# sxyu/plenoctree

Hardware: AMD Instinct MI355X
Metric: training rays/sec (800x800, 64+128 samples) (higher is better)
Workload: dtype f32

## Files before the change

### include/plenoctree_hip.h

```cpp
#ifndef PLENOCTREE_HIP_H_
#define PLENOCTREE_HIP_H_

#include <stddef.h>
#include <stdint.h>

#ifdef __cplusplus
extern "C" {
#endif

#define PXO_OK 0
#define PXO_ERR_ARG (-1)
#define PXO_ERR_HIP (-2)
#define PXO_ERR_WORKSPACE (-3)
#define PXO_ERR_UNSUPPORTED (-4)

#define PXO_NET_DEPTH 8
#define PXO_NET_WIDTH 256
#define PXO_SKIP_LAYER 4
#define PXO_ENC_DIM 63
#define PXO_ENC_PAD 64
#define PXO_NUM_LEAVES 20
#define PXO_VD_NUM_LEAVES 24
#define PXO_VD_WIDTH_CONDITION 128
#define PXO_VD_DIR_ENC 27

typedef struct PxoCfg {
  int32_t num_coarse_samples;
  int32_t num_fine_samples;
  int32_t sh_deg;
  int32_t min_deg_point;
  int32_t max_deg_point;
  int32_t white_bkgd;
  int32_t lindisp;
  int32_t sparsity_npoints;
  float near_;
  float far_;
  float sparsity_weight;
  float sparsity_length;
  float sparsity_radius;
  float weight_decay_mult;
  int32_t mlp_precision;
  float noise_std;
  int32_t skip_zero_rows;
} PxoCfg;

#define PXO_MLP_F32 0
#define PXO_MLP_BF16X3 1
#define PXO_MLP_BF16X6 2

typedef struct PxoLeaf {
  int32_t layer;
  int32_t is_bias;
  int64_t offset;
  int32_t rows;
  int32_t cols;
} PxoLeaf;

#define PXO_ABI_VERSION 9
const char* pxo_last_error(void);
int pxo_version(void);
size_t pxo_cfg_bytes(void);
int pxo_tile_rows(void);

int pxo_param_layout(const PxoCfg* cfg, PxoLeaf* leaves, int64_t* floats_per_mlp);

int pxo_packed_sizes(const PxoCfg* cfg, int64_t* fwd_floats, int64_t* bwd_floats);
int pxo_pack_weights(const PxoCfg* cfg, const float* mlp_params, float* packed_fwd,
                     float* packed_bwd, void* stream);


int pxo_sample_along_rays(const float* origins, const float* directions, int64_t B, int S,
                          float near_, float far_, int lindisp, const float* t_rand,
                          float* z_vals, float* pts, void* stream);

int pxo_posenc(const float* x, int64_t N, float* enc, void* stream);

size_t pxo_relu_mask_bytes(int64_t M);
int pxo_mlp_fwd(const PxoCfg* cfg, const float* packed_fwd, const float* pts, int64_t M,
                float* raw_rgb, float* raw_sigma, float* acts, float* enc, void* relu_mask,
                void* stream);

size_t pxo_dbias_partial_bytes(int64_t M);
int pxo_mlp_bwd_data(const PxoCfg* cfg, const float* packed_bwd, const float* d_raw_rgb,
                     const float* d_raw_sigma, const void* relu_mask, int64_t M, float* dz,
                     float* dbias_partial, void* stream);

int pxo_wgrad_workspace_bytes(const PxoCfg* cfg, int64_t M, size_t* bytes);
int pxo_mlp_bwd_weights(const PxoCfg* cfg, const float* acts, const float* enc, const float* dz,
                        const float* d_raw_rgb, const float* d_raw_sigma,
                        const float* dbias_partial, int64_t M, float* grads, void* ws,
                        size_t ws_bytes, void* stream);

int pxo_shade_composite_fwd(const PxoCfg* cfg, const float* raw_rgb, const float* raw_sigma,
                            const float* z_vals, const float* directions, const float* viewdirs,
                            int64_t B, int S, float* comp_rgb, float* disp, float* acc,
                            float* weights, void* stream);
int pxo_shade_composite_bwd(const PxoCfg* cfg, const float* raw_rgb, const float* raw_sigma,
                            const float* z_vals, const float* directions, const float* viewdirs,
                            const float* d_comp_rgb, int64_t B, int S, float* d_raw_rgb,
                            float* d_raw_sigma, void* stream);

int pxo_shade_composite_train(const PxoCfg* cfg, const float* raw_rgb, const float* raw_sigma,
                              const float* z_vals, const float* directions, const float* viewdirs,
                              const float* pixels, int64_t B, int S, float* comp_rgb, float* weights,
                              float* ray_sse, float* d_raw_rgb, float* d_raw_sigma, int64_t n_sp,
                              float* sp_exp, void* stream);

int pxo_sample_pdf(const float* z_coarse, const float* w_coarse, const float* origins,
                   const float* directions, int64_t B, int Nc, int Nf, const float* u,
                   float* z_out, float* pts, void* stream);

int pxo_add_gaussian_noise(float* raw, int64_t n, float noise_std, const float* noise, uint64_t seed,
                           uint64_t stream_id, void* stream);

int pxo_uniform(uint64_t seed, uint64_t stream_id, int64_t n, float lo, float hi, float* out,
                void* stream);

int pxo_randint(uint64_t seed, uint64_t stream_id, int64_t count, int64_t n, int64_t* out, void* stream);

int pxo_generate_rays(const float* c2w, int W, int H, float focal, const int64_t* pixel_ids, int64_t B,
                      float* origins, float* directions, float* viewdirs, void* stream);

int pxo_sample_batch(uint64_t seed, uint64_t stream_id, const float* c2w, int W, int H, float focal,
                     const float* image_rgb, int64_t B, int64_t first, int64_t* pixel_ids, float* origins,
                     float* directions, float* viewdirs, float* pixels, void* stream);

int pxo_generate_rays_multi(const float* c2w, int n_cams, int W, int H, float focal, const int64_t* ray_ids,
                            int64_t B, float* origins, float* directions, float* viewdirs, void* stream);

int pxo_generate_rays_ndc(const float* c2w, int n_cams, int W, int H, float focal, float ndc_near, const int64_t* ray_ids,
                          int64_t B, float* origins, float* directions, float* viewdirs, void* stream);

int pxo_sample_batch_ndc(uint64_t seed, uint64_t stream_id, const float* c2w, int W, int H, float focal, float ndc_near,
                         const float* image_rgb, int64_t B, int64_t first, int64_t* pixel_ids, float* origins,
                         float* directions, float* viewdirs, float* pixels, void* stream);

int pxo_mean_over_samples(const PxoCfg* cfg, const float* raw_rgb, const float* raw_sigma, int64_t n_cells,
                          int S, float* out, void* stream);

int pxo_adam_step(float* params, float* m, float* v, const float* grads, int64_t n, float lr,
                  int64_t step, float grad_scale, void* stream);

int pxo_adam_pack_step(const PxoCfg* cfg, float* params, float* m, float* v, const float* grads, float lr,
                       int64_t step, float grad_scale, float* packed_fwd0, float* packed_bwd0,
                       float* packed_fwd1, float* packed_bwd1, void* stream);


int pxo_render_workspace_bytes(const PxoCfg* cfg, int64_t B, size_t* bytes);
int pxo_render_fwd(const PxoCfg* cfg, const float* packed_fwd0, const float* packed_fwd1,
                   const float* origins, const float* directions, const float* viewdirs,
                   int64_t B, int randomized, const float* t_rand, const float* u, uint64_t seed,
                   float* rgb_c, float* disp_c, float* acc_c, float* rgb_f, float* disp_f,
                   float* acc_f, void* ws, size_t ws_bytes, void* stream);

int pxo_sg_render_fwd(const PxoCfg* cfg, const float* lobes, const float* packed_fwd0, const float* packed_fwd1,
                      const float* origins, const float* directions, const float* viewdirs, int64_t B, int randomized,
                      const float* t_rand, const float* u, uint64_t seed, float* rgb_c, float* disp_c, float* acc_c,
                      float* rgb_f, float* disp_f, float* acc_f, void* ws, size_t ws_bytes, void* stream);

#define PXO_OCC_MAX_RESO 1024
#define PXO_OCC_MAX_CHANNELS 4096
typedef struct PxoOccGrid {
  const uint32_t* bits;
  int32_t reso;
  float offset[3];
  float scale[3];
  int32_t outside_live;
} PxoOccGrid;

int pxo_occ_pack(const float* sigma, int reso, float sigma_thresh, int dilate, uint32_t* bits, void* stream);

int pxo_occ_cull_workspace_bytes(int64_t M, size_t* bytes);
int pxo_occ_cull(const PxoOccGrid* occ, const float* pts, int64_t M, float* pts_live, int32_t* slot, int64_t* n_live_dev, void* ws,
                 size_t ws_bytes, void* stream);

int pxo_occ_expand(const float* raw_rgb_live, const float* raw_sigma_live, const int32_t* slot, int64_t M, int C, float* raw_rgb,
                   float* raw_sigma, void* stream);

int pxo_render_culled_workspace_bytes(const PxoCfg* cfg, int64_t B, size_t* bytes);
int pxo_render_fwd_culled(const PxoCfg* cfg, const PxoOccGrid* occ, const float* lobes, const float* packed_fwd0,
                          const float* packed_fwd1, const float* origins, const float* directions, const float* viewdirs, int64_t B,
                          int randomized, const float* t_rand, const float* u, uint64_t seed, float* rgb_c, float* disp_c,
                          float* acc_c, float* rgb_f, float* disp_f, float* acc_f, int64_t live_rows[2], void* ws, size_t ws_bytes,
                          void* stream);

int pxo_occ_gather(const float* d_raw_rgb, const float* d_raw_sigma, const int32_t* slot, int64_t M, int C, float* d_rgb_live,
                   float* d_sigma_live, void* stream);

int pxo_train_culled_workspace_bytes(const PxoCfg* cfg, int64_t B, size_t* bytes);
int pxo_train_fwd_bwd_culled(const PxoCfg* cfg, const PxoOccGrid* occ, const float* params, const float* packed_fwd0,
                             const float* packed_bwd0, const float* packed_fwd1, const float* packed_bwd1, const float* origins,
                             const float* directions, const float* viewdirs, const float* pixels, int64_t B, int randomized,
                             const float* t_rand, const float* u, const float* sp_points, uint64_t seed, float* grads,
                             float* stats, void* ws, size_t ws_bytes, void* grads0_ready, void* stream, int64_t live_rows[2]);

int pxo_sg_lobes(const float* sg_params, int K, float* lobes, void* stream);

#define PXO_SG_RAYS_PER_BLOCK 4
int pxo_sg_shade_composite_train(const PxoCfg* cfg, const float* lobes, const float* raw_rgb, const float* raw_sigma,
                                 const float* z_vals, const float* directions, const float* viewdirs,
                                 const float* pixels, int64_t B, int S, float* comp_rgb, float* weights,
                                 float* ray_sse, float* d_raw_rgb, float* d_raw_sigma, int64_t n_sp,
                                 float* sp_exp, float* d_lobes, float* lobe_partials, void* stream);

int pxo_sg_train_workspace_bytes(const PxoCfg* cfg, int64_t B, size_t* bytes);
int pxo_sg_train_fwd_bwd_bucketed(const PxoCfg* cfg, const float* params, const float* sg_params, const float* packed_fwd0,
                                  const float* packed_bwd0, const float* packed_fwd1, const float* packed_bwd1,
                                  const float* origins, const float* directions, const float* viewdirs,
                                  const float* pixels, int64_t B, int randomized, const float* t_rand, const float* u,
                                  const float* sp_points, uint64_t seed, float* grads, float* sg_grads, float* stats,
                                  void* ws, size_t ws_bytes, void* grads0_ready, void* stream);
int pxo_sg_train_fwd_bwd(const PxoCfg* cfg, const float* params, const float* sg_params, const float* packed_fwd0,
                         const float* packed_bwd0, const float* packed_fwd1, const float* packed_bwd1,
                         const float* origins, const float* directions, const float* viewdirs, const float* pixels,
                         int64_t B, int randomized, const float* t_rand, const float* u, const float* sp_points,
                         uint64_t seed, float* grads, float* sg_grads, float* stats, void* ws, size_t ws_bytes,
                         void* stream);

int pxo_train_workspace_bytes(const PxoCfg* cfg, int64_t B, size_t* bytes);
int pxo_train_fwd_bwd(const PxoCfg* cfg, const float* params, const float* packed_fwd0,
                      const float* packed_bwd0, const float* packed_fwd1,
                      const float* packed_bwd1, const float* origins, const float* directions,
                      const float* viewdirs, const float* pixels, int64_t B, int randomized,
                      const float* t_rand, const float* u, const float* sp_points, uint64_t seed,
                      float* grads, float* stats, void* ws, size_t ws_bytes, void* stream);

int pxo_train_fwd_bwd_bucketed(const PxoCfg* cfg, const float* params, const float* packed_fwd0,
                               const float* packed_bwd0, const float* packed_fwd1,
                               const float* packed_bwd1, const float* origins, const float* directions,
                               const float* viewdirs, const float* pixels, int64_t B, int randomized,
                               const float* t_rand, const float* u, const float* sp_points, uint64_t seed,
                               float* grads, float* stats, void* ws, size_t ws_bytes, void* grads0_ready,
                               void* stream);

int pxo_train_backward_work(const PxoCfg* cfg, int64_t B, void* ws, size_t ws_bytes, int64_t* live_chunks,
                            int64_t* total_chunks, void* stream);

int pxo_event_create(void** event);
int pxo_event_destroy(void* event);
int pxo_stream_wait_event(void* stream, void* event);

int pxo_eval_points(const PxoCfg* cfg, const float* packed_fwd, const float* points, int64_t N,
                    float* raw_rgb, float* raw_sigma, void* stream);

int pxo_grid_sigma(const PxoCfg* cfg, const float* packed_fwd, int reso, int x0, int x1,
                   const float offset[3], const float scale[3], float* sigma_out, void* stream);

int pxo_vd_param_layout(PxoLeaf* leaves, int64_t* floats_per_mlp);
int pxo_vd_packed_floats(int64_t* floats);
int pxo_vd_pack_weights(const float* mlp_params, float* packed, void* stream);

int pxo_vd_eval_workspace_bytes(int64_t N, int64_t R, int cross_broadcast, size_t* bytes);
int pxo_vd_eval_points_raw(int mlp_precision, const float* packed, const float* points, int64_t N, const float* viewdirs,
                           int64_t R, int cross_broadcast, float* raw_rgb, float* raw_sigma, void* ws, size_t ws_bytes,
                           void* stream);

int pxo_vd_project_workspace_bytes(int64_t N, int64_t R, size_t* bytes);
int pxo_vd_project_sh(int mlp_precision, const float* packed, const float* points, int64_t N, const float* dirs, int64_t R,
                      int sh_deg, float* coeffs, float* raw_sigma, void* ws, size_t ws_bytes, void* stream);

int pxo_vd_render_workspace_bytes(const PxoCfg* cfg, int64_t B, size_t* bytes);
int pxo_vd_render_fwd(const PxoCfg* cfg, const float* packed0, const float* packed1, const float* origins,
                      const float* directions, const float* viewdirs, int64_t B, int randomized, const float* t_rand,
                      const float* u, uint64_t seed, float* rgb_c, float* disp_c, float* acc_c, float* rgb_f, float* disp_f,
                      float* acc_f, void* ws, size_t ws_bytes, void* stream);
int pxo_vd_composite_fwd(const PxoCfg* cfg, const float* raw_rgb, const float* raw_sigma, const float* z_vals,
                         const float* directions, int64_t B, int S, float* comp_rgb, float* disp, float* acc,
                         float* weights, void* stream);

#define PXO_TUNE_TILE_SCHED 0
#define PXO_TUNE_WGRAD_RANGES 1
#define PXO_TUNE_WGRAD_SKINNY_RANGES 2
#define PXO_TUNE_COARSE_REVERSE_STREAM 3
#define PXO_TUNE_X6_WGRAD 4
#define PXO_TUNE_VD_RAY_BLOCK 5
#define PXO_VD_RAY_BLOCK_DEFAULT 1024
#define PXO_VD_RAY_BLOCK_MAX 4096
int pxo_set_tuning(int knob, int value);
int pxo_get_tuning(int knob, int* value);

int pxo_occupy_cus(int blocks, int threads, float micros, int lds_bytes, void* stream);

#define PXO_PROF_MLP_FWD 0
#define PXO_PROF_MLP_BWD_DATA 1
#define PXO_PROF_WGRAD_MAIN 2
#define PXO_PROF_WGRAD_OTHER 3
#define PXO_PROF_NUM_TAGS 4
#define PXO_PROF_ALL ((1 << PXO_PROF_NUM_TAGS) - 1)
int pxo_profile_enable(int tag_mask);
int pxo_profile_read(int tag, int64_t* launches, double* total_ms, int64_t* total_rows);

#ifdef __cplusplus
}
#endif
#endif
```

### plenoctree_amd/_lib.py

```python
import ctypes
import os
from ctypes import (POINTER, Structure, c_char_p, c_double, c_float, c_int, c_int32, c_int64, c_size_t,
                    c_uint64, c_void_p)

HERE = os.path.dirname(os.path.abspath(__file__))
LIB_PATH = os.path.join(HERE, "libplenoctree_hip.so")

NET_DEPTH = 8
NET_WIDTH = 256
ENC_DIM = 63
ENC_PAD = 64
NUM_LEAVES = 20
VD_NUM_LEAVES = 24
VD_WIDTH_CONDITION = 128
VD_DIR_ENC = 27
MLP_F32, MLP_BF16X3, MLP_BF16X6 = 0, 1, 2


class PxoError(RuntimeError):
    pass


class PxoCfg(Structure):
    _fields_ = [
        ("num_coarse_samples", c_int32),
        ("num_fine_samples", c_int32),
        ("sh_deg", c_int32),
        ("min_deg_point", c_int32),
        ("max_deg_point", c_int32),
        ("white_bkgd", c_int32),
        ("lindisp", c_int32),
        ("sparsity_npoints", c_int32),
        ("near_", c_float),
        ("far_", c_float),
        ("sparsity_weight", c_float),
        ("sparsity_length", c_float),
        ("sparsity_radius", c_float),
        ("weight_decay_mult", c_float),
        ("mlp_precision", c_int32),
        ("noise_std", c_float),
        ("skip_zero_rows", c_int32),
    ]


class PxoLeaf(Structure):
    _fields_ = [
        ("layer", c_int32),
        ("is_bias", c_int32),
        ("offset", c_int64),
        ("rows", c_int32),
        ("cols", c_int32),
    ]


class PxoRenderOpts(Structure):
    _fields_ = [("step_size", c_float), ("background_brightness", c_float), ("sigma_thresh", c_float),
                ("stop_thresh", c_float)]


class PxoTree(Structure):
    _fields_ = [("child", c_void_p), ("data", c_void_p), ("n_internal", c_int64), ("data_dim", c_int32),
                ("basis_dim", c_int32), ("offset", c_float * 3), ("invradius", c_float * 3)]


class PxoCamera(Structure):
    _fields_ = [("c2w", c_void_p), ("fx", c_float), ("fy", c_float), ("width", c_int32), ("height", c_int32)]


class PxoNdc(Structure):
    _fields_ = [("width", c_int32), ("height", c_int32), ("focal", c_float), ("near", c_float)]


class PxoQuantLayout(Structure):
    _fields_ = [("idx_offset", c_int64), ("palette_offset", c_int64), ("sigma_offset", c_int64),
                ("retained_offset", c_int64), ("total_bytes", c_int64), ("idx_stride", c_int32), ("ret_stride", c_int32)]


class PxoQuantTree(Structure):
    _fields_ = [("child", c_void_p), ("idx", c_void_p), ("palette", c_void_p), ("sigma", c_void_p), ("retained", c_void_p),
                ("n_internal", c_int64), ("basis_dim", c_int32), ("n_retained", c_int32), ("bits", c_int32),
                ("idx_stride", c_int32), ("ret_stride", c_int32), ("offset", c_float * 3), ("invradius", c_float * 3)]


class PxoHalfTree(Structure):
    _fields_ = [("child", c_void_p), ("data", c_void_p), ("n_internal", c_int64), ("data_dim", c_int32),
                ("basis_dim", c_int32), ("row_stride", c_int32), ("offset", c_float * 3), ("invradius", c_float * 3)]


class PxoOccGrid(Structure):
    _fields_ = [("bits", c_void_p), ("reso", c_int32), ("offset", c_float * 3), ("scale", c_float * 3), ("outside_live", c_int32)]


OCC_MAX_RESO = 1024
TREE_MAX_DEPTH = 10
ABI_VERSION = 9
SG_RAYS_PER_BLOCK = 4

P = c_void_p
CFG = POINTER(PxoCfg)
F3 = POINTER(c_float)

SIGNATURES = {
    "pxo_last_error": (c_char_p, []),
    "pxo_version": (c_int, []),
    "pxo_cfg_bytes": (c_size_t, []),
    "pxo_set_tuning": (c_int, [c_int, c_int]),
    "pxo_get_tuning": (c_int, [c_int, POINTER(c_int)]),
    "pxo_occupy_cus": (c_int, [c_int, c_int, c_float, c_int, P]),
    "pxo_tile_rows": (c_int, []),
    "pxo_param_layout": (c_int, [CFG, POINTER(PxoLeaf), POINTER(c_int64)]),
    "pxo_packed_sizes": (c_int, [CFG, POINTER(c_int64), POINTER(c_int64)]),
    "pxo_pack_weights": (c_int, [CFG, P, P, P, P]),
    "pxo_sample_along_rays": (c_int, [P, P, c_int64, c_int, c_float, c_float, c_int, P, P, P, P]),
    "pxo_posenc": (c_int, [P, c_int64, P, P]),
    "pxo_relu_mask_bytes": (c_size_t, [c_int64]),
    "pxo_mlp_fwd": (c_int, [CFG, P, P, c_int64, P, P, P, P, P, P]),
    "pxo_dbias_partial_bytes": (c_size_t, [c_int64]),
    "pxo_mlp_bwd_data": (c_int, [CFG, P, P, P, P, c_int64, P, P, P]),
    "pxo_wgrad_workspace_bytes": (c_int, [CFG, c_int64, POINTER(c_size_t)]),
    "pxo_mlp_bwd_weights": (c_int, [CFG, P, P, P, P, P, P, c_int64, P, P, c_size_t, P]),
    "pxo_shade_composite_fwd": (c_int, [CFG, P, P, P, P, P, c_int64, c_int, P, P, P, P, P]),
    "pxo_shade_composite_bwd": (c_int, [CFG, P, P, P, P, P, P, c_int64, c_int, P, P, P]),
    "pxo_shade_composite_train": (c_int, [CFG, P, P, P, P, P, P, c_int64, c_int, P, P, P, P, P, c_int64, P, P]),
    "pxo_sample_pdf": (c_int, [P, P, P, P, c_int64, c_int, c_int, P, P, P, P]),
    "pxo_add_gaussian_noise": (c_int, [P, c_int64, c_float, P, c_uint64, c_uint64, P]),
    "pxo_uniform": (c_int, [c_uint64, c_uint64, c_int64, c_float, c_float, P, P]),
    "pxo_randint": (c_int, [c_uint64, c_uint64, c_int64, c_int64, P, P]),
    "pxo_generate_rays": (c_int, [P, c_int, c_int, c_float, P, c_int64, P, P, P, P]),
    "pxo_sample_batch": (c_int, [c_uint64, c_uint64, P, c_int, c_int, c_float, P, c_int64, c_int64, P, P, P, P, P, P]),
    "pxo_generate_rays_multi": (c_int, [P, c_int, c_int, c_int, c_float, P, c_int64, P, P, P, P]),
    "pxo_generate_rays_ndc": (c_int, [P, c_int, c_int, c_int, c_float, c_float, P, c_int64, P, P, P, P]),
    "pxo_sample_batch_ndc": (c_int, [c_uint64, c_uint64, P, c_int, c_int, c_float, c_float, P, c_int64, c_int64, P, P, P, P, P,
                                     P]),
    "pxo_mean_over_samples": (c_int, [CFG, P, P, c_int64, c_int, P, P]),
    "pxo_adam_step": (c_int, [P, P, P, P, c_int64, c_float, c_int64, c_float, P]),
    "pxo_adam_pack_step": (c_int, [CFG, P, P, P, P, c_float, c_int64, c_float, P, P, P, P, P]),
    "pxo_render_workspace_bytes": (c_int, [CFG, c_int64, POINTER(c_size_t)]),
    "pxo_render_fwd": (c_int, [CFG, P, P, P, P, P, c_int64, c_int, P, P, c_uint64, P, P, P, P, P, P, P,
                               c_size_t, P]),
    "pxo_sg_render_fwd": (c_int, [CFG, P, P, P, P, P, P, c_int64, c_int, P, P, c_uint64, P, P, P, P, P, P, P,
                                  c_size_t, P]),
    "pxo_occ_pack": (c_int, [P, c_int, c_float, c_int, P, P]),
    "pxo_occ_cull_workspace_bytes": (c_int, [c_int64, POINTER(c_size_t)]),
    "pxo_occ_cull": (c_int, [POINTER(PxoOccGrid), P, c_int64, P, P, P, P, c_size_t, P]),
    "pxo_occ_expand": (c_int, [P, P, P, c_int64, c_int, P, P, P]),
    "pxo_render_culled_workspace_bytes": (c_int, [CFG, c_int64, POINTER(c_size_t)]),
    "pxo_render_fwd_culled": (c_int, [CFG, POINTER(PxoOccGrid), P, P, P, P, P, P, c_int64, c_int, P, P, c_uint64, P, P, P, P, P, P,
                                      POINTER(c_int64), P, c_size_t, P]),
    "pxo_occ_gather": (c_int, [P, P, P, c_int64, c_int, P, P, P]),
    "pxo_train_culled_workspace_bytes": (c_int, [CFG, c_int64, POINTER(c_size_t)]),
    "pxo_train_fwd_bwd_culled": (c_int, [CFG, POINTER(PxoOccGrid), P, P, P, P, P, P, P, P, P, c_int64, c_int, P, P, P, c_uint64, P,
                                         P, P, c_size_t, P, P, POINTER(c_int64)]),
    "pxo_train_workspace_bytes": (c_int, [CFG, c_int64, POINTER(c_size_t)]),
    "pxo_train_fwd_bwd": (c_int, [CFG, P, P, P, P, P, P, P, P, P, c_int64, c_int, P, P, P, c_uint64, P, P,
                                  P, c_size_t, P]),
    "pxo_train_fwd_bwd_bucketed": (c_int, [CFG, P, P, P, P, P, P, P, P, P, c_int64, c_int, P, P, P, c_uint64, P, P,
                                           P, c_size_t, P, P]),
    "pxo_sg_lobes": (c_int, [P, c_int, P, P]),
    "pxo_sg_shade_composite_train": (c_int, [CFG, P, P, P, P, P, P, P, c_int64, c_int, P, P, P, P, P, c_int64, P, P, P, P]),
    "pxo_sg_train_workspace_bytes": (c_int, [CFG, c_int64, POINTER(c_size_t)]),
    "pxo_sg_train_fwd_bwd": (c_int, [CFG, P, P, P, P, P, P, P, P, P, P, c_int64, c_int, P, P, P, c_uint64, P, P, P,
                                     P, c_size_t, P]),
    "pxo_sg_train_fwd_bwd_bucketed": (c_int, [CFG, P, P, P, P, P, P, P, P, P, P, c_int64, c_int, P, P, P, c_uint64, P, P, P,
                                              P, c_size_t, P, P]),
    "pxo_train_backward_work": (c_int, [CFG, c_int64, P, c_size_t, POINTER(c_int64), POINTER(c_int64), P]),
    "pxo_event_create": (c_int, [POINTER(c_void_p)]),
    "pxo_event_destroy": (c_int, [P]),
    "pxo_stream_wait_event": (c_int, [P, P]),
    "pxo_eval_points": (c_int, [CFG, P, P, c_int64, P, P, P]),
    "pxo_profile_enable": (c_int, [c_int]),
    "pxo_profile_read": (c_int, [c_int, POINTER(c_int64), POINTER(ctypes.c_double), POINTER(c_int64)]),
    "pxo_grid_sigma": (c_int, [CFG, P, c_int, c_int, c_int, POINTER(c_float), POINTER(c_float), P, P]),
    "pxo_vd_param_layout": (c_int, [POINTER(PxoLeaf), POINTER(c_int64)]),
    "pxo_vd_packed_floats": (c_int, [POINTER(c_int64)]),
    "pxo_vd_pack_weights": (c_int, [P, P, P]),
    "pxo_vd_eval_workspace_bytes": (c_int, [c_int64, c_int64, c_int, POINTER(c_size_t)]),
    "pxo_vd_eval_points_raw": (c_int, [c_int, P, P, c_int64, P, c_int64, c_int, P, P, P, c_size_t, P]),
    "pxo_vd_project_workspace_bytes": (c_int, [c_int64, c_int64, POINTER(c_size_t)]),
    "pxo_vd_project_sh": (c_int, [c_int, P, P, c_int64, P, c_int64, c_int, P, P, P, c_size_t, P]),
    "pxo_vd_render_workspace_bytes": (c_int, [CFG, c_int64, POINTER(c_size_t)]),
    "pxo_vd_render_fwd": (c_int, [CFG, P, P, P, P, P, c_int64, c_int, P, P, c_uint64, P, P, P, P, P, P, P, c_size_t, P]),
    "pxo_vd_composite_fwd": (c_int, [CFG, P, P, P, P, c_int64, c_int, P, P, P, P, P]),
    "pxo_threshold_mask": (c_int, [P, c_int64, c_float, P, P]),
    "pxo_tree_workspace_bytes": (c_int, [c_int, POINTER(c_size_t)]),
    "pxo_tree_count_nodes": (c_int, [P, c_int, P, c_size_t, POINTER(c_int64), P]),
    "pxo_tree_build": (c_int, [P, c_size_t, c_int, POINTER(c_int64), P, P, P]),
    "pxo_tree_sample_cells": (c_int, [P, c_int64, c_int64, c_int, P, F3, F3, P, P]),
    "pxo_tree_sample_leaves": (c_int, [P, P, c_int64, c_int, P, F3, F3, P, P]),
    "pxo_tree_query": (c_int, [P, P, c_int64, F3, F3, P, P]),
    "pxo_tree_relu_sigma": (c_int, [P, c_int64, c_int, P]),
    "pxo_grid_weight_workspace_bytes": (c_int, [c_int, POINTER(c_size_t)]),
    "pxo_grid_weight_render": (c_int, [P, c_int, P, c_int, c_float, c_float, c_int, c_int, POINTER(PxoRenderOpts),
                                       F3, F3, P, P, c_size_t, P]),
    "pxo_octree_set_lanes_per_ray": (c_int, [c_int, c_int]),
    "pxo_octree_set_tuning": (c_int, [c_int, c_int]),
    "pxo_octree_get_tuning": (c_int, [c_int, POINTER(c_int)]),
    "pxo_octree_render_fwd": (c_int, [POINTER(PxoTree), POINTER(PxoCamera), P, P, P, c_int64,
                                      POINTER(PxoRenderOpts), P, P]),
    "pxo_octree_render_aux_fwd": (c_int, [POINTER(PxoTree), POINTER(PxoCamera), P, P, P, c_int64,
                                          POINTER(PxoRenderOpts), c_float, P, P, P]),
    "pxo_octree_render_bwd": (c_int, [POINTER(PxoTree), POINTER(PxoCamera), P, P, P, c_int64,
                                      POINTER(PxoRenderOpts), P, P, P, P]),
    "pxo_octree_render_sg_fwd": (c_int, [POINTER(PxoTree), P, POINTER(PxoCamera), P, P, P, c_int64,
                                         POINTER(PxoRenderOpts), P, P]),
    "pxo_octree_render_sg_bwd": (c_int, [POINTER(PxoTree), P, POINTER(PxoCamera), P, P, P, c_int64,
                                         POINTER(PxoRenderOpts), P, P, P, P]),
    "pxo_octree_render_ndc_fwd": (c_int, [POINTER(PxoTree), POINTER(PxoCamera), P, P, P, c_int64,
                                          POINTER(PxoRenderOpts), P, P, POINTER(PxoNdc)]),
    "pxo_octree_render_ndc_bwd": (c_int, [POINTER(PxoTree), POINTER(PxoCamera), P, P, P, c_int64,
                                          POINTER(PxoRenderOpts), P, P, P, P, POINTER(PxoNdc)]),
    "pxo_grid_weight_render_ndc": (c_int, [P, c_int, P, c_int, c_float, c_float, c_int, c_int, POINTER(PxoRenderOpts),
                                           F3, F3, P, P, c_size_t, P, POINTER(PxoNdc)]),
    "pxo_octree_quant_pack_bytes": (c_int, [c_int64, c_int, c_int, c_int, POINTER(PxoQuantLayout)]),
    "pxo_octree_quant_pack": (c_int, [P, P, P, c_int, P, c_int64, c_int, c_int, c_int, P, c_size_t, P]),
    "pxo_octree_render_quant_fwd": (c_int, [POINTER(PxoQuantTree), POINTER(PxoCamera), P, P, P, c_int64,
                                            POINTER(PxoRenderOpts), P, P]),
    "pxo_octree_render_quant_aux_fwd": (c_int, [POINTER(PxoQuantTree), POINTER(PxoCamera), P, P, P, c_int64,
                                                POINTER(PxoRenderOpts), c_float, P, P, P]),
    "pxo_octree_half_pack_bytes": (c_int, [c_int64, c_int, POINTER(c_int32), POINTER(c_int64)]),
    "pxo_octree_half_pack": (c_int, [P, c_int64, c_int, P, c_size_t, P]),
    "pxo_octree_render_half_fwd": (c_int, [POINTER(PxoHalfTree), P, POINTER(PxoCamera), P, P, P, c_int64,
                                           POINTER(PxoRenderOpts), P, P, POINTER(PxoNdc)]),
    "pxo_octree_render_half_aux_fwd": (c_int, [POINTER(PxoHalfTree), POINTER(PxoCamera), P, P, P, c_int64,
                                               POINTER(PxoRenderOpts), c_float, P, P, P]),
    "pxo_octree_count_work": (c_int, [POINTER(PxoTree), POINTER(PxoCamera), POINTER(PxoRenderOpts), P, P, P]),
    "pxo_grid_weight_count_work": (c_int, [P, c_int, P, c_int, c_float, c_float, c_int, c_int, POINTER(PxoRenderOpts),
                                           F3, F3, P, P, P]),
    "pxo_octree_weight_accum_cams": (c_int, [POINTER(PxoTree), P, c_int, c_float, c_float, c_int, c_int, POINTER(PxoRenderOpts),
                                             c_int, P, P, POINTER(PxoNdc)]),
    "pxo_octree_weight_accum_rays": (c_int, [POINTER(PxoTree), P, P, c_int64, POINTER(PxoRenderOpts), c_int, P, P,
                                             POINTER(PxoNdc)]),
    "pxo_tree_collapse_mark": (c_int, [P, P, P, c_int64, c_int, P, P]),
    "pxo_tree_collapse_emit": (c_int, [P, P, P, c_int, P, P, P, c_int64, c_int64, P, P, P, P, P]),
    "pxo_tree_lod_fill": (c_int, [P, P, P, c_int64, c_int, c_int, P]),
    "pxo_octree_render_foot_fwd": (c_int, [POINTER(PxoTree), P, POINTER(PxoCamera), P, P, P, c_int64,
                                           POINTER(PxoRenderOpts), c_float, c_int, P, P]),
    "pxo_octree_render_foot_aux_fwd": (c_int, [POINTER(PxoTree), POINTER(PxoCamera), P, P, P, c_int64,
                                               POINTER(PxoRenderOpts), c_float, c_int, c_float, P, P, P]),
    "pxo_mc_workspace_bytes": (c_int, [c_int, c_int, c_int, POINTER(c_size_t)]),
    "pxo_mc_count": (c_int, [P, c_int, c_int, c_int, c_double, P, P, c_size_t, POINTER(c_int64), P]),
    "pxo_mc_emit": (c_int, [P, c_int, c_int, c_int, c_double, P, P, c_size_t, POINTER(c_int64), P, P, P, P]),
    "pxo_tree_sigma_grid": (c_int, [POINTER(PxoTree), c_int, c_int, P, P, P]),
    "pxo_mc_vertex_gradients": (c_int, [P, c_int, c_int, c_int, c_double, P, c_size_t, POINTER(c_int64), P, P, P]),
    "pxo_shade_points": (c_int, [P, c_int64, P, P, c_int64, c_int, P, P, P]),
    "pxo_image_mse": (c_int, [P, P, c_int64, P, P, P]),
    "pxo_sgd_step": (c_int, [P, P, P, c_int64, c_float, c_float, c_int, c_int, P]),
}

_lib = None


def load(path=None):
    global _lib
    if _lib is not None:
        return _lib
    if path is None and os.environ.get("PXO_LIB"):
        if os.environ.get("PXO_ALLOW_VARIANT") != "1":
            raise PxoError("PXO_LIB is set but PXO_ALLOW_VARIANT != 1: refusing to load a variant kernel library")
        path = os.environ["PXO_LIB"]
    path = path or LIB_PATH
    import torch
    if torch.cuda.is_available():
        torch.cuda.init()
    if not os.path.exists(path):
        raise PxoError(
            f"{path} not found: build it with `python -m plenoctree_amd.build` "
            "(hipcc --offload-arch=gfx950); there is no CPU fallback")
    lib = ctypes.CDLL(path)
    for name, (restype, argtypes) in SIGNATURES.items():
        try:
            fn = getattr(lib, name)
# ... 33 lines not shown
```

### plenoctree_amd/csrc/mlp_kernels.hip

```cpp
#include "pxo_mlp.h"

namespace pxo {

__global__ void pack_fwd_kernel(const float* __restrict__ p, int deg, float* __restrict__ out) {
  const int nhb = head_blocks(deg);
  const int64_t total = fwd_image_floats(deg);
  const int64_t bias_off = fwd_bias_off(deg);
  for (int64_t idx = blockIdx.x * (int64_t)blockDim.x + threadIdx.x; idx < total;
       idx += (int64_t)gridDim.x * blockDim.x) {
    float v;
    if (idx >= bias_off) {
      v = fwd_image_bias(p, deg, (int)(idx - bias_off));
    } else {
      int l = 0;
      while (l < 8 && idx >= fwd_layer_off(l + 1)) ++l;
      int64_t loc = idx - fwd_layer_off(l);
      const int ncb = l < 8 ? 8 : nhb;
      int j = (int)(loc & 3), lane = (int)((loc >> 2) & 63);
      int64_t cg = loc >> 8;
      int c = (int)(cg % ncb), g = (int)(cg / ncb);
      int k = 8 * g + 4 * (lane >> 5) + j, n = 32 * c + (lane & 31);
      v = src_weight(p, deg, l, k, n);
    }
    out[idx] = v;
// ... 7 lines not shown
  for (int64_t idx = blockIdx.x * (int64_t)blockDim.x + threadIdx.x; idx < total;
       idx += (int64_t)gridDim.x * blockDim.x) {
    int l;
    int64_t loc;
    if (idx < head_sz) { l = 8; loc = idx; }
    else { int q = (int)((idx - head_sz) / (256 * 256)); l = 7 - q; loc = idx - head_sz - (int64_t)q * 256 * 256; }
    int j = (int)(loc & 3), lane = (int)((loc >> 2) & 63);
    int64_t cg = loc >> 8;
    int c = (int)(cg % 8), g = (int)(cg / 8);
    int k = 8 * g + 4 * (lane >> 5) + j, n = 32 * c + (lane & 31);
    out[idx] = src_weight(p, deg, l, n, k);
  }
}

int launch_pack(const PxoCfg* cfg, const float* mlp_params, float* fwd, float* bwd, hipStream_t s) {
  if (cfg->mlp_precision == PXO_MLP_BF16X6) return launch_pack_x6(cfg, mlp_params, fwd, bwd, s);
  if (cfg->mlp_precision == PXO_MLP_BF16X3) {
    if (bwd) { set_error("pack_weights: mlp_precision bf16x3 is forward-only (packed_bwd must be NULL)"); return PXO_ERR_UNSUPPORTED; }
    return launch_pack_x3(cfg, mlp_params, fwd, s);
  }
  hipLaunchKernelGGL(pack_fwd_kernel, dim3(512), dim3(256), 0, s, mlp_params, cfg->sh_deg, fwd);
  if (bwd) hipLaunchKernelGGL(pack_bwd_kernel, dim3(512), dim3(256), 0, s, mlp_params, cfg->sh_deg, bwd);
  return check_launch("pack_weights");
}

__global__ void posenc_kernel(const float* __restrict__ x, int64_t N, float* __restrict__ enc) {
  int64_t idx = blockIdx.x * (int64_t)blockDim.x + threadIdx.x;
  if (idx >= N * kEnc) return;
  int64_t r = idx / kEnc;
  int col = (int)(idx - r * kEnc);
  enc[idx] = enc_value(x[r * 3], x[r * 3 + 1], x[r * 3 + 2], col);
}

int launch_posenc(const float* x, int64_t N, float* enc, hipStream_t s) {
  if (N == 0) return PXO_OK;
  int64_t total = N * kEnc;
  hipLaunchKernelGGL(posenc_kernel, dim3((unsigned)((total + 255) / 256)), dim3(256), 0, s, x, N, enc);
  return check_launch("posenc");
}

template <int RBN> struct EncGeom {
  static constexpr int kRows = 32 * RBN;
  static constexpr int kParts = kMlpThreads / kRows;
  static constexpr int kColsPer = kEncPad / kParts;
};
template <int RBN, bool GRID = true, bool KEEP = false>
__device__ __forceinline__ void posenc_tile(float* __restrict__ lds, const float* __restrict__ pts,
                                            const GridSpec& grid, int64_t row0, int64_t M, int tid,
                                            float (*keep)[EncGeom<RBN>::kColsPer] = nullptr) {
  constexpr int kRows = EncGeom<RBN>::kRows, kColsPer = EncGeom<RBN>::kColsPer;
  const int row = tid % kRows, part = tid / kRows;
  const int64_t grow = row0 + row;
  float p0 = 0.f, p1 = 0.f, p2 = 0.f;
  if (grow < M) {
    if (GRID && grid.enabled) grid_point(grid, grow, p0, p1, p2);
    else { p0 = pts[grow * 3]; p1 = pts[grow * 3 + 1]; p2 = pts[grow * 3 + 2]; }
  }
#pragma unroll 4
  for (int i = 0; i < kColsPer; ++i) {
    const int col = part * kColsPer + i;
    const float e = enc_value(p0, p1, p2, col);
    lds[row * kLDA + col] = e;
    if (KEEP) (*keep)[i] = e;
  }
}
template <int RBN>
__device__ __forceinline__ void posenc_restore(float* __restrict__ lds, int tid, const float (&keep)[EncGeom<RBN>::kColsPer]) {
  constexpr int kRows = EncGeom<RBN>::kRows, kColsPer = EncGeom<RBN>::kColsPer;
  const int row = tid % kRows, part = tid / kRows;
#pragma unroll
  for (int i = 0; i < kColsPer; ++i) lds[row * kLDA + part * kColsPer + i] = keep[i];
}

template <int RBN, int CBN>
__device__ __forceinline__ void mfma_group(const f32x4 (&a)[RBN], const f32x4 (&b)[CBN], f32x16 (&acc)[RBN][CBN]) {
#pragma unroll
  for (int j = 0; j < 4; ++j)
#pragma unroll
    for (int r = 0; r < RBN; ++r)
#pragma unroll
      for (int c = 0; c < CBN; ++c)
        acc[r][c] = __builtin_amdgcn_mfma_f32_32x32x2f32(a[r][j], b[c][j], acc[r][c], 0, 0, 0);
}

struct ARows {
  const float* base;
  uint32_t lo, hi;
};
__device__ __forceinline__ ARows make_arows(const float* lds, int lane) {
  ARows a{lds, (uint32_t)((lane & 31) * kLDA + (lane >> 5) * 4), 0u};
  a.hi = a.lo + 2 * 32 * kLDA;
  asm volatile("" : "+v"(a.hi));
  return a;
}
template <int RBN>
__device__ __forceinline__ void load_a(const ARows& ar, int g, f32x4 (&a)[RBN]) {
#pragma unroll
  for (int r = 0; r < RBN; ++r)
    a[r] = *reinterpret_cast<const f32x4*>(ar.base + (r < 2 ? ar.lo : ar.hi) + (r & 1) * 32 * kLDA + g * 8);
}
struct WImage {
  __amdgpu_buffer_rsrc_t rsrc;
  uint32_t voff;
};
__device__ __forceinline__ WImage make_wimage(const float* image, int64_t floats, int lane) {
  return WImage{__builtin_amdgcn_make_buffer_rsrc(const_cast<float*>(image), 0, (int)(floats * 4), 0x00020000),
                (uint32_t)lane * 16u};
}
typedef unsigned int u32x4 __attribute__((ext_vector_type(4)));
template <int CBN>
__device__ __forceinline__ void load_b(const WImage& w, int wu, int g, int kg_stride, f32x4 (&b)[CBN]) {
#pragma unroll
  for (int c = 0; c < CBN; ++c)
    b[c] = __builtin_bit_cast(f32x4, __builtin_amdgcn_raw_buffer_load_b128(w.rsrc, w.voff, (wu + g * kg_stride + c * 64) * 16, 0));
}

constexpr int kBDist = 3;
template <int CBN>
__device__ __forceinline__ void gemm_prefetch_b(const WImage& w, int wu, int kgroups, int kg_stride,
                                                f32x4 (&b)[4][CBN]) {
  const int last = kgroups - 1;
#pragma unroll
  for (int i = 0; i < kBDist; ++i) load_b<CBN>(w, wu, i < last ? i : last, kg_stride, b[i]);
}

struct TileCopy {
  __amdgpu_buffer_rsrc_t out;
  uint32_t voff;
  const float* src;
  uint32_t src_hi;
  bool on;
};
template <int RBN>
__device__ __forceinline__ TileCopy make_tile_copy(const float* lds, float* dst, int64_t row0, int64_t M, int wave, int lane,
                                                   bool on) {
  const int c4 = lane & 7, rsub = lane >> 3;
  const int64_t rows = M - row0 < 32 * RBN ? M - row0 : 32 * RBN;
  TileCopy t;
  t.out = __builtin_amdgcn_make_buffer_rsrc(dst + row0 * kW, 0, on ? (int)(rows * kW * 4) : 0, 0x00020000);
  t.voff = (uint32_t)(rsub * kW + wave * 32 + c4 * 4) * 4u;
  t.src = lds + rsub * kLDA + wave * 32 + c4 * 4;
  t.src_hi = 8 * 8 * kLDA;
  asm volatile("" : "+v"(t.src_hi));
  t.on = on;
  return t;
}
template <int RBN>
__device__ __forceinline__ void tile_copy_slab(const TileCopy& t, int i) {
  const f32x4 v = i < 8 ? *reinterpret_cast<const f32x4*>(t.src + i * 8 * kLDA)
                        : *reinterpret_cast<const f32x4*>(t.src + t.src_hi + (i - 8) * 8 * kLDA);
  __builtin_amdgcn_raw_buffer_store_b128(__builtin_bit_cast(u32x4, v), t.out, t.voff, i * 8 * kW * 4, 0);
}

template <int RBN, int CBN, bool COPY = false>
__device__ __forceinline__ void gemm_lds_packed(const ARows& arow, const WImage& w, int wu,
                                                int kgroups, int kg_stride, f32x16 (&acc)[RBN][CBN],
                                                f32x4 (&b)[4][CBN], const TileCopy* tc = nullptr) {
  constexpr int D = kBDist;
  static_assert(D == 2 || D == 3, "kBDist");
  f32x4 a0[RBN], a1[RBN];
  const int last = kgroups - 1;
  auto cl = [&](int g) { return g < last ? g : last; };
  load_a<RBN>(arow, 0, a0);
  for (int g = 0; g < kgroups; g += 4) {
    load_a<RBN>(arow, g + 1, a1);
    load_b<CBN>(w, wu, cl(g + D), kg_stride, b[D & 3]);
    PXO_PIN();
    mfma_group<RBN, CBN>(a0, b[0], acc);
    PXO_PIN();
    if (COPY && tc->on && g < 4 * RBN) {
      switch (g >> 2) {
        case 0: tile_copy_slab<RBN>(*tc, 0); break;
        case 1: tile_copy_slab<RBN>(*tc, 4 + 0); break;
        case 2: if (RBN > 2) tile_copy_slab<RBN>(*tc, 8 + 0); break;
        default: if (RBN > 2) tile_copy_slab<RBN>(*tc, 12 + 0); break;
      }
      PXO_PIN();
    }
    load_a<RBN>(arow, g + 2, a0);
    load_b<CBN>(w, wu, cl(g + 1 + D), kg_stride, b[(1 + D) & 3]);
    PXO_PIN();
    mfma_group<RBN, CBN>(a1, b[1], acc);
    PXO_PIN();
    if (COPY && tc->on && g < 4 * RBN) {
      switch (g >> 2) {
        case 0: tile_copy_slab<RBN>(*tc, 1); break;
        case 1: tile_copy_slab<RBN>(*tc, 4 + 1); break;
        case 2: if (RBN > 2) tile_copy_slab<RBN>(*tc, 8 + 1); break;
        default: if (RBN > 2) tile_copy_slab<RBN>(*tc, 12 + 1); break;
      }
      PXO_PIN();
    }
    load_a<RBN>(arow, g + 3, a1);
    load_b<CBN>(w, wu, cl(g + 2 + D), kg_stride, b[(2 + D) & 3]);
    PXO_PIN();
    mfma_group<RBN, CBN>(a0, b[2], acc);
    PXO_PIN();
    if (COPY && tc->on && g < 4 * RBN) {
      switch (g >> 2) {
        case 0: tile_copy_slab<RBN>(*tc, 2); break;
        case 1: tile_copy_slab<RBN>(*tc, 4 + 2); break;
        case 2: if (RBN > 2) tile_copy_slab<RBN>(*tc, 8 + 2); break;
        default: if (RBN > 2) tile_copy_slab<RBN>(*tc, 12 + 2); break;
      }
      PXO_PIN();
    }
    load_a<RBN>(arow, cl(g + 4), a0);
    load_b<CBN>(w, wu, cl(g + 3 + D), kg_stride, b[(3 + D) & 3]);
    PXO_PIN();
    mfma_group<RBN, CBN>(a1, b[3], acc);
    PXO_PIN();
    if (COPY && tc->on && g < 4 * RBN) {
      switch (g >> 2) {
        case 0: tile_copy_slab<RBN>(*tc, 3); break;
        case 1: tile_copy_slab<RBN>(*tc, 4 + 3); break;
        case 2: if (RBN > 2) tile_copy_slab<RBN>(*tc, 8 + 3); break;
        default: if (RBN > 2) tile_copy_slab<RBN>(*tc, 12 + 3); break;
      }
      PXO_PIN();
    }
  }
}

template <int CBN>
__device__ __forceinline__ void gemm_head(const float* __restrict__ arow, const f32x4* __restrict__ wp, int cb_stride,
                                          int kg_stride, f32x16 (&acc)[1][CBN]) {
  f32x4 a0[1], a1[1], b0[CBN], b1[CBN], b2[CBN], b3[CBN];
  auto lb = [&](int g, f32x4 (&b)[CBN]) {
#pragma unroll
    for (int c = 0; c < CBN; ++c) b[c] = wp[(int64_t)g * kg_stride + c * cb_stride];
  };
  auto la = [&](int g, f32x4 (&a)[1]) { a[0] = *reinterpret_cast<const f32x4*>(arow + g * 8); };
  lb(0, b0); lb(1, b1);
  la(0, a0);
  for (int g = 0; g < 32; g += 4) {
    la(g + 1, a1); lb(g + 2, b2); PXO_PIN();
    mfma_group<1, CBN>(a0, b0, acc); PXO_PIN();
    la(g + 2, a0); lb(g + 3, b3); PXO_PIN();
    mfma_group<1, CBN>(a1, b1, acc); PXO_PIN();
    la(g + 3, a1); lb(g + 4 < 31 ? g + 4 : 31, b0); PXO_PIN();
    mfma_group<1, CBN>(a0, b2, acc); PXO_PIN();
    la(g + 4 < 31 ? g + 4 : 31, a0); lb(g + 5 < 31 ? g + 5 : 31, b1); PXO_PIN();
    mfma_group<1, CBN>(a1, b3, acc); PXO_PIN();
  }
}

template <int RBN, int CBN>
__device__ __forceinline__ void zero_acc(f32x16 (&acc)[RBN][CBN]) {
#pragma unroll
  for (int r = 0; r < RBN; ++r)
#pragma unroll
    for (int c = 0; c < CBN; ++c)
#pragma unroll
      for (int i = 0; i < 16; ++i) acc[r][c][i] = 0.f;
}

__device__ __forceinline__ int frag_row(int reg, int lane) { return (reg & 3) + 8 * (reg >> 2) + 4 * (lane >> 5); }

template <int RBN>
__device__ __forceinline__ void store_wave_cols(const float* __restrict__ lds, float* __restrict__ dst, int64_t row0,
                                                int64_t M, int wave, int lane) {
  const int c4 = lane & 7, rsub = lane >> 3;
  const int64_t rows = M - row0 < 32 * RBN ? M - row0 : 32 * RBN;
  const __amdgpu_buffer_rsrc_t out = __builtin_amdgcn_make_buffer_rsrc(dst + row0 * kW, 0, (int)(rows * kW * 4), 0x00020000);
  const uint32_t voff = (uint32_t)(rsub * kW + wave * 32 + c4 * 4) * 4u;
  const float* __restrict__ src = lds + rsub * kLDA + wave * 32 + c4 * 4;
#pragma unroll
  for (int i0 = 0; i0 < 4 * RBN; i0 += 4) {
    f32x4 v[4];
#pragma unroll
    for (int i = 0; i < 4; ++i) v[i] = *reinterpret_cast<const f32x4*>(src + (i0 + i) * 8 * kLDA);
#pragma unroll
    for (int i = 0; i < 4; ++i)
      __builtin_amdgcn_raw_buffer_store_b128(__builtin_bit_cast(u32x4, v[i]), out, voff, (i0 + i) * 8 * kW * 4, 0);
  }
}

__device__ __forceinline__ float mask_pop(uint32_t& mw, float x) {
  float r;
  asm volatile("v_add_co_u32 %0, vcc, %0, %0\n\tv_cndmask_b32 %1, 0, %2, vcc" : "+v"(mw), "=v"(r) : "v"(x) : "vcc");
  return r;
}

constexpr int kRB = kTM / 32;
constexpr int kCB = 8 / kMlpWaves;

template <int NHB, bool SAVE, bool RGB, int RBN>
__device__ __forceinline__ void fwd_tile(float* __restrict__ lds, const float* __restrict__ pk,
                                         const float* __restrict__ pts, const GridSpec& grid, int64_t M, int deg,
                                         int64_t row0, int64_t slot, float* __restrict__ raw_rgb,
                                         float* __restrict__ raw_sigma, float* __restrict__ acts,
                                         float* __restrict__ enc_out, uint32_t* __restrict__ mask, int tid, int lane,
                                         int wave) {
  constexpr int kRows = 32 * RBN;
  constexpr int kWordsUsed = RBN * kCB * 16 / 32;
  asm volatile("" : "+v"(tid));
  lane = tid & 63;
  const int C = rgb_channels(deg);
  const float* __restrict__ bias = pk + fwd_bias_off(deg);
  const float* arow1 = lds + (lane & 31) * kLDA + (lane >> 5) * 4;
  const ARows arow = make_arows(lds, lane);
  const WImage wimg = make_wimage(pk, fwd_image_floats(deg), lane);
  const bool full = row0 + kRows <= M;
  lds_barrier();
  float enc_keep[EncGeom<RBN>::kColsPer];
  posenc_tile<RBN, !SAVE, !SAVE>(lds, pts, grid, row0, M, tid, &enc_keep);
  lds_barrier();
  if (SAVE) {
#pragma unroll
    for (int i = 0; i < kRows * kEncPad / 4 / kMlpThreads; ++i) {
// ... 152 lines not shown

unsigned mlp_grid(int64_t M) {
  const int64_t tiles = num_tiles(M), cap = kMlpWgPerCu * (int64_t)num_cus();
  return (unsigned)(tiles < cap ? tiles : cap);
}

static int launch_fwd_any(const PxoCfg* cfg, const float* pk, const float* pts, const GridSpec& grid,
                          int64_t M, float* raw_rgb, float* raw_sigma, float* acts, float* enc,
                          uint32_t* mask, unsigned int* tile_counter, hipStream_t s) {
  if (M == 0) return PXO_OK;
  KernelTimer timer(PXO_PROF_MLP_FWD, M, s);
  dim3 grid_dim(mlp_grid(M)), block(kMlpThreads);
  const TileSched ts = tile_sched(M, grid_dim.x);
  head_switch(cfg->sh_deg, [&](auto nhb) {
    constexpr int NHB = decltype(nhb)::value;
    const auto kernel = acts && raw_rgb && tile_counter ? mlp_fwd_kernel<NHB, true, true, true>
                        : acts && raw_rgb               ? mlp_fwd_kernel<NHB, true, true>
                        : acts                          ? mlp_fwd_kernel<NHB, true, false>
                        : raw_rgb                       ? mlp_fwd_kernel<NHB, false, true>
                                                        : mlp_fwd_kernel<NHB, false, false>;
    hipLaunchKernelGGL(kernel, grid_dim, block, 0, s, pk, pts, grid, M, cfg->sh_deg, ts, raw_rgb, raw_sigma, acts, enc, mask,
                       tile_counter);
  });
  return check_launch("mlp_fwd");
}

int launch_mlp_fwd(const PxoCfg* cfg, const float* packed_fwd, const float* pts, int64_t M,
                   float* raw_rgb, float* raw_sigma, float* acts, float* enc, uint32_t* mask,
                   hipStream_t s, unsigned int* tile_counter) {
  if (cfg->mlp_precision == PXO_MLP_BF16X6)
    return launch_mlp_fwd_x6(cfg, packed_fwd, pts, 0, 0, nullptr, nullptr, M, raw_rgb, raw_sigma, acts, enc, mask, tile_counter, s);
  if (cfg->mlp_precision == PXO_MLP_BF16X3) {
    if (acts || enc || mask) { set_error("mlp_fwd: mlp_precision bf16x3 is inference-only (no saved tensors)"); return PXO_ERR_UNSUPPORTED; }
    return launch_mlp_fwd_x3(cfg, packed_fwd, pts, 0, 0, nullptr, nullptr, M, raw_rgb, raw_sigma, s);
  }
  return launch_fwd_any(cfg, packed_fwd, pts, make_grid_spec(false, 0, 0, nullptr, nullptr), M, raw_rgb, raw_sigma, acts, enc,
                        mask, tile_counter, s);
}

int launch_mlp_fwd_grid(const PxoCfg* cfg, const float* packed_fwd, int reso, int x0, int x1,
                        const float* off, const float* scale, float* sigma_out, hipStream_t s) {
  const int64_t M = (int64_t)(x1 - x0) * reso * reso;
  if (cfg->mlp_precision == PXO_MLP_BF16X6)
    return launch_mlp_fwd_x6(cfg, packed_fwd, nullptr, reso, x0, off, scale, M, nullptr, sigma_out, nullptr, nullptr, nullptr,
                             nullptr, s);
  if (cfg->mlp_precision == PXO_MLP_BF16X3)
    return launch_mlp_fwd_x3(cfg, packed_fwd, nullptr, reso, x0, off, scale, M, nullptr, sigma_out, s);
  return launch_fwd_any(cfg, packed_fwd, nullptr, make_grid_spec(true, reso, x0, off, scale), M, nullptr, sigma_out, nullptr,
                        nullptr, nullptr, nullptr, s);
}

template <int NHB, int RBN, bool SKIP>
__device__ __forceinline__ int bwd_tile(float* __restrict__ lds, float* __restrict__ db_slot, uint8_t* __restrict__ tile_live,
                                         const float* __restrict__ pkb, const float* __restrict__ d_raw_rgb,
                                         const float* __restrict__ d_raw_sigma, const uint32_t* __restrict__ mask,
                                         int64_t M, int deg, int64_t row0, int64_t slot, float* __restrict__ dz,
                                         int* __restrict__ nz, uint8_t* __restrict__ chunk_live,
                                         int tid, int lane, int wave, int mask_word0 = 0) {
  constexpr int NH = 32 * NHB;
  constexpr int kRows = 32 * RBN;
  constexpr int kWordsUsed = RBN * kCB * 16 / 32;
  constexpr int kChunks = kRows / kLiveRows;
  const int C = rgb_channels(deg);
  const ARows arow = make_arows(lds, lane);
  const WImage wimg = make_wimage(pkb, bwd_image_floats(deg), lane);
  lds_barrier();
  if (SKIP && tid < kChunks) nz[tid] = 0;
  if (SKIP) lds_barrier();
  for (int idx = tid; idx < kRows * NH; idx += kMlpThreads) {
    const int row = idx / NH, col = idx - row * NH;
    const int64_t grow = row0 + row;
    float v = 0.f;
    if (grow < M) {
      if (col < C) { if (d_raw_rgb) v = d_raw_rgb[grow * C + col]; }
      else if (col == C) v = d_raw_sigma[grow];
    }
    lds[row * kLDA + col] = v;
    if (SKIP && v != 0.f) nz[row / kLiveRows] = 1;
  }
  lds_barrier();
  if (SKIP) {
    int any = 0;
#pragma unroll
    for (int c = 0; c < kChunks; ++c) any |= nz[c];
    if (tid < kChunks) chunk_live[row0 / kLiveRows + tid] = (uint8_t)nz[tid];
    if (tid == 0) *tile_live = (uint8_t)(any != 0);
    if (!any) return 0;
    if (RBN == kRB) {
      int lo = 0, hi = 0;
#pragma unroll
      for (int c = 0; c < kChunks / 2; ++c) { lo |= nz[c]; hi |= nz[kChunks / 2 + c]; }
      if (!hi) return 1;
      if (!lo) return 2;
    }
  } else if (tid == 0) {
    *tile_live = 1;
  }
  if (tid < NH) {
    float sum = 0.f;
#pragma unroll 8
    for (int row = 0; row < kRows; ++row) sum += lds[row * kLDA + tid];
    db_slot[8 * kW + tid] = sum;
  }
  if (NH < kW && tid >= NH && tid < kW) db_slot[8 * kW + tid] = 0.f;

  f32x16 acc[RBN][kCB];
  f32x4 bfrag[4][kCB];
  zero_acc(acc);
  uint32_t mw[kMaskWords];
  {
    const uint32_t* mp = mask + ((slot * kDepth + (kDepth - 1)) * kMlpThreads + tid) * kMaskWords + mask_word0;
#pragma unroll
    for (int w = 0; w < kWordsUsed; ++w) mw[w] = mp[w];
    const int wp = (wave * kCB) * 64;
    gemm_prefetch_b<kCB>(wimg, wp, 4 * NHB, 8 * 64, bfrag);
    gemm_lds_packed<RBN, kCB>(arow, wimg, wp, 4 * NHB, 8 * 64, acc, bfrag);
  }
  for (int l = kDepth - 1; l >= 0; --l) {
    const int wp = (int)(bwd_layer_off(l > 0 ? l : 1, deg) / 4) + (wave * kCB) * 64;
    if (l > 0) gemm_prefetch_b<kCB>(wimg, wp, 32, 8 * 64, bfrag);
    lds_barrier();
    int tid_e = tid;
    asm volatile("" : "+v"(tid_e));
    const int lane_e = tid_e & 63;
#pragma unroll
    for (int c = 0; c < kCB; ++c) {
      const int col = (wave * kCB + c) * 32 + (lane_e & 31);
      float colsum = 0.f;
#pragma unroll
      for (int r = 0; r < RBN; ++r)
#pragma unroll
        for (int reg = 0; reg < 16; ++reg) {
          const int row = r * 32 + frag_row(reg, lane_e);
          const float v = mask_pop(mw[((r * kCB + c) * 16 + reg) >> 5], acc[r][c][reg]);
          lds[row * kLDA + col] = v;
          colsum += v;
        }
      colsum += __shfl_xor(colsum, 32);
      if (lane_e < 32) db_slot[l * kW + col] = colsum;
    }
    if (l == 0) store_wave_cols<RBN>(lds, dz, row0, M, wave, lane_e);
    lds_barrier();
    if (l == 0) break;
    zero_acc(acc);
    const uint32_t* mp = mask + ((slot * kDepth + (l - 1)) * kMlpThreads + tid_e) * kMaskWords + mask_word0;
#pragma unroll
    for (int w = 0; w < kWordsUsed; ++w) mw[w] = mp[w];
    const TileCopy tc = make_tile_copy<RBN>(lds, dz + (int64_t)l * M * kW, row0, M, wave, lane, true);
    gemm_lds_packed<RBN, kCB, true>(arow, wimg, wp, 32, 8 * 64, acc, bfrag, &tc);
  }
  return 0;
}

template <int NHB, bool SKIP, bool DYN>
__global__ __launch_bounds__(kMlpThreads, kMlpWgPerCu * kMlpWaves / 4) void mlp_bwd_data_kernel(
    const float* __restrict__ pkb, const float* __restrict__ d_raw_rgb,
    const float* __restrict__ d_raw_sigma, const uint32_t* __restrict__ mask, int64_t M, int deg, TileSched ts,
    float* __restrict__ dz, float* __restrict__ dbias_partial, uint8_t* __restrict__ chunk_live,
    unsigned int* __restrict__ tile_counter) {
  __shared__ __attribute__((aligned(16))) float lds[kTM * kLDA + kTM / kLiveRows + 4];
  int* __restrict__ nz = reinterpret_cast<int*>(lds + kTM * kLDA);
  const int tid = threadIdx.x, lane = tid & 63;
  const int wave = __builtin_amdgcn_readfirstlane(tid >> 6);
  uint8_t* const tile_live = reinterpret_cast<uint8_t*>(dbias_partial + mask_slots(M) * 9 * kW);
  const int64_t n_slots = ts.n_full + ts.n_half;
  auto run = [&](int64_t slot) {
    float* db = dbias_partial + slot * 9 * kW;
    if (slot < ts.n_full) {
      const int half = bwd_tile<NHB, kRB, SKIP>(lds, db, tile_live + slot, pkb, d_raw_rgb, d_raw_sigma, mask, M, deg,
                                                slot * kTM, slot, dz, nz, chunk_live, tid, lane, wave);
      if (SKIP && half)
        bwd_tile<NHB, kRB / 2, SKIP>(lds, db, tile_live + slot, pkb, d_raw_rgb, d_raw_sigma, mask, M, deg,
                                     slot * kTM + (half - 1) * (kTM / 2), slot, dz, nz, chunk_live, tid, lane, wave, half - 1);
    } else
      bwd_tile<NHB, kRB / 2, SKIP>(lds, db, tile_live + slot, pkb, d_raw_rgb, d_raw_sigma, mask, M, deg,
                             ts.half_row0 + (slot - ts.n_full) * (kTM / 2), slot, dz, nz, chunk_live, tid, lane, wave);
  };
  if (!DYN) {
    for (int64_t slot = blockIdx.x; slot < ts.n_full; slot += gridDim.x) run(slot);
    for (int64_t h = blockIdx.x; h < ts.n_half; h += gridDim.x) run(ts.n_full + h);
  } else {
    const TileTicket tk{nz + kTM / kLiveRows, tile_counter};
    for (int64_t slot = blockIdx.x; slot < n_slots;) {
      const int ticket = tk.draw(tid);
      run(slot);
      slot = tk.take(tid, ticket);
    }
  }
}

int mlp_bwd_partials(int64_t M) {
  const TileSched ts = tile_sched(M, mlp_grid(M));
  return (int)(ts.n_full + ts.n_half);
}

int launch_mlp_bwd_data(const PxoCfg* cfg, const float* packed_bwd, const float* d_raw_rgb,
                        const float* d_raw_sigma, const uint32_t* mask, int64_t M, float* dz,
                        float* dbias_partial, uint8_t* chunk_live, unsigned int* tile_counter, hipStream_t s,
                        bool bias_from_wgrad) {
  if (M == 0) return PXO_OK;
  if (cfg->mlp_precision == PXO_MLP_BF16X6)
    return launch_mlp_bwd_data_x6(cfg, packed_bwd, d_raw_rgb, d_raw_sigma, mask, M, dz, dbias_partial, chunk_live, tile_counter, s,
                                  !bias_from_wgrad);
  if (cfg->mlp_precision != PXO_MLP_F32) { set_error("mlp_bwd_data: mlp_precision bf16x3 is inference-only"); return PXO_ERR_UNSUPPORTED; }
  KernelTimer timer(PXO_PROF_MLP_BWD_DATA, M, s);
  dim3 grid_dim(mlp_grid(M)), block(kMlpThreads);
  const TileSched ts = tile_sched(M, grid_dim.x);
  head_switch(cfg->sh_deg, [&](auto nhb) {
    constexpr int NHB = decltype(nhb)::value;
    const auto kernel = chunk_live ? (tile_counter ? mlp_bwd_data_kernel<NHB, true, true> : mlp_bwd_data_kernel<NHB, true, false>)
                                   : (tile_counter ? mlp_bwd_data_kernel<NHB, false, true> : mlp_bwd_data_kernel<NHB, false, false>);
    hipLaunchKernelGGL(kernel, grid_dim, block, 0, s, packed_bwd, d_raw_rgb, d_raw_sigma, mask, M, cfg->sh_deg, ts, dz,
                       dbias_partial, chunk_live, tile_counter);
  });
  return check_launch("mlp_bwd_data");
}

}
```

### plenoctree_amd/csrc/pxo_api.hip

```cpp
#include <atomic>
#include <cstdarg>
#include <cstdio>
#include <cstring>
#include <string>
#include <vector>

#include "pxo_common.h"

namespace pxo {

static thread_local std::string g_last_error;

void set_error(const char* fmt, ...) {
  char buf[1024];
  va_list ap;
  va_start(ap, fmt);
  vsnprintf(buf, sizeof(buf), fmt, ap);
  va_end(ap);
  g_last_error = buf;
}

int check_launch(const char* what) {
  hipError_t e = hipGetLastError();
  if (e != hipSuccess) {
    set_error("%s: %s", what, hipGetErrorString(e));
    return PXO_ERR_HIP;
  }
  return PXO_OK;
}

int num_cus() {
  static int n = 0;
  if (n == 0) {
    int dev = 0;
    hipDeviceProp_t prop;
    if (hipGetDevice(&dev) == hipSuccess && hipGetDeviceProperties(&prop, dev) == hipSuccess) n = prop.multiProcessorCount;
    if (n <= 0) n = 256;
    if (2 * n > kMaxMlpGrid) n = kMaxMlpGrid / 2;
  }
  return n;
}

static std::atomic<int> g_tune_tile_sched{1};
static std::atomic<int> g_tune_wgrad_ranges{0};
static std::atomic<int> g_tune_wgrad_skinny_ranges{0};
static std::atomic<int> g_tune_x6_wgrad{1};
static std::atomic<int> g_tune_coarse_stream{0};
static std::atomic<int> g_tune_vd_ray_block{PXO_VD_RAY_BLOCK_DEFAULT};
Tuning tuning_snapshot() {
  return Tuning{g_tune_tile_sched.load(), g_tune_wgrad_ranges.load(), g_tune_wgrad_skinny_ranges.load(),
                g_tune_coarse_stream.load(), g_tune_x6_wgrad.load(), g_tune_vd_ray_block.load()};
}

struct SideStream { hipStream_t stream = nullptr; hipEvent_t fork = nullptr, join = nullptr; };
static SideStream* side_stream() {
  static thread_local std::vector<SideStream> per_device;
  int dev = 0;
  if (hipGetDevice(&dev) != hipSuccess || dev < 0) return nullptr;
  if ((size_t)dev >= per_device.size()) per_device.resize(dev + 1);
  SideStream& x = per_device[dev];
  if (x.stream) return &x;
  int lo = 0, hi = 0;
  (void)hipDeviceGetStreamPriorityRange(&lo, &hi);
  if (hipStreamCreateWithPriority(&x.stream, hipStreamNonBlocking, lo) != hipSuccess) { x.stream = nullptr; return nullptr; }
  if (hipEventCreateWithFlags(&x.fork, hipEventDisableTiming) != hipSuccess ||
      hipEventCreateWithFlags(&x.join, hipEventDisableTiming) != hipSuccess) {
    (void)hipStreamDestroy(x.stream);
    x.stream = nullptr;
    return nullptr;
  }
  return &x;
}

struct SideFork {
  hipStream_t s, sc;
  SideStream* side = nullptr;
  SideFork(hipStream_t s_, bool fork) : s(s_), sc(s_) {
    SideStream* x = fork ? side_stream() : nullptr;
    if (x && hipEventRecord(x->fork, s) == hipSuccess && hipStreamWaitEvent(x->stream, x->fork, 0) == hipSuccess) {
      side = x;
      sc = x->stream;
    }
  }
  ~SideFork() { (void)join(); }
  bool join() {
    if (!side) return true;
    SideStream* x = side;
    side = nullptr;
    return hipEventRecord(x->join, sc) == hipSuccess && hipStreamWaitEvent(s, x->join, 0) == hipSuccess;
  }
};

int validate_cfg(const PxoCfg* cfg) {
  PXO_REQUIRE(cfg != nullptr, "cfg is NULL");
  PXO_REQUIRE(cfg->sh_deg >= 0 && cfg->sh_deg <= 4, "sh_deg %d not in [0,4] (nerf_sh/nerf/sh.py:69)", cfg->sh_deg);
  PXO_REQUIRE(cfg->min_deg_point == 0 && cfg->max_deg_point == 10,
              "only min_deg_point=0,max_deg_point=10 is built (got %d,%d)", cfg->min_deg_point, cfg->max_deg_point);
  PXO_REQUIRE(cfg->num_coarse_samples >= 3 && cfg->num_coarse_samples <= 128, "num_coarse_samples %d not in [3,128]",
              cfg->num_coarse_samples);
  PXO_REQUIRE(cfg->num_fine_samples >= 0 && cfg->num_coarse_samples + cfg->num_fine_samples <= 256,
              "num_coarse_samples+num_fine_samples must be <= 256");
  PXO_REQUIRE(cfg->mlp_precision == PXO_MLP_F32 || cfg->mlp_precision == PXO_MLP_BF16X3 || cfg->mlp_precision == PXO_MLP_BF16X6,
              "mlp_precision %d unknown", cfg->mlp_precision);
  PXO_REQUIRE(cfg->noise_std >= 0.f, "noise_std %g < 0 (0 = None)", (double)cfg->noise_std);
  PXO_REQUIRE(cfg->skip_zero_rows == 0 || cfg->skip_zero_rows == 1, "skip_zero_rows %d is not 0 / 1", cfg->skip_zero_rows);
  return PXO_OK;
}

struct ProfRecord { hipEvent_t a, b; int tag; int64_t rows; };
static unsigned g_prof_mask = 0;
static std::vector<ProfRecord> g_prof;

KernelTimer::KernelTimer(int tag, int64_t rows, hipStream_t s) : slot(-1), stream(s) {
  if (!((g_prof_mask >> tag) & 1u)) return;
  ProfRecord r;
  if (hipEventCreate(&r.a) != hipSuccess || hipEventCreate(&r.b) != hipSuccess) return;
  r.tag = tag; r.rows = rows;
  (void)hipEventRecord(r.a, s);
  g_prof.push_back(r);
  slot = (int)g_prof.size() - 1;
}
KernelTimer::~KernelTimer() {
  if (slot >= 0) (void)hipEventRecord(g_prof[slot].b, stream);
}

struct Carver {
  char* base;
  size_t off = 0;
  explicit Carver(void* b) : base(reinterpret_cast<char*>(b)) {}
  template <typename T>
  T* take(int64_t count) {
    off = (off + 255) & ~(size_t)255;
    T* p = base ? reinterpret_cast<T*>(base + off) : nullptr;
    off += (size_t)count * sizeof(T);
    return p;
  }
};

struct PassBuffers {
  int64_t M = 0;
  int S = 0;
  float *z, *pts, *raw_rgb, *raw_sigma, *acts, *enc, *comp_rgb, *disp, *acc, *weights;
  uint32_t* mask;
  float *ray_sse, *d_raw_rgb, *d_raw_sigma, *dz, *dbias;
  uint8_t* live;
};

static void carve_pass(Carver& c, PassBuffers& p, int64_t B, int S, int64_t extra_rows, int C, bool train,
                       bool own_outputs) {
  p.S = S;
  p.M = B * S + extra_rows;
  p.z = c.take<float>(B * S);
  p.pts = c.take<float>(p.M * 3);
  p.raw_rgb = c.take<float>(p.M * C);
  p.raw_sigma = c.take<float>(p.M);
  p.weights = c.take<float>(B * S);
  if (own_outputs) {
    p.comp_rgb = c.take<float>(B * 3);
    p.disp = c.take<float>(B);
    p.acc = c.take<float>(B);
  }
  if (train) {
    p.acts = c.take<float>(p.M * kW * kDepth);
    p.enc = c.take<float>(p.M * kEncPad);
    p.mask = c.take<uint32_t>(mask_words(p.M));
    p.ray_sse = c.take<float>(B);
    p.d_raw_rgb = c.take<float>(p.M * C);
    p.d_raw_sigma = c.take<float>(p.M);
    p.dz = c.take<float>(p.M * kW * kDepth);
    p.dbias = c.take<float>(dbias_floats(p.M));
    p.live = c.take<uint8_t>(live_flags(p.M));
  } else {
    p.acts = p.enc = p.ray_sse = p.d_raw_rgb = p.d_raw_sigma = p.dz = p.dbias = nullptr;
    p.mask = nullptr;
    p.live = nullptr;
  }
}

constexpr int kStepWordsAt = 98;
constexpr int kStepWords = 6;
constexpr unsigned int kStepRecord = 0x5E7D5700u;
constexpr unsigned int kStepRecordCulled = 0x5E7DC000u;

struct TrainWs {
  PassBuffers c, f;
  float *t_rand, *u, *sp, *scalars, *sp_exp;
  void* wgrad_ws;
  size_t wgrad_bytes;
  int64_t n_sp;
  size_t total;
};

static void carve_train(const PxoCfg* cfg, int64_t B, void* ws, bool train, TrainWs& t) {
  Carver c(ws);
  const int C = rgb_channels(cfg->sh_deg);
  const int Nc = cfg->num_coarse_samples, Nf = cfg->num_fine_samples;
  const bool sp = train && cfg->sparsity_weight > 0.f && cfg->sparsity_npoints > 0;
  t.n_sp = sp ? cfg->sparsity_npoints : 0;
  carve_pass(c, t.c, B, Nc, Nf > 0 ? 0 : t.n_sp, C, train, train);
  if (Nf > 0) carve_pass(c, t.f, B, Nc + Nf, t.n_sp, C, train, train);
  t.t_rand = c.take<float>(B * Nc);
  t.u = c.take<float>(B * (Nf > 0 ? Nf : 1));
  t.sp = c.take<float>(t.n_sp * 3 + 4);
  t.scalars = c.take<float>(128);
// ... 44 lines not shown
  k.total = (c.off + 255) & ~(size_t)255;
}

#define PXO_TRY(expr)            \
  do {                           \
    int _rc = (expr);            \
    if (_rc != PXO_OK) return _rc; \
  } while (0)

struct Layout { TrainWs t; SgWs g; CullWs k; size_t total; };
static int lay_out(const PxoCfg* cfg, int64_t B, void* ws, size_t ws_bytes, bool train, bool sg, bool cull, const char* who,
                   Layout& L) {
  carve_train(cfg, B, ws, train, L.t);
  L.total = L.t.total;
  L.g = SgWs{nullptr, nullptr, nullptr, 0, L.total};
  if (sg) { carve_sg(cfg, B, ws, L.total, L.g); L.total = L.g.total; }
  if (cull) {
    const int S = cfg->num_coarse_samples + cfg->num_fine_samples;
    PXO_REQUIRE(B * (int64_t)S + L.t.n_sp < ((int64_t)1 << 31), "%s: %lld rays x %d samples exceed 2^31 rows", who, (long long)B, S);
    carve_cull(cfg, B, ws, L.t, train, L.k);
    L.total = L.k.total;
  }
  if (ws && ws_bytes < L.total) {
    set_error("%s: workspace %zu < %zu", who, ws_bytes, L.total);
    return PXO_ERR_WORKSPACE;
  }
  return PXO_OK;
}
static int workspace_bytes(const PxoCfg* cfg, int64_t B, bool train, bool sg, bool cull, const char* who, size_t* bytes) {
  PXO_TRY(validate_cfg(cfg));
  PXO_REQUIRE(bytes && B >= (train ? 1 : 0), "%s: bad arguments", who);
  Layout L;
  PXO_TRY(lay_out(cfg, B, nullptr, 0, train, sg, cull, who, L));
  *bytes = L.total;
  return PXO_OK;
}

struct CullCtx { const PxoOccGrid* occ; CullWs* k; int64_t* host; int64_t* live_rows; };
static int open_cull(const PxoOccGrid* occ, CullWs& k, int64_t* live_rows, const char* who, CullCtx& cx) {
  static thread_local int64_t* pinned = nullptr;
  if (!pinned && hipHostMalloc((void**)&pinned, 2 * sizeof(int64_t), hipHostMallocDefault) != hipSuccess) pinned = nullptr;
  if (!pinned) {
    set_error("%s: hipHostMalloc of the count words failed", who);
    return PXO_ERR_HIP;
  }
  cx = CullCtx{occ, &k, pinned, live_rows};
  return PXO_OK;
}
static int refuse_noise(const PxoCfg* cfg, int randomized, const char* who) {
  if (randomized && cfg->noise_std > 0.f) {
    set_error("%s: noise_std > 0 with randomized sampling (noise on a culled sample's zero sigma would resurrect it)", who);
    return PXO_ERR_UNSUPPORTED;
  }
  return PXO_OK;
}
static int require_train_precision(const PxoCfg* cfg, const char* who) {
  if (cfg->mlp_precision != PXO_MLP_F32 && cfg->mlp_precision != PXO_MLP_BF16X6) {
    set_error("%s: training runs in float32 or its float32-accurate bf16x6 emulation only (mlp_precision bf16x3 is an inference option)", who);
    return PXO_ERR_UNSUPPORTED;
  }
  return PXO_OK;
}

struct Draws { const float* t_rand; const float* u; bool noisy; uint64_t seed; };

static int prepare_draws(const PxoCfg* cfg, TrainWs& t, int64_t B, int randomized, const float* t_rand, const float* u,
                         const float* sp_points, uint64_t seed, hipStream_t s, Draws& out, const float* params = nullptr,
                         int64_t n_params = 0, float* sumsq_partial = nullptr, unsigned int* step_words = nullptr,
                         int n_words = 0, unsigned int first_word = 0) {
  const int Nc = cfg->num_coarse_samples, Nf = cfg->num_fine_samples;
  PassBuffers& last = Nf > 0 ? t.f : t.c;
  UniformJob jobs[3];
  int nj = 0;
  if (randomized && !t_rand) { jobs[nj++] = UniformJob{0, B * Nc, 0.f, 1.f, t.t_rand}; t_rand = t.t_rand; }
  if (randomized && Nf > 0 && !u) { jobs[nj++] = UniformJob{1, B * Nf, 0.f, 1.f, t.u}; u = t.u; }
  if (!randomized) { t_rand = nullptr; u = nullptr; }
  if (t.n_sp > 0) {
    float* dst = last.pts + B * last.S * 3;
    if (sp_points) {
      if (hipMemcpyAsync(dst, sp_points, (size_t)t.n_sp * 3 * sizeof(float), hipMemcpyDeviceToDevice, s) != hipSuccess) {
        set_error("hipMemcpyAsync(sp_points) failed");
        return PXO_ERR_HIP;
      }
    } else {
      jobs[nj++] = UniformJob{2, t.n_sp * 3, -cfg->sparsity_radius, cfg->sparsity_radius, dst};
    }
  }
  out.t_rand = t_rand; out.u = u;
  out.noisy = randomized != 0 && cfg->noise_std > 0.f;
  out.seed = seed;
  return launch_uniform_jobs(seed, jobs, nj, s, params, n_params, sumsq_partial, step_words, n_words, first_word);
}

static int level_forward(const PxoCfg* cfg, TrainWs& t, int level, const float* packed_fwd, const float* o, const float* d,
                         const float* v, int64_t B, const Draws& dr, const float* pixels, float* rgb, float* disp, float* acc,
                         hipStream_t s, unsigned int* tile_counter, const float* lobes, float* lobe_partials, const CullCtx* cx,
                         const char* who, int64_t* M_run = nullptr) {
  const int Nc = cfg->num_coarse_samples, Nf = cfg->num_fine_samples;
  const bool last = level == 1 || Nf == 0;
  PassBuffers& p = level == 0 ? t.c : t.f;
  if (level == 0)
    PXO_TRY(launch_sample_along_rays(o, d, B, Nc, cfg->near_, cfg->far_, cfg->lindisp, dr.t_rand, p.z, p.pts, s));
  else
    PXO_TRY(launch_sample_pdf(t.c.z, t.c.weights, o, d, B, Nc, Nf, dr.u, p.z, p.pts, s));
  int64_t M = p.M;
  if (!cx) {
    PXO_TRY(launch_mlp_fwd(cfg, packed_fwd, p.pts, M, p.raw_rgb, p.raw_sigma, p.acts, p.enc, p.mask, s, tile_counter));
  } else {
    CullWs& k = *cx->k;
    const int64_t rows = B * p.S, extra = p.M - rows;
    PXO_TRY(launch_occ_cull(*cx->occ, p.pts, rows, k.pts_live, k.slot, k.n_live + level, k.cull, s));
    if (hipMemcpyAsync(cx->host + level, k.n_live + level, sizeof(int64_t), hipMemcpyDeviceToHost, s) != hipSuccess ||
        hipStreamSynchronize(s) != hipSuccess) {
      set_error("%s: reading the live-row count: %s", who, hipGetErrorString(hipGetLastError()));
      return PXO_ERR_HIP;
    }
    const int64_t n_live = cx->host[level];
    if (n_live < 0 || n_live > rows) {
      set_error("%s: live-row count %lld outside [0, %lld]", who, (long long)n_live, (long long)rows);
      return PXO_ERR_HIP;
    }
    if (extra > 0) {
      if (hipMemcpyAsync(k.pts_live + 3 * n_live, p.pts + 3 * rows, (size_t)extra * 3 * sizeof(float), hipMemcpyDeviceToDevice, s) !=
          hipSuccess) {
        set_error("%s: hipMemcpyAsync(sparsity points) failed", who);
        return PXO_ERR_HIP;
      }
      PXO_TRY(launch_occ_tail_slots(k.slot + rows, extra, n_live, s));
    }
    M = n_live + extra;
    if (M > 0) PXO_TRY(launch_mlp_fwd(cfg, packed_fwd, k.pts_live, M, k.rgb_live, k.sigma_live, p.acts, p.enc, p.mask, s, tile_counter));
    PXO_TRY(launch_occ_expand(k.rgb_live, k.sigma_live, k.slot, p.M, rgb_channels(cfg->sh_deg), p.raw_rgb, p.raw_sigma, s));
    if (cx->live_rows) cx->live_rows[level] = n_live;
  }
  if (M_run) *M_run = M;
  if (dr.noisy) PXO_TRY(launch_add_noise(p.raw_sigma, B * p.S, cfg->noise_std, nullptr, dr.seed, 3 + level, s));
  if (pixels)
    return launch_shade_composite_train(cfg, p.raw_rgb, p.raw_sigma, p.z, d, v, pixels, B, p.S, nullptr, last ? nullptr : p.weights,
                                        p.ray_sse, p.d_raw_rgb, p.d_raw_sigma, last ? t.n_sp : 0, t.sp_exp, lobes, lobe_partials, s);
  return launch_shade_composite_fwd(cfg, p.raw_rgb, p.raw_sigma, p.z, d, v, B, p.S, rgb, disp, acc, p.weights, s, lobes);
}

static int level_reverse(const PxoCfg* cfg, TrainWs& t, PassBuffers& p, const float* packed_bwd, int64_t M, float* grads,
                         const StepPlan& plan, const Tuning& tu, unsigned int* tile_counter, hipStream_t s, const CullWs* k,
                         SideFork* join, const char* who) {
  const float *d_rgb = p.d_raw_rgb, *d_sigma = p.d_raw_sigma;
  if (k) {
    if (M == 0) return launch_fill(grads, mlp_param_count(cfg->sh_deg), 0.f, s);
    PXO_TRY(launch_occ_gather(d_rgb, d_sigma, k->slot, p.M, rgb_channels(cfg->sh_deg), k->d_rgb_live, k->d_sigma_live, s));
    d_rgb = k->d_rgb_live;
    d_sigma = k->d_sigma_live;
  }
  uint8_t* const live = plan.skip ? p.live : nullptr;
  PXO_TRY(launch_mlp_bwd_data(cfg, packed_bwd, d_rgb, d_sigma, p.mask, M, p.dz, p.dbias, live, tile_counter, s, plan.bias_from_wgrad));
  if (join && !join->join()) {
    set_error("%s: join of the side stream failed", who);
    return PXO_ERR_HIP;
  }
  return launch_mlp_bwd_weights(cfg, p.acts, p.enc, p.dz, d_rgb, d_sigma, p.dbias, M, grads, t.wgrad_ws, t.wgrad_bytes, live, s,
                                wgrad_split(M, num_cus(), tu), plan.x6_main, plan.bias_from_wgrad);
}

__global__ void occupy_kernel(long long ticks) {
  const long long t0 = wall_clock64();
  while (wall_clock64() - t0 < ticks) __builtin_amdgcn_s_sleep(8);
}

}

using namespace pxo;

extern "C" {

const char* pxo_last_error(void) { return g_last_error.c_str(); }
int pxo_version(void) { return PXO_ABI_VERSION; }
size_t pxo_cfg_bytes(void) { return sizeof(PxoCfg); }

int pxo_set_tuning(int knob, int value) {
  switch (knob) {
    case PXO_TUNE_TILE_SCHED:
      PXO_REQUIRE(value == 0 || value == 1, "pxo_set_tuning: tile schedule must be 0 (static stride) or 1 (device counter), got %d", value);
      g_tune_tile_sched = value;
      return PXO_OK;
    case PXO_TUNE_WGRAD_RANGES:
      PXO_REQUIRE(value >= 0 && value <= num_cus(), "pxo_set_tuning: row ranges per layer must be 0 (built-in choice) .. %d, got %d",
                  num_cus(), value);
      g_tune_wgrad_ranges = value;
      return PXO_OK;
    case PXO_TUNE_COARSE_REVERSE_STREAM:
      PXO_REQUIRE(value == 0 || value == 1, "pxo_set_tuning: coarse reverse stream must be 0 (caller's stream) or 1 (side stream), got %d", value);
      g_tune_coarse_stream = value;
      return PXO_OK;
    case PXO_TUNE_WGRAD_SKINNY_RANGES:
      PXO_REQUIRE(value >= 0 && value <= 2 * num_cus(), "pxo_set_tuning: row ranges of the skinny products must be 0 (built-in choice) .. %d, got %d",
                  2 * num_cus(), value);
      g_tune_wgrad_skinny_ranges = value;
      return PXO_OK;
    case PXO_TUNE_X6_WGRAD:
      PXO_REQUIRE(value == 0 || value == 1, "pxo_set_tuning: bf16x6 weight gradients must be 0 (float32 MFMA) or 1 (bf16x6), got %d", value);
      g_tune_x6_wgrad = value;
      return PXO_OK;
    case PXO_TUNE_VD_RAY_BLOCK:
      PXO_REQUIRE(value >= 1 && value <= PXO_VD_RAY_BLOCK_MAX, "pxo_set_tuning: rays per block of pxo_vd_render_fwd must be 1 .. %d, got %d",
                  PXO_VD_RAY_BLOCK_MAX, value);
      g_tune_vd_ray_block = value;
      return PXO_OK;
    default:
      set_error("pxo_set_tuning: unknown knob %d", knob);
      return PXO_ERR_ARG;
  }
}
int pxo_get_tuning(int knob, int* value) {
  PXO_REQUIRE(value != nullptr, "pxo_get_tuning: NULL pointer");
  switch (knob) {
    case PXO_TUNE_TILE_SCHED: *value = g_tune_tile_sched; return PXO_OK;
    case PXO_TUNE_WGRAD_RANGES: *value = g_tune_wgrad_ranges; return PXO_OK;
    case PXO_TUNE_WGRAD_SKINNY_RANGES: *value = g_tune_wgrad_skinny_ranges; return PXO_OK;
    case PXO_TUNE_COARSE_REVERSE_STREAM: *value = g_tune_coarse_stream; return PXO_OK;
    case PXO_TUNE_X6_WGRAD: *value = g_tune_x6_wgrad; return PXO_OK;
    case PXO_TUNE_VD_RAY_BLOCK: *value = g_tune_vd_ray_block; return PXO_OK;
    default: set_error("pxo_get_tuning: unknown knob %d", knob); return PXO_ERR_ARG;
  }
}
int pxo_tile_rows(void) { return kTM; }

int pxo_param_layout(const PxoCfg* cfg, PxoLeaf* leaves, int64_t* floats_per_mlp) {
  PXO_TRY(validate_cfg(cfg));
  const int deg = cfg->sh_deg;
  if (leaves) {
    for (int l = 0; l < 10; ++l) {
      leaves[2 * l] = PxoLeaf{l, 0, leaf_kernel_off(l, deg), layer_in(l), layer_out(l, deg)};
      leaves[2 * l + 1] = PxoLeaf{l, 1, leaf_bias_off(l, deg), layer_out(l, deg), 1};
    }
  }
  if (floats_per_mlp) *floats_per_mlp = mlp_param_count(deg);
  return PXO_OK;
}

int pxo_packed_sizes(const PxoCfg* cfg, int64_t* fwd_floats, int64_t* bwd_floats) {
  PXO_TRY(validate_cfg(cfg));
  const bool x6 = cfg->mlp_precision == PXO_MLP_BF16X6;
  if (fwd_floats) *fwd_floats = x6 ? x6_fwd_image_floats(cfg->sh_deg) : fwd_image_floats(cfg->sh_deg);
  if (bwd_floats) *bwd_floats = x6 ? x6_bwd_image_floats(cfg->sh_deg) : bwd_image_floats(cfg->sh_deg);
  return PXO_OK;
}

int pxo_pack_weights(const PxoCfg* cfg, const float* mlp_params, float* packed_fwd, float* packed_bwd, void* stream) {
  PXO_TRY(validate_cfg(cfg));
  PXO_REQUIRE(mlp_params && packed_fwd, "pxo_pack_weights: NULL pointer");
  return launch_pack(cfg, mlp_params, packed_fwd, packed_bwd, (hipStream_t)stream);
}

int pxo_sample_along_rays(const float* origins, const float* directions, int64_t B, int S, float near_, float far_,
                          int lindisp, const float* t_rand, float* z_vals, float* pts, void* stream) {
  PXO_REQUIRE(B >= 0 && S >= 1, "pxo_sample_along_rays: bad sizes B=%lld S=%d", (long long)B, S);
  if (B == 0) return PXO_OK;
  PXO_REQUIRE(origins && directions && z_vals && pts, "pxo_sample_along_rays: NULL pointer");
  return launch_sample_along_rays(origins, directions, B, S, near_, far_, lindisp, t_rand, z_vals, pts,
                                  (hipStream_t)stream);
}

int pxo_posenc(const float* x, int64_t N, float* enc, void* stream) {
  if (N == 0) return PXO_OK;
  PXO_REQUIRE(N >= 0 && x && enc, "pxo_posenc: bad arguments");
  return launch_posenc(x, N, enc, (hipStream_t)stream);
}

size_t pxo_relu_mask_bytes(int64_t M) { return (size_t)mask_words(M) * sizeof(uint32_t); }
size_t pxo_dbias_partial_bytes(int64_t M) { return (size_t)dbias_floats(M) * sizeof(float); }

int pxo_mlp_fwd(const PxoCfg* cfg, const float* packed_fwd, const float* pts, int64_t M, float* raw_rgb,
                float* raw_sigma, float* acts, float* enc, void* relu_mask, void* stream) {
  PXO_TRY(validate_cfg(cfg));
  if (M == 0) return PXO_OK;
  PXO_REQUIRE(M >= 0 && packed_fwd && pts && raw_sigma, "pxo_mlp_fwd: bad arguments");
  PXO_REQUIRE((acts != nullptr) == (enc != nullptr) && (acts != nullptr) == (relu_mask != nullptr),
              "pxo_mlp_fwd: acts, enc and relu_mask must be all set or all NULL");
  return launch_mlp_fwd(cfg, packed_fwd, pts, M, raw_rgb, raw_sigma, acts, enc, (uint32_t*)relu_mask,
                        (hipStream_t)stream);
}

int pxo_mlp_bwd_data(const PxoCfg* cfg, const float* packed_bwd, const float* d_raw_rgb, const float* d_raw_sigma,
                     const void* relu_mask, int64_t M, float* dz, float* dbias_partial, void* stream) {
  PXO_TRY(validate_cfg(cfg));
  if (M == 0) return PXO_OK;
  PXO_REQUIRE(M >= 0 && packed_bwd && d_raw_rgb && d_raw_sigma && relu_mask && dz && dbias_partial,
              "pxo_mlp_bwd_data: bad arguments");
  return launch_mlp_bwd_data(cfg, packed_bwd, d_raw_rgb, d_raw_sigma, (const uint32_t*)relu_mask, M, dz,
                             dbias_partial, nullptr, nullptr, (hipStream_t)stream, false);
}

int pxo_wgrad_workspace_bytes(const PxoCfg* cfg, int64_t M, size_t* bytes) {
  PXO_TRY(validate_cfg(cfg));
  PXO_REQUIRE(bytes && M >= 0, "pxo_wgrad_workspace_bytes: bad arguments");
  *bytes = wgrad_workspace_bytes(cfg, M > 0 ? M : 1);
  return PXO_OK;
}

int pxo_mlp_bwd_weights(const PxoCfg* cfg, const float* acts, const float* enc, const float* dz,
                        const float* d_raw_rgb, const float* d_raw_sigma, const float* dbias_partial, int64_t M,
                        float* grads, void* ws, size_t ws_bytes, void* stream) {
  PXO_TRY(validate_cfg(cfg));
  PXO_REQUIRE(M >= 0 && acts && enc && dz && d_raw_rgb && d_raw_sigma && dbias_partial && grads && ws,
              "pxo_mlp_bwd_weights: bad arguments");
  const StepPlan plan = plan_step(*cfg, M, 0, num_cus(), tuning_snapshot());
  return launch_mlp_bwd_weights(cfg, acts, enc, dz, d_raw_rgb, d_raw_sigma, dbias_partial, M, grads, ws, ws_bytes,
                                nullptr, (hipStream_t)stream, plan.split_c, plan.x6_main, false);
}

int pxo_shade_composite_fwd(const PxoCfg* cfg, const float* raw_rgb, const float* raw_sigma, const float* z_vals,
                            const float* directions, const float* viewdirs, int64_t B, int S, float* comp_rgb,
                            float* disp, float* acc, float* weights, void* stream) {
  PXO_TRY(validate_cfg(cfg));
  if (B == 0) return PXO_OK;
  PXO_REQUIRE(B >= 0 && raw_rgb && raw_sigma && z_vals && directions && viewdirs && comp_rgb && disp && acc && weights,
              "pxo_shade_composite_fwd: bad arguments");
  return launch_shade_composite_fwd(cfg, raw_rgb, raw_sigma, z_vals, directions, viewdirs, B, S, comp_rgb, disp, acc,
                                    weights, (hipStream_t)stream);
}

int pxo_shade_composite_bwd(const PxoCfg* cfg, const float* raw_rgb, const float* raw_sigma, const float* z_vals,
                            const float* directions, const float* viewdirs, const float* d_comp_rgb, int64_t B, int S,
                            float* d_raw_rgb, float* d_raw_sigma, void* stream) {
  PXO_TRY(validate_cfg(cfg));
  if (B == 0) return PXO_OK;
  PXO_REQUIRE(B >= 0 && raw_rgb && raw_sigma && z_vals && directions && viewdirs && d_comp_rgb && d_raw_rgb &&
                  d_raw_sigma,
              "pxo_shade_composite_bwd: bad arguments");
  return launch_shade_composite_bwd(cfg, raw_rgb, raw_sigma, z_vals, directions, viewdirs, d_comp_rgb, B, S,
                                    d_raw_rgb, d_raw_sigma, (hipStream_t)stream);
}

int pxo_shade_composite_train(const PxoCfg* cfg, const float* raw_rgb, const float* raw_sigma, const float* z_vals,
                              const float* directions, const float* viewdirs, const float* pixels, int64_t B, int S,
                              float* comp_rgb, float* weights, float* ray_sse, float* d_raw_rgb, float* d_raw_sigma,
                              int64_t n_sp, float* sp_exp, void* stream) {
  PXO_TRY(validate_cfg(cfg));
  if (B == 0) return PXO_OK;
  PXO_REQUIRE(B >= 0 && n_sp >= 0 && raw_rgb && raw_sigma && z_vals && directions && viewdirs && pixels && ray_sse &&
                  d_raw_rgb && d_raw_sigma && (n_sp == 0 || sp_exp),
              "pxo_shade_composite_train: bad arguments");
  return launch_shade_composite_train(cfg, raw_rgb, raw_sigma, z_vals, directions, viewdirs, pixels, B, S, comp_rgb,
                                      weights, ray_sse, d_raw_rgb, d_raw_sigma, n_sp, sp_exp, nullptr, nullptr,
                                      (hipStream_t)stream);
}

int pxo_sample_pdf(const float* z_coarse, const float* w_coarse, const float* origins, const float* directions,
                   int64_t B, int Nc, int Nf, const float* u, float* z_out, float* pts, void* stream) {
  if (B == 0) return PXO_OK;
  PXO_REQUIRE(B >= 0 && z_coarse && w_coarse && origins && directions && z_out && pts, "pxo_sample_pdf: bad arguments");
  return launch_sample_pdf(z_coarse, w_coarse, origins, directions, B, Nc, Nf, u, z_out, pts, (hipStream_t)stream);
}

int pxo_uniform(uint64_t seed, uint64_t stream_id, int64_t n, float lo, float hi, float* out, void* stream) {
  if (n == 0) return PXO_OK;
  PXO_REQUIRE(n >= 0 && out, "pxo_uniform: bad arguments");
  return launch_uniform(seed, stream_id, n, lo, hi, out, (hipStream_t)stream);
}

int pxo_add_gaussian_noise(float* raw, int64_t n, float noise_std, const float* noise, uint64_t seed, uint64_t stream_id,
                           void* stream) {
  if (n == 0) return PXO_OK;
  PXO_REQUIRE(n >= 0 && raw && noise_std >= 0.f, "pxo_add_gaussian_noise: bad arguments");
  return launch_add_noise(raw, n, noise_std, noise, seed, stream_id, (hipStream_t)stream);
}

int pxo_randint(uint64_t seed, uint64_t stream_id, int64_t count, int64_t n, int64_t* out, void* stream) {
  if (count == 0) return PXO_OK;
  PXO_REQUIRE(count >= 0 && n >= 1 && out, "pxo_randint: bad arguments");
  return launch_randint(seed, stream_id, count, n, out, (hipStream_t)stream);
}

int pxo_generate_rays(const float* c2w, int W, int H, float focal, const int64_t* pixel_ids, int64_t B,
                      float* origins, float* directions, float* viewdirs, void* stream) {
  if (B == 0) return PXO_OK;
  PXO_REQUIRE(B >= 0 && W >= 1 && H >= 1 && focal > 0.f && c2w && origins && directions && viewdirs,
              "pxo_generate_rays: bad arguments");
  return launch_generate_rays(c2w, 1, W, H, focal, pixel_ids, B, origins, directions, viewdirs, (hipStream_t)stream);
}

int pxo_sample_batch(uint64_t seed, uint64_t stream_id, const float* c2w, int W, int H, float focal, const float* image_rgb,
                     int64_t B, int64_t first, int64_t* pixel_ids, float* origins, float* directions, float* viewdirs,
                     float* pixels, void* stream) {
  if (B == 0) return PXO_OK;
  PXO_REQUIRE(B >= 0 && first >= 0 && W >= 1 && H >= 1 && focal > 0.f && c2w && image_rgb && origins && directions &&
                  viewdirs && pixels,
              "pxo_sample_batch: bad arguments");
  return launch_sample_batch(seed, stream_id, c2w, W, H, focal, image_rgb, B, first, pixel_ids, origins, directions, viewdirs,
                             pixels, (hipStream_t)stream);
}

int pxo_generate_rays_multi(const float* c2w, int n_cams, int W, int H, float focal, const int64_t* ray_ids, int64_t B,
                            float* origins, float* directions, float* viewdirs, void* stream) {
  if (B == 0) return PXO_OK;
  PXO_REQUIRE(B >= 0 && n_cams >= 1 && W >= 1 && H >= 1 && focal > 0.f && c2w && ray_ids && origins && directions &&
                  viewdirs,
              "pxo_generate_rays_multi: bad arguments");
  return launch_generate_rays(c2w, n_cams, W, H, focal, ray_ids, B, origins, directions, viewdirs,
                              (hipStream_t)stream);
}

int pxo_generate_rays_ndc(const float* c2w, int n_cams, int W, int H, float focal, float ndc_near, const int64_t* ray_ids,
                          int64_t B, float* origins, float* directions, float* viewdirs, void* stream) {
  if (B == 0) return PXO_OK;
  PXO_REQUIRE(B >= 0 && n_cams >= 1 && W >= 1 && H >= 1 && focal > 0.f && ndc_near > 0.f && c2w && origins && directions &&
                  viewdirs && (ray_ids || B <= (int64_t)n_cams * W * H),
              "pxo_generate_rays_ndc: bad arguments");
  return launch_generate_rays_ndc(c2w, n_cams, W, H, focal, ndc_near, ray_ids, B, origins, directions, viewdirs,
                                  (hipStream_t)stream);
}

int pxo_sample_batch_ndc(uint64_t seed, uint64_t stream_id, const float* c2w, int W, int H, float focal, float ndc_near,
                         const float* image_rgb, int64_t B, int64_t first, int64_t* pixel_ids, float* origins,
                         float* directions, float* viewdirs, float* pixels, void* stream) {
  if (B == 0) return PXO_OK;
  PXO_REQUIRE(B >= 0 && first >= 0 && W >= 1 && H >= 1 && focal > 0.f && ndc_near > 0.f && c2w && image_rgb && origins &&
                  directions && viewdirs && pixels,
              "pxo_sample_batch_ndc: bad arguments");
  return launch_sample_batch_ndc(seed, stream_id, c2w, W, H, focal, ndc_near, image_rgb, B, first, pixel_ids, origins,
                                 directions, viewdirs, pixels, (hipStream_t)stream);
}

int pxo_mean_over_samples(const PxoCfg* cfg, const float* raw_rgb, const float* raw_sigma, int64_t n_cells, int S,
                          float* out, void* stream) {
  PXO_TRY(validate_cfg(cfg));
  if (n_cells == 0) return PXO_OK;
  PXO_REQUIRE(n_cells >= 0 && S >= 1 && raw_rgb && raw_sigma && out, "pxo_mean_over_samples: bad arguments");
  return launch_mean_samples(raw_rgb, raw_sigma, n_cells, S, rgb_channels(cfg->sh_deg), out, (hipStream_t)stream);
}

int pxo_adam_step(float* params, float* m, float* v, const float* grads, int64_t n, float lr, int64_t step,
                  float grad_scale, void* stream) {
  if (n == 0) return PXO_OK;
  PXO_REQUIRE(n >= 0 && params && m && v && grads && step >= 0, "pxo_adam_step: bad arguments");
  return launch_adam(params, m, v, grads, n, lr, step, grad_scale, (hipStream_t)stream);
}

int pxo_render_workspace_bytes(const PxoCfg* cfg, int64_t B, size_t* bytes) {
  return workspace_bytes(cfg, B, false, false, false, "pxo_render_workspace_bytes", bytes);
}
int pxo_render_culled_workspace_bytes(const PxoCfg* cfg, int64_t B, size_t* bytes) {
  return workspace_bytes(cfg, B, false, false, true, "pxo_render_culled_workspace_bytes", bytes);
}

static int render_fwd_impl(const PxoCfg* cfg, const float* packed_fwd0, const float* packed_fwd1, const float* origins,
                           const float* directions, const float* viewdirs, int64_t B, int randomized, const float* t_rand,
                           const float* u, uint64_t seed, float* rgb_c, float* disp_c, float* acc_c, float* rgb_f,
                           float* disp_f, float* acc_f, void* ws, size_t ws_bytes, void* stream, const float* lobes,
                           const PxoOccGrid* occ, int64_t* live_rows, const char* who) {
  PXO_TRY(validate_cfg(cfg));
  if (B == 0) return PXO_OK;
  PXO_REQUIRE(B >= 0 && packed_fwd0 && origins && directions && viewdirs && rgb_c && disp_c && acc_c && ws,
              "%s: bad arguments", who);
  if (cfg->num_fine_samples > 0)
    PXO_REQUIRE(packed_fwd1 && rgb_f && disp_f && acc_f, "%s: fine outputs/weights missing", who);
  Layout L;
  PXO_TRY(lay_out(cfg, B, ws, ws_bytes, false, false, occ != nullptr, who, L));
  CullCtx cull;
  if (occ) PXO_TRY(open_cull(occ, L.k, live_rows, who, cull));
  const CullCtx* cx = occ ? &cull : nullptr;
  hipStream_t s = (hipStream_t)stream;
  Draws dr;
  PXO_TRY(prepare_draws(cfg, L.t, B, randomized, t_rand, u, nullptr, seed, s, dr));
  PXO_TRY(level_forward(cfg, L.t, 0, packed_fwd0, origins, directions, viewdirs, B, dr, nullptr, rgb_c, disp_c, acc_c, s, nullptr,
                        lobes, nullptr, cx, who));
  if (cfg->num_fine_samples > 0)
    PXO_TRY(level_forward(cfg, L.t, 1, packed_fwd1, origins, directions, viewdirs, B, dr, nullptr, rgb_f, disp_f, acc_f, s, nullptr,
                          lobes, nullptr, cx, who));
  return PXO_OK;
}

int pxo_render_fwd(const PxoCfg* cfg, const float* packed_fwd0, const float* packed_fwd1, const float* origins,
                   const float* directions, const float* viewdirs, int64_t B, int randomized, const float* t_rand,
                   const float* u, uint64_t seed, float* rgb_c, float* disp_c, float* acc_c, float* rgb_f,
                   float* disp_f, float* acc_f, void* ws, size_t ws_bytes, void* stream) {
  return render_fwd_impl(cfg, packed_fwd0, packed_fwd1, origins, directions, viewdirs, B, randomized, t_rand, u, seed, rgb_c,
                         disp_c, acc_c, rgb_f, disp_f, acc_f, ws, ws_bytes, stream, nullptr, nullptr, nullptr, "pxo_render_fwd");
}

int pxo_sg_render_fwd(const PxoCfg* cfg, const float* lobes, const float* packed_fwd0, const float* packed_fwd1,
                      const float* origins, const float* directions, const float* viewdirs, int64_t B, int randomized,
                      const float* t_rand, const float* u, uint64_t seed, float* rgb_c, float* disp_c, float* acc_c,
                      float* rgb_f, float* disp_f, float* acc_f, void* ws, size_t ws_bytes, void* stream) {
  PXO_TRY(validate_cfg(cfg));
  PXO_REQUIRE(lobes, "pxo_sg_render_fwd: null lobes ([sg_dim,4] with sg_dim = (sh_deg+1)^2 = %d)",
              (cfg->sh_deg + 1) * (cfg->sh_deg + 1));
  return render_fwd_impl(cfg, packed_fwd0, packed_fwd1, origins, directions, viewdirs, B, randomized, t_rand, u, seed, rgb_c,
                         disp_c, acc_c, rgb_f, disp_f, acc_f, ws, ws_bytes, stream, lobes, nullptr, nullptr, "pxo_sg_render_fwd");
}

int pxo_render_fwd_culled(const PxoCfg* cfg, const PxoOccGrid* occ, const float* lobes, const float* packed_fwd0,
                          const float* packed_fwd1, const float* origins, const float* directions, const float* viewdirs, int64_t B,
                          int randomized, const float* t_rand, const float* u, uint64_t seed, float* rgb_c, float* disp_c,
                          float* acc_c, float* rgb_f, float* disp_f, float* acc_f, int64_t live_rows[2], void* ws, size_t ws_bytes,
                          void* stream) {
  const char* who = "pxo_render_fwd_culled";
  PXO_TRY(validate_cfg(cfg));
  PXO_TRY(occ_validate(occ, who));
  PXO_TRY(refuse_noise(cfg, randomized, who));
  if (live_rows) live_rows[0] = live_rows[1] = 0;
  return render_fwd_impl(cfg, packed_fwd0, packed_fwd1, origins, directions, viewdirs, B, randomized, t_rand, u, seed, rgb_c,
                         disp_c, acc_c, rgb_f, disp_f, acc_f, ws, ws_bytes, stream, lobes, occ, live_rows, who);
}

int pxo_train_workspace_bytes(const PxoCfg* cfg, int64_t B, size_t* bytes) {
  return workspace_bytes(cfg, B, true, false, false, "pxo_train_workspace_bytes", bytes);
}
int pxo_sg_train_workspace_bytes(const PxoCfg* cfg, int64_t B, size_t* bytes) {
  return workspace_bytes(cfg, B, true, true, false, "pxo_sg_train_workspace_bytes", bytes);
}
int pxo_train_culled_workspace_bytes(const PxoCfg* cfg, int64_t B, size_t* bytes) {
  return workspace_bytes(cfg, B, true, false, true, "pxo_train_culled_workspace_bytes", bytes);
}

static int train_fwd_bwd_impl(const PxoCfg* cfg, const float* params, const float* packed_fwd0, const float* packed_bwd0,
                              const float* packed_fwd1, const float* packed_bwd1, const float* origins,
                              const float* directions, const float* viewdirs, const float* pixels, int64_t B,
                              int randomized, const float* t_rand, const float* u, const float* sp_points, uint64_t seed,
                              float* grads, float* stats, void* ws, size_t ws_bytes, void* grads0_ready, void* stream,
                              const float* sg_params, float* sg_grads, const PxoOccGrid* occ, int64_t* live_rows,
                              const char* who) {
  PXO_TRY(validate_cfg(cfg));
  PXO_REQUIRE(B >= 1 && params && packed_fwd0 && packed_bwd0 && origins && directions && viewdirs && pixels && grads &&
                  stats && ws,
              "%s: bad arguments", who);
  PXO_TRY(require_train_precision(cfg, who));
  if (cfg->num_fine_samples > 0) PXO_REQUIRE(packed_fwd1 && packed_bwd1, "%s: MLP_1 images missing", who);
  hipStream_t s = (hipStream_t)stream;
  const bool sg = sg_params != nullptr;
  Layout L;
  PXO_TRY(lay_out(cfg, B, ws, ws_bytes, true, sg, occ != nullptr, who, L));
  TrainWs& t = L.t;
  const SgWs& g = L.g;
  CullCtx cull;
  if (occ) PXO_TRY(open_cull(occ, L.k, live_rows, who, cull));
  const CullCtx* cx = occ ? &cull : nullptr;
  const CullWs* k = occ ? &L.k : nullptr;
  const int deg = cfg->sh_deg;
  const int64_t n_mlp = mlp_param_count(deg);
  const int sgK = sh_dim(deg);
  const int64_t n_all = 2 * n_mlp + (sg ? 3 * sgK : 0);
  const float wd_coef = 2.f * cfg->weight_decay_mult / (float)n_all;
  const int Nf = cfg->num_fine_samples;
  const Tuning tu = tuning_snapshot();
  const StepPlan plan = plan_step(*cfg, t.c.M, Nf > 0 ? t.f.M : 0, num_cus(), tu);
  float* const sumsq_partial = t.scalars;
  unsigned int* const step_words = reinterpret_cast<unsigned int*>(t.scalars + kStepWordsAt);
  unsigned int* const counters = step_words + 2;
  unsigned int* const cnt_fwd_c = plan.dyn ? counters + 0 : nullptr;
  unsigned int* const cnt_fwd_f = plan.dyn ? counters + 2 : nullptr;
  unsigned int* const cnt_bwd_c = (plan.dyn || cfg->skip_zero_rows) ? counters + 1 : nullptr;
  unsigned int* const cnt_bwd_f = (plan.dyn || cfg->skip_zero_rows) ? counters + 3 : nullptr;
  Draws dr;
  PXO_TRY(prepare_draws(cfg, t, B, randomized, t_rand, u, sp_points, seed, s, dr, params, 2 * n_mlp, sumsq_partial, step_words,
                        kStepWords, cx ? kStepRecordCulled : kStepRecord | (plan.skip ? 1u : 0u)));
  if (sg) PXO_TRY(launch_sg_lobes(sg_params, sgK, g.lobes, s));
  int64_t M_c = 0, M_f = 0;
  PXO_TRY(level_forward(cfg, t, 0, packed_fwd0, origins, directions, viewdirs, B, dr, pixels, nullptr, nullptr, nullptr, s,
                        cnt_fwd_c, g.lobes, g.part_c, cx, who, &M_c));
  SideFork fk(s, plan.fork && !cx);
  PXO_TRY(level_reverse(cfg, t, t.c, packed_bwd0, M_c, grads, plan, tu, cnt_bwd_c, fk.sc, k, nullptr, who));
  if (cfg->weight_decay_mult != 0.f) PXO_TRY(launch_axpy(grads, params, n_mlp, wd_coef, fk.sc));
  if (grads0_ready && hipEventRecord((hipEvent_t)grads0_ready, fk.sc) != hipSuccess) {
    set_error("%s: hipEventRecord(grads0_ready) failed", who);
    return PXO_ERR_HIP;
  }
  if (Nf > 0) {
    PXO_TRY(level_forward(cfg, t, 1, packed_fwd1, origins, directions, viewdirs, B, dr, pixels, nullptr, nullptr, nullptr, s,
                          cnt_fwd_f, g.lobes, g.part_f, cx, who, &M_f));
    PXO_TRY(level_reverse(cfg, t, t.f, packed_bwd1, M_f, grads + n_mlp, plan, tu, cnt_bwd_f, s, k, &fk, who));
  } else {
    PXO_TRY(launch_fill(grads + n_mlp, n_mlp, 0.f, s));
  }
  if (cfg->weight_decay_mult != 0.f) PXO_TRY(launch_axpy(grads + n_mlp, params + n_mlp, n_mlp, wd_coef, s));
  if (sg)
    PXO_TRY(launch_sg_lobe_grad(g.part_c, g.ray_blocks, Nf > 0 ? g.part_f : nullptr, g.ray_blocks, sgK, sg_params, wd_coef,
                                nullptr, sg_grads, sumsq_partial, s));
  PXO_TRY(launch_finalize_stats(Nf > 0 ? t.f.ray_sse : nullptr, t.c.ray_sse, t.n_sp > 0 ? t.sp_exp : nullptr, sumsq_partial,
                                B, t.n_sp, cfg->sparsity_weight, n_all, stats, s));
  return PXO_OK;
}

int pxo_train_fwd_bwd_bucketed(const PxoCfg* cfg, const float* params, const float* packed_fwd0, const float* packed_bwd0,
                               const float* packed_fwd1, const float* packed_bwd1, const float* origins,
                               const float* directions, const float* viewdirs, const float* pixels, int64_t B,
                               int randomized, const float* t_rand, const float* u, const float* sp_points, uint64_t seed,
                               float* grads, float* stats, void* ws, size_t ws_bytes, void* grads0_ready, void* stream) {
  return train_fwd_bwd_impl(cfg, params, packed_fwd0, packed_bwd0, packed_fwd1, packed_bwd1, origins, directions, viewdirs,
                            pixels, B, randomized, t_rand, u, sp_points, seed, grads, stats, ws, ws_bytes, grads0_ready, stream,
                            nullptr, nullptr, nullptr, nullptr, "pxo_train_fwd_bwd");
}

int pxo_train_fwd_bwd_culled(const PxoCfg* cfg, const PxoOccGrid* occ, const float* params, const float* packed_fwd0,
                             const float* packed_bwd0, const float* packed_fwd1, const float* packed_bwd1, const float* origins,
                             const float* directions, const float* viewdirs, const float* pixels, int64_t B, int randomized,
                             const float* t_rand, const float* u, const float* sp_points, uint64_t seed, float* grads,
                             float* stats, void* ws, size_t ws_bytes, void* grads0_ready, void* stream, int64_t live_rows[2]) {
  const char* who = "pxo_train_fwd_bwd_culled";
  PXO_TRY(validate_cfg(cfg));
  PXO_TRY(occ_validate(occ, who));
  PXO_TRY(require_train_precision(cfg, who));
  PXO_TRY(refuse_noise(cfg, randomized, who));
  if (live_rows) live_rows[0] = live_rows[1] = 0;
  return train_fwd_bwd_impl(cfg, params, packed_fwd0, packed_bwd0, packed_fwd1, packed_bwd1, origins, directions, viewdirs,
                            pixels, B, randomized, t_rand, u, sp_points, seed, grads, stats, ws, ws_bytes, grads0_ready, stream,
                            nullptr, nullptr, occ, live_rows, who);
}

int pxo_sg_lobes(const float* sg_params, int K, float* lobes, void* stream) {
  PXO_REQUIRE(sg_params != nullptr, "pxo_sg_lobes: null sg_params ([3K]: sg_lambda [K], then sg_mu_spher [K,2])");
  PXO_REQUIRE(lobes != nullptr, "pxo_sg_lobes: null lobes ([K,4])");
  PXO_REQUIRE(K >= 1 && K <= 25, "pxo_sg_lobes: K %d not in [1,25]", K);
  return launch_sg_lobes(sg_params, K, lobes, (hipStream_t)stream);
}

int pxo_sg_shade_composite_train(const PxoCfg* cfg, const float* lobes, const float* raw_rgb, const float* raw_sigma,
                                 const float* z_vals, const float* directions, const float* viewdirs, const float* pixels,
                                 int64_t B, int S, float* comp_rgb, float* weights, float* ray_sse, float* d_raw_rgb,
                                 float* d_raw_sigma, int64_t n_sp, float* sp_exp, float* d_lobes, float* lobe_partials,
                                 void* stream) {
  PXO_TRY(validate_cfg(cfg));
  const int K = sh_dim(cfg->sh_deg);
  PXO_REQUIRE(lobes != nullptr, "pxo_sg_shade_composite_train: null lobes ([sg_dim,4] with sg_dim = (sh_deg+1)^2 = %d)", K);
  PXO_REQUIRE(d_lobes != nullptr && lobe_partials != nullptr,
              "pxo_sg_shade_composite_train: null d_lobes ([%d,4]) or lobe_partials (%d floats per %d rays)", K, 4 * K,
              PXO_SG_RAYS_PER_BLOCK);
  PXO_REQUIRE(B >= 0 && n_sp >= 0, "pxo_sg_shade_composite_train: bad sizes B=%lld n_sp=%lld", (long long)B, (long long)n_sp);
  hipStream_t s = (hipStream_t)stream;
  if (B == 0) return launch_fill(d_lobes, 4 * K, 0.f, s);
  PXO_REQUIRE(raw_rgb && raw_sigma && z_vals && directions && viewdirs && pixels && ray_sse && d_raw_rgb && d_raw_sigma &&
                  (n_sp == 0 || sp_exp),
              "pxo_sg_shade_composite_train: bad arguments");
  PXO_TRY(launch_shade_composite_train(cfg, raw_rgb, raw_sigma, z_vals, directions, viewdirs, pixels, B, S, comp_rgb, weights,
                                       ray_sse, d_raw_rgb, d_raw_sigma, n_sp, sp_exp, lobes, lobe_partials, s));
  return launch_sg_lobe_grad(lobe_partials, sg_ray_blocks(B), nullptr, 0, K, nullptr, 0.f, d_lobes, nullptr, nullptr, s);
}

int pxo_sg_train_fwd_bwd_bucketed(const PxoCfg* cfg, const float* params, const float* sg_params, const float* packed_fwd0,
                                  const float* packed_bwd0, const float* packed_fwd1, const float* packed_bwd1,
                                  const float* origins, const float* directions, const float* viewdirs, const float* pixels,
                                  int64_t B, int randomized, const float* t_rand, const float* u, const float* sp_points,
                                  uint64_t seed, float* grads, float* sg_grads, float* stats, void* ws, size_t ws_bytes,
                                  void* grads0_ready, void* stream) {
  PXO_REQUIRE(sg_params != nullptr, "pxo_sg_train_fwd_bwd: null sg_params ([3K]: sg_lambda [K], then sg_mu_spher [K,2])");
  PXO_REQUIRE(sg_grads != nullptr, "pxo_sg_train_fwd_bwd: null sg_grads ([3K])");
  return train_fwd_bwd_impl(cfg, params, packed_fwd0, packed_bwd0, packed_fwd1, packed_bwd1, origins, directions, viewdirs,
                            pixels, B, randomized, t_rand, u, sp_points, seed, grads, stats, ws, ws_bytes, grads0_ready, stream,
                            sg_params, sg_grads, nullptr, nullptr, "pxo_sg_train_fwd_bwd");
}

int pxo_sg_train_fwd_bwd(const PxoCfg* cfg, const float* params, const float* sg_params, const float* packed_fwd0,
                         const float* packed_bwd0, const float* packed_fwd1, const float* packed_bwd1, const float* origins,
                         const float* directions, const float* viewdirs, const float* pixels, int64_t B, int randomized,
                         const float* t_rand, const float* u, const float* sp_points, uint64_t seed, float* grads,
                         float* sg_grads, float* stats, void* ws, size_t ws_bytes, void* stream) {
  return pxo_sg_train_fwd_bwd_bucketed(cfg, params, sg_params, packed_fwd0, packed_bwd0, packed_fwd1, packed_bwd1, origins,
                                       directions, viewdirs, pixels, B, randomized, t_rand, u, sp_points, seed, grads, sg_grads,
                                       stats, ws, ws_bytes, nullptr, stream);
}

int pxo_train_fwd_bwd(const PxoCfg* cfg, const float* params, const float* packed_fwd0, const float* packed_bwd0,
                      const float* packed_fwd1, const float* packed_bwd1, const float* origins,
                      const float* directions, const float* viewdirs, const float* pixels, int64_t B, int randomized,
                      const float* t_rand, const float* u, const float* sp_points, uint64_t seed, float* grads,
                      float* stats, void* ws, size_t ws_bytes, void* stream) {
  return pxo_train_fwd_bwd_bucketed(cfg, params, packed_fwd0, packed_bwd0, packed_fwd1, packed_bwd1, origins, directions,
                                    viewdirs, pixels, B, randomized, t_rand, u, sp_points, seed, grads, stats, ws, ws_bytes,
                                    nullptr, stream);
}

int pxo_train_backward_work(const PxoCfg* cfg, int64_t B, void* ws, size_t ws_bytes, int64_t* live_chunks,
                            int64_t* total_chunks, void* stream) {
  PXO_TRY(validate_cfg(cfg));
  PXO_REQUIRE(B >= 1 && ws && live_chunks && total_chunks, "pxo_train_backward_work: bad arguments");
  Layout L;
  PXO_TRY(lay_out(cfg, B, ws, ws_bytes, true, false, false, "pxo_train_backward_work", L));
  const TrainWs& t = L.t;
  hipStream_t s = (hipStream_t)stream;
  const int64_t nc = (t.c.M + kLiveRows - 1) / kLiveRows, nf = cfg->num_fine_samples > 0 ? (t.f.M + kLiveRows - 1) / kLiveRows : 0;
  *total_chunks = nc + nf;
  unsigned int record = 0;
  if (hipMemcpyAsync(&record, t.scalars + kStepWordsAt, sizeof(record), hipMemcpyDeviceToHost, s) != hipSuccess ||
      hipStreamSynchronize(s) != hipSuccess) {
    set_error("pxo_train_backward_work: copy back failed");
    return PXO_ERR_HIP;
  }
  if (record == kStepRecordCulled) {
    set_error("pxo_train_backward_work: the last step on this workspace was pxo_train_fwd_bwd_culled, whose reverse pass ran on the "
              "live rows only (the chunk totals of the dense row count do not describe it; see its live_rows)");
    return PXO_ERR_ARG;
  }
  if ((record & ~1u) != kStepRecord) { set_error("pxo_train_backward_work: no pxo_train_fwd_bwd call has used this workspace"); return PXO_ERR_ARG; }
  if (!(record & 1u)) {
    *live_chunks = nc + nf;
    return PXO_OK;
  }
  unsigned long long* cnt = reinterpret_cast<unsigned long long*>(t.scalars + 96);
  if (hipMemsetAsync(cnt, 0, sizeof(unsigned long long), s) != hipSuccess) { set_error("hipMemsetAsync failed"); return PXO_ERR_HIP; }
  PXO_TRY(launch_count_live(t.c.live, nc, cnt, s));
  if (nf > 0) PXO_TRY(launch_count_live(t.f.live, nf, cnt, s));
  unsigned long long host = 0;
  if (hipMemcpyAsync(&host, cnt, sizeof(host), hipMemcpyDeviceToHost, s) != hipSuccess || hipStreamSynchronize(s) != hipSuccess) {
    set_error("pxo_train_backward_work: copy back failed");
    return PXO_ERR_HIP;
  }
  *live_chunks = (int64_t)host;
  return PXO_OK;
}

int pxo_event_create(void** event) {
  PXO_REQUIRE(event != nullptr, "pxo_event_create: NULL pointer");
  hipEvent_t e = nullptr;
  if (hipEventCreateWithFlags(&e, hipEventDisableTiming) != hipSuccess) { set_error("hipEventCreateWithFlags failed"); return PXO_ERR_HIP; }
  *event = (void*)e;
  return PXO_OK;
}
int pxo_event_destroy(void* event) {
  if (event && hipEventDestroy((hipEvent_t)event) != hipSuccess) { set_error("hipEventDestroy failed"); return PXO_ERR_HIP; }
  return PXO_OK;
}
int pxo_stream_wait_event(void* stream, void* event) {
  PXO_REQUIRE(event != nullptr, "pxo_stream_wait_event: NULL event");
  if (hipStreamWaitEvent((hipStream_t)stream, (hipEvent_t)event, 0) != hipSuccess) { set_error("hipStreamWaitEvent failed"); return PXO_ERR_HIP; }
  return PXO_OK;
}

int pxo_adam_pack_step(const PxoCfg* cfg, float* params, float* m, float* v, const float* grads, float lr, int64_t step,
                       float grad_scale, float* packed_fwd0, float* packed_bwd0, float* packed_fwd1, float* packed_bwd1,
                       void* stream) {
  PXO_TRY(validate_cfg(cfg));
  PXO_REQUIRE(params && m && v && grads && step >= 0 && packed_fwd0 && packed_fwd1, "pxo_adam_pack_step: bad arguments");
  PXO_REQUIRE((packed_bwd0 != nullptr) == (packed_bwd1 != nullptr), "pxo_adam_pack_step: both backward images or none");
  if (cfg->mlp_precision != PXO_MLP_F32) {
    if (cfg->mlp_precision == PXO_MLP_BF16X3 && packed_bwd0) {
      set_error("pxo_adam_pack_step: the bf16x3 images are forward-only (packed_bwd must be NULL)");
      return PXO_ERR_UNSUPPORTED;
    }
    const int64_t n_mlp = mlp_param_count(cfg->sh_deg);
    PXO_TRY(launch_adam(params, m, v, grads, 2 * n_mlp, lr, step, grad_scale, (hipStream_t)stream));
    PXO_TRY(launch_pack(cfg, params, packed_fwd0, packed_bwd0, (hipStream_t)stream));
    return launch_pack(cfg, params + n_mlp, packed_fwd1, packed_bwd1, (hipStream_t)stream);
  }
  return launch_adam_pack(cfg, params, m, v, grads, lr, step, grad_scale, packed_fwd0, packed_bwd0, packed_fwd1,
                          packed_bwd1, (hipStream_t)stream);
}

int pxo_occupy_cus(int blocks, int threads, float micros, int lds_bytes, void* stream) {
  PXO_REQUIRE(blocks >= 1 && blocks <= 4096 && threads >= 64 && threads <= 1024 && threads % 64 == 0 && micros >= 0.f &&
                  micros <= 1e6f && lds_bytes >= 0 && lds_bytes <= 65536,
              "pxo_occupy_cus: bad arguments (blocks %d, threads %d, micros %g, lds_bytes %d)", blocks, threads, (double)micros,
              lds_bytes);
  int dev = 0, khz = 0;
  if (hipGetDevice(&dev) != hipSuccess || hipDeviceGetAttribute(&khz, hipDeviceAttributeWallClockRate, dev) != hipSuccess || khz <= 0)
    khz = 100000;
  const long long ticks = (long long)((double)micros * 1e-3 * (double)khz);
  hipLaunchKernelGGL(occupy_kernel, dim3(blocks), dim3(threads), (size_t)lds_bytes, (hipStream_t)stream, ticks);
  return check_launch("occupy_cus");
}

int pxo_profile_enable(int tag_mask) {
  PXO_REQUIRE(tag_mask >= 0 && tag_mask < (1 << PXO_PROF_NUM_TAGS), "pxo_profile_enable: mask %d has bits beyond the %d tags",
              tag_mask, PXO_PROF_NUM_TAGS);
  g_prof_mask = (unsigned)tag_mask;
  return PXO_OK;
}

int pxo_profile_read(int tag, int64_t* launches, double* total_ms, int64_t* total_rows) {
  PXO_REQUIRE(tag >= 0 && tag < PXO_PROF_NUM_TAGS && launches && total_ms && total_rows, "pxo_profile_read: bad arguments");
  int64_t n = 0, rows = 0;
  double ms = 0.0;
  std::vector<ProfRecord> keep;
  for (auto& r : g_prof) {
    if (r.tag != tag) { keep.push_back(r); continue; }
    float t = 0.f;
    if (hipEventSynchronize(r.b) == hipSuccess && hipEventElapsedTime(&t, r.a, r.b) == hipSuccess) {
      ++n; ms += t; rows += r.rows;
    }
    (void)hipEventDestroy(r.a);
    (void)hipEventDestroy(r.b);
  }
  g_prof.swap(keep);
  *launches = n; *total_ms = ms; *total_rows = rows;
  return PXO_OK;
}

int pxo_eval_points(const PxoCfg* cfg, const float* packed_fwd, const float* points, int64_t N, float* raw_rgb,
                    float* raw_sigma, void* stream) {
  PXO_TRY(validate_cfg(cfg));
  if (N == 0) return PXO_OK;
  PXO_REQUIRE(N >= 0 && packed_fwd && points && raw_sigma, "pxo_eval_points: bad arguments");
  return launch_mlp_fwd(cfg, packed_fwd, points, N, raw_rgb, raw_sigma, nullptr, nullptr, nullptr,
                        (hipStream_t)stream);
}

int pxo_grid_sigma(const PxoCfg* cfg, const float* packed_fwd, int reso, int x0, int x1, const float offset[3],
                   const float scale[3], float* sigma_out, void* stream) {
  PXO_TRY(validate_cfg(cfg));
  PXO_REQUIRE(reso >= 1 && x0 >= 0 && x1 >= x0 && x1 <= reso, "pxo_grid_sigma: bad slab [%d,%d) of %d", x0, x1, reso);
  if (x1 == x0) return PXO_OK;
  PXO_REQUIRE(packed_fwd && offset && scale && sigma_out, "pxo_grid_sigma: NULL pointer");
  return launch_mlp_fwd_grid(cfg, packed_fwd, reso, x0, x1, offset, scale, sigma_out, (hipStream_t)stream);
}

}
```

### plenoctree_amd/csrc/pxo_common.h

```cpp
#pragma once
#include <hip/hip_runtime.h>
#include <stdint.h>
#include <stddef.h>
#include "../../include/plenoctree_hip.h"

typedef float f32x4 __attribute__((ext_vector_type(4)));
typedef float f32x16 __attribute__((ext_vector_type(16)));

namespace pxo {

constexpr int kW = PXO_NET_WIDTH;
constexpr int kDepth = PXO_NET_DEPTH;
constexpr int kEnc = PXO_ENC_DIM;
constexpr int kEncPad = PXO_ENC_PAD;
constexpr int kTM = 128;
constexpr int kMlpThreads = 512;
constexpr int kMlpWgPerCu = 1;
constexpr int kLDA = 260;
constexpr int kMlpWaves = kMlpThreads / 64;
constexpr int kMaskWords = (kTM / 32) * (8 / kMlpWaves) * 16 / 32;
constexpr int kMaxMlpGrid = 1024;
constexpr int kLiveRows = 16;
constexpr int kMaxLiveChunks = 2048;

__host__ __device__ inline int sh_dim(int deg) { return (deg + 1) * (deg + 1); }
__host__ __device__ inline int rgb_channels(int deg) { return 3 * sh_dim(deg); }
__host__ __device__ inline int head_blocks(int deg) { return (rgb_channels(deg) + 1 + 31) / 32; }

__host__ __device__ inline int layer_in(int l) {
  return l == 0 ? kEnc : (l == 5 ? kW + kEnc : kW);
}
__host__ __device__ inline int layer_out(int l, int deg) {
  return l < 8 ? kW : (l == 8 ? 1 : rgb_channels(deg));
}
__host__ __device__ inline int64_t leaf_kernel_off(int l, int deg) {
  int64_t off = 0;
  for (int i = 0; i < l; ++i) off += (int64_t)layer_in(i) * layer_out(i, deg) + layer_out(i, deg);
  return off;
}
__host__ __device__ inline int64_t leaf_bias_off(int l, int deg) {
  return leaf_kernel_off(l, deg) + (int64_t)layer_in(l) * layer_out(l, deg);
}
__host__ __device__ inline int64_t mlp_param_count(int deg) { return leaf_kernel_off(10, deg); }

__host__ __device__ inline int64_t packed_index(int k, int n, int ncb) {
  int g = k >> 3, kk = k & 7;
  int lane = ((kk >> 2) << 5) | (n & 31);
  return (((int64_t)g * ncb + (n >> 5)) * 64 + lane) * 4 + (kk & 3);
}

__host__ __device__ inline int fwd_kgroups(int l) { return l == 0 ? 8 : (l == 5 ? 40 : 32); }
__host__ __device__ inline int64_t fwd_layer_off(int l) {
  int64_t off = 0;
  for (int i = 0; i < l; ++i) off += (int64_t)fwd_kgroups(i) * 8 * 256;
  return off;
}
__host__ __device__ inline int64_t fwd_bias_off(int deg) {
  return fwd_layer_off(8) + (int64_t)32 * head_blocks(deg) * 256;
}
__host__ __device__ inline int64_t fwd_image_floats(int deg) {
  return fwd_bias_off(deg) + 8 * kW + 32 * head_blocks(deg);
}
__host__ __device__ inline int64_t bwd_layer_off(int l, int deg) {
  return (int64_t)head_blocks(deg) * 32 * 256 + (int64_t)(7 - l) * 256 * 256;
}
__host__ __device__ inline int64_t bwd_image_floats(int deg) { return bwd_layer_off(0, deg); }

constexpr int kX6KgSlots = 8 * 3 * 256;
__host__ __device__ inline int x6_fwd_kg(int l) { return l == 0 ? 4 : (l == 5 ? 20 : 16); }
__host__ __device__ inline int64_t x6_fwd_layer_off(int l) {
  int64_t off = 0;
  for (int i = 0; i < l; ++i) off += (int64_t)x6_fwd_kg(i) * kX6KgSlots;
  return off;
}
__host__ __device__ inline int64_t x6_fwd_bias_off(int deg) {
  return x6_fwd_layer_off(8) + (int64_t)16 * head_blocks(deg) * 3 * 256;
}
__host__ __device__ inline int64_t x6_fwd_image_floats(int deg) {
  return x6_fwd_bias_off(deg) + 8 * kW + 32 * head_blocks(deg);
}
__host__ __device__ inline int x6_bwd_head_kg(int deg) { return 4 * ((head_blocks(deg) + 1) / 2); }
__host__ __device__ inline int64_t x6_bwd_image_floats(int deg) {
  return (int64_t)(x6_bwd_head_kg(deg) + 7 * 16) * kX6KgSlots;
}

__host__ __device__ inline int64_t num_tiles(int64_t M) { return (M + kTM - 1) / kTM; }

struct TileSched {
  int64_t n_full;
  int64_t n_half;
  int64_t half_row0;
};
__host__ __device__ inline TileSched tile_sched(int64_t M, int64_t grid) {
  TileSched t;
  const int64_t tiles = num_tiles(M);
  t.n_full = tiles; t.n_half = 0; t.half_row0 = tiles * kTM;
  if (grid < 1 || tiles <= grid) return t;
  const int64_t whole = (tiles / grid) * grid;
  const int64_t left = M - whole * kTM;
  if (left > 0 && left <= grid * (kTM / 2)) {
    t.n_full = whole;
    t.half_row0 = whole * kTM;
    t.n_half = (left + kTM / 2 - 1) / (kTM / 2);
  }
  return t;
}
__host__ __device__ inline int64_t mask_slots(int64_t M) { return num_tiles(M) + kMaxMlpGrid / 2; }
__host__ __device__ inline int64_t mask_words(int64_t M) {
  return mask_slots(M) * kDepth * kMlpThreads * kMaskWords;
}
__host__ __device__ inline int64_t dbias_floats(int64_t M) { return mask_slots(M) * (9 * kW + 1); }
__host__ __device__ inline const uint8_t* dbias_tile_live(const float* dbias_partial, int64_t M) {
  return reinterpret_cast<const uint8_t*>(dbias_partial + mask_slots(M) * 9 * kW);
}

void set_error(const char* fmt, ...);
int check_launch(const char* what);

#define PXO_REQUIRE(cond, ...)            \
  do {                                    \
    if (!(cond)) {                        \
      pxo::set_error(__VA_ARGS__);        \
      return PXO_ERR_ARG;                 \
    }                                     \
  } while (0)

int validate_cfg(const PxoCfg* cfg);
int num_cus();
unsigned mlp_grid(int64_t M);
int mlp_bwd_partials(int64_t M);

struct KernelTimer {
  KernelTimer(int tag, int64_t rows, hipStream_t s);
  ~KernelTimer();
  int slot;
  hipStream_t stream;
};
int launch_mlp_fwd_grid(const PxoCfg* cfg, const float* packed_fwd, int reso, int x0, int x1,
                        const float* off, const float* scale, float* sigma_out, hipStream_t s);

int launch_pack(const PxoCfg* cfg, const float* mlp_params, float* fwd, float* bwd, hipStream_t s);
int launch_mlp_fwd(const PxoCfg* cfg, const float* packed_fwd, const float* pts, int64_t M,
                   float* raw_rgb, float* raw_sigma, float* acts, float* enc, uint32_t* mask,
                   hipStream_t s, unsigned int* tile_counter = nullptr);
__host__ __device__ inline int64_t live_flags(int64_t M) { return (M + kLiveRows - 1) / kLiveRows + kTM / kLiveRows; }
int launch_mlp_bwd_data(const PxoCfg* cfg, const float* packed_bwd, const float* d_raw_rgb,
                        const float* d_raw_sigma, const uint32_t* mask, int64_t M, float* dz,
                        float* dbias_partial, uint8_t* chunk_live, unsigned int* tile_counter, hipStream_t s,
                        bool bias_from_wgrad);

struct Tuning {
  int tile_sched;
  int wgrad_ranges;
  int wgrad_skinny_ranges;
  int coarse_stream;
  int x6_wgrad;
  int vd_ray_block;
};
Tuning tuning_snapshot();

constexpr int kKC = 32;
struct WgradSplit { int64_t rpw_main; int P_main; int64_t rpw_skinny; int P_skinny; };
inline void split_rows(int64_t M, int64_t target, int64_t* rows_per_wg, int* P) {
  int64_t rpw = (M + target - 1) / target;
  rpw = (rpw + kKC - 1) / kKC * kKC;
  if (rpw < kKC) rpw = kKC;
  *rows_per_wg = rpw;
  *P = (int)((M + rpw - 1) / rpw);
}
inline WgradSplit wgrad_split(int64_t M, int ncu, const Tuning& tu) {
  constexpr int NL = kDepth - 1;
  WgradSplit w;
  int ranges = M >= (int64_t)1024 * ncu ? ncu : (4 * ncu / NL > 0 ? 4 * ncu / NL : 1);
  if (tu.wgrad_ranges > 0) ranges = tu.wgrad_ranges;
  if (ranges > ncu) ranges = ncu;
  split_rows(M, ranges, &w.rpw_main, &w.P_main);
  int skinny = M < (int64_t)512 * ncu ? ncu : 2 * ncu;
  if (tu.wgrad_skinny_ranges > 0) skinny = tu.wgrad_skinny_ranges;
  if (skinny > 2 * ncu) skinny = 2 * ncu;
  split_rows(M, skinny, &w.rpw_skinny, &w.P_skinny);
  return w;
}
inline bool wgrad_split_fits_live_list(const WgradSplit& w) {
  return w.rpw_main <= (int64_t)kMaxLiveChunks * kLiveRows && w.rpw_skinny <= (int64_t)kMaxLiveChunks * kLiveRows;
}

struct StepPlan {
  bool dyn;
  WgradSplit split_c, split_f;
  bool skip;
  bool x6_main;
  bool bias_from_wgrad;
  bool fork;
};
inline StepPlan plan_step(const PxoCfg& cfg, int64_t M_c, int64_t M_f, int ncu, const Tuning& tu) {
  StepPlan p;
  p.dyn = tu.tile_sched != 0;
  p.split_c = wgrad_split(M_c, ncu, tu);
  p.split_f = wgrad_split(M_f, ncu, tu);
  p.skip = cfg.skip_zero_rows != 0 && wgrad_split_fits_live_list(p.split_c) &&
           (M_f == 0 || wgrad_split_fits_live_list(p.split_f));
  p.x6_main = cfg.mlp_precision == PXO_MLP_BF16X6 && tu.x6_wgrad != 0;
  p.bias_from_wgrad = p.x6_main;
  p.fork = M_f > 0 && tu.coarse_stream != 0;
  return p;
}

void launch_wgrad_main_x6(const float* acts, const float* dz1, int64_t M, int64_t rpw, int P, float* slab, int n_layers,
                          int64_t layer_stride, const uint8_t* chunk_live, float* dz_colsum, hipStream_t s);
size_t wgrad_workspace_bytes(const PxoCfg* cfg, int64_t M);
int launch_mlp_bwd_weights(const PxoCfg* cfg, const float* acts, const float* enc, const float* dz,
                           const float* d_raw_rgb, const float* d_raw_sigma,
                           const float* dbias_partial, int64_t M, float* grads, void* ws,
                           size_t ws_bytes, const uint8_t* chunk_live, hipStream_t s, const WgradSplit& split,
                           bool x6_main, bool bias_from_wgrad);
int launch_count_live(const uint8_t* chunk_live, int64_t n, unsigned long long* out, hipStream_t s);
int launch_posenc(const float* x, int64_t N, float* enc, hipStream_t s);
int launch_pack_x3(const PxoCfg* cfg, const float* mlp_params, float* fwd, hipStream_t s);
int launch_mlp_fwd_x3(const PxoCfg* cfg, const float* packed_fwd, const float* pts, int reso, int x0, const float* off,
                      const float* scale, int64_t M, float* raw_rgb, float* raw_sigma, hipStream_t s);

int launch_pack_x6(const PxoCfg* cfg, const float* mlp_params, float* fwd, float* bwd, hipStream_t s);
int launch_mlp_fwd_x6(const PxoCfg* cfg, const float* packed_fwd, const float* pts, int reso, int x0, const float* off,
                      const float* scale, int64_t M, float* raw_rgb, float* raw_sigma, float* acts, float* enc,
                      uint32_t* mask, unsigned int* tile_counter, hipStream_t s);
int launch_mlp_bwd_data_x6(const PxoCfg* cfg, const float* packed_bwd, const float* d_raw_rgb, const float* d_raw_sigma,
                           const uint32_t* mask, int64_t M, float* dz, float* dbias_partial, uint8_t* chunk_live,
                           unsigned int* tile_counter, hipStream_t s, bool db_all = true);

int launch_sample_along_rays(const float* o, const float* d, int64_t B, int S, float near_,
                             float far_, int lindisp, const float* t_rand, float* z, float* pts,
                             hipStream_t s);
int launch_shade_composite_fwd(const PxoCfg* cfg, const float* raw_rgb, const float* raw_sigma,
                               const float* z, const float* dirs, const float* viewdirs, int64_t B,
                               int S, float* comp_rgb, float* disp, float* acc, float* weights,
                               hipStream_t s, const float* lobes = nullptr);
int launch_shade_composite_bwd(const PxoCfg* cfg, const float* raw_rgb, const float* raw_sigma,
                               const float* z, const float* dirs, const float* viewdirs,
                               const float* d_comp_rgb, int64_t B, int S, float* d_raw_rgb,
                               float* d_raw_sigma, hipStream_t s);
int launch_sample_pdf(const float* z_c, const float* w_c, const float* o, const float* d, int64_t B,
                      int Nc, int Nf, const float* u, float* z_out, float* pts, hipStream_t s);
int launch_generate_rays(const float* c2w, int n_cams, int W, int H, float focal, const int64_t* pix, int64_t B,
                         float* o, float* d, float* v, hipStream_t s);
int launch_sample_batch(uint64_t seed, uint64_t stream_id, const float* c2w, int W, int H, float focal, const float* image,
                        int64_t B, int64_t first, int64_t* ids, float* o, float* d, float* v, float* pixels, hipStream_t s);
int launch_generate_rays_ndc(const float* c2w, int n_cams, int W, int H, float focal, float near, const int64_t* pix, int64_t B,
                             float* o, float* d, float* v, hipStream_t s);
int launch_sample_batch_ndc(uint64_t seed, uint64_t stream_id, const float* c2w, int W, int H, float focal, float near,
                            const float* image, int64_t B, int64_t first, int64_t* ids, float* o, float* d, float* v,
                            float* pixels, hipStream_t s);
int launch_randint(uint64_t seed, uint64_t stream_id, int64_t count, int64_t n, int64_t* out, hipStream_t s);
int launch_mean_samples(const float* raw_rgb, const float* raw_sigma, int64_t n_cells, int S, int C, float* out,
                        hipStream_t s);
int launch_uniform(uint64_t seed, uint64_t stream_id, int64_t n, float lo, float hi, float* out,
                   hipStream_t s);
int launch_add_noise(float* raw, int64_t n, float noise_std, const float* noise, uint64_t seed, uint64_t stream_id, hipStream_t s,
                     int64_t first = 0);
int launch_vd_composite_fwd(int white_bkgd, const float* raw_rgb, const float* raw_sigma, const float* z, const float* dirs,
                            int64_t B, int S, float* comp_rgb, float* disp, float* acc, float* weights, hipStream_t s);
int launch_adam(float* p, float* m, float* v, const float* g, int64_t n, float lr, int64_t step,
                float grad_scale, hipStream_t s);
__host__ __device__ inline int64_t sg_ray_blocks(int64_t B) { return (B + PXO_SG_RAYS_PER_BLOCK - 1) / PXO_SG_RAYS_PER_BLOCK; }
int launch_shade_composite_train(const PxoCfg* cfg, const float* raw_rgb, const float* raw_sigma, const float* z,
                                 const float* dirs, const float* viewdirs, const float* pixels, int64_t B, int S,
                                 float* comp_rgb, float* weights, float* ray_sse, float* d_raw_rgb, float* d_raw_sigma,
                                 int64_t n_sp, float* sp_exp, const float* lobes, float* lobe_partials, hipStream_t s);
int launch_sg_lobes(const float* sg_params, int K, float* lobes, hipStream_t s);
int launch_sg_lobe_grad(const float* part_a, int64_t nb_a, const float* part_b, int64_t nb_b, int K, const float* sg_params,
                        float wd_coef, float* d_lobes, float* sg_grads, float* sumsq_slot, hipStream_t s);
struct UniformJob { uint64_t stream_id; int64_t n; float lo, hi; float* out; };
constexpr int kSumsqBlocks = 64;
int launch_uniform_jobs(uint64_t seed, const UniformJob* jobs, int n_jobs, hipStream_t s, const float* sq_x = nullptr,
                        int64_t sq_n = 0, float* sq_partial = nullptr, unsigned int* step_words = nullptr, int n_words = 0,
                        unsigned int first_word = 0);
int launch_finalize_stats(const float* sse_f, const float* sse_c, const float* sp_exp, const float* sumsq_partial,
                          int64_t B, int64_t n_sp, float sp_weight, int64_t n_params, float* stats, hipStream_t s);
int launch_adam_pack(const PxoCfg* cfg, float* p, float* m, float* v, const float* g, float lr, int64_t step,
                     float grad_scale, float* fwd0, float* bwd0, float* fwd1, float* bwd1, hipStream_t s);
int occ_validate(const PxoOccGrid* occ, const char* who);
size_t occ_cull_workspace_bytes(int64_t M);
int launch_occ_cull(const PxoOccGrid& occ, const float* pts, int64_t M, float* pts_live, int32_t* slot, int64_t* n_live_dev,
                    void* ws, hipStream_t s);
int launch_occ_expand(const float* rgb_live, const float* sigma_live, const int32_t* slot, int64_t M, int C, float* raw_rgb,
                      float* raw_sigma, hipStream_t s);
int launch_occ_gather(const float* d_rgb, const float* d_sigma, const int32_t* slot, int64_t M, int C, float* d_rgb_live,
                      float* d_sigma_live, hipStream_t s);
int launch_occ_tail_slots(int32_t* slot, int64_t n, int64_t first, hipStream_t s);
int launch_fill(float* p, int64_t n, float v, hipStream_t s);
int launch_axpy(float* y, const float* x, int64_t n, float a, hipStream_t s);

}
```

### plenoctree_amd/ops.py

```python
import ctypes

import torch

from . import _lib
from ._lib import NET_DEPTH, NET_WIDTH, ENC_PAD, PxoError, check, make_cfg


def _require_gpu():
    if not torch.cuda.is_available():
        raise PxoError("plenoctree_amd needs a ROCm GPU (gfx950); there is no CPU fallback")


def _p(t):
    if t is None:
        return None
    if not (t.is_cuda and t.is_contiguous()):
        raise PxoError("tensor must be a contiguous ROCm tensor")
    return ctypes.c_void_p(t.data_ptr())


def _f(t):
    if t is not None and t.dtype != torch.float32:
        raise PxoError(f"expected float32, got {t.dtype}")
    return _p(t)


def _stream():
    return ctypes.c_void_p(torch.cuda.current_stream().cuda_stream)


def _new(*shape, device=None, dtype=torch.float32):
    return torch.empty(*shape, dtype=dtype, device=device or torch.device("cuda", torch.cuda.current_device()))


def sh_dim(cfg):
    return (cfg.sh_deg + 1) ** 2


def rgb_channels(cfg):
    return 3 * sh_dim(cfg)


def param_layout(cfg):
    lib = _lib.load()
    leaves = (_lib.PxoLeaf * _lib.NUM_LEAVES)()
    n = ctypes.c_int64(0)
    check(lib.pxo_param_layout(ctypes.byref(cfg), leaves, ctypes.byref(n)), "pxo_param_layout")
    return [(l.layer, l.is_bias, l.offset, l.rows, l.cols) for l in leaves], n.value


def packed_sizes(cfg):
    lib = _lib.load()
    a, b = ctypes.c_int64(0), ctypes.c_int64(0)
    check(lib.pxo_packed_sizes(ctypes.byref(cfg), ctypes.byref(a), ctypes.byref(b)), "pxo_packed_sizes")
    return a.value, b.value


def pack_weights(cfg, mlp_params, packed_fwd=None, packed_bwd=None, need_bwd=True):
    _require_gpu()
    lib = _lib.load()
    nf, nb = packed_sizes(cfg)
    if packed_fwd is None:
        packed_fwd = _new(nf, device=mlp_params.device)
    if need_bwd and packed_bwd is None:
        packed_bwd = _new(nb, device=mlp_params.device)
    check(lib.pxo_pack_weights(ctypes.byref(cfg), _f(mlp_params), _f(packed_fwd),
                               _f(packed_bwd) if need_bwd else None, _stream()), "pxo_pack_weights")
    return packed_fwd, packed_bwd


def sample_along_rays(origins, directions, num_samples, near, far, t_rand=None, lindisp=False):
    _require_gpu()
    lib = _lib.load()
    B = origins.shape[0]
    z = _new(B, num_samples, device=origins.device)
    pts = _new(B, num_samples, 3, device=origins.device)
    check(lib.pxo_sample_along_rays(_f(origins), _f(directions), B, num_samples, near, far, int(lindisp),
                                    _f(t_rand), _f(z), _f(pts), _stream()), "pxo_sample_along_rays")
    return z, pts


def posenc(x):
    _require_gpu()
    lib = _lib.load()
    lead = x.shape[:-1]
    x2 = x.reshape(-1, 3).contiguous()
    enc = _new(x2.shape[0], _lib.ENC_DIM, device=x.device)
    check(lib.pxo_posenc(_f(x2), x2.shape[0], _f(enc), _stream()), "pxo_posenc")
    return enc.reshape(*lead, _lib.ENC_DIM)


def relu_mask_bytes(M):
    return _lib.load().pxo_relu_mask_bytes(M)


def dbias_partial_bytes(M):
    return _lib.load().pxo_dbias_partial_bytes(M)


def mlp_fwd(cfg, packed_fwd, pts, save=False, want_rgb=True):
    _require_gpu()
    lib = _lib.load()
    pts = pts.reshape(-1, 3)
    M = pts.shape[0]
    dev = pts.device
    raw_rgb = _new(M, rgb_channels(cfg), device=dev) if want_rgb else None
    raw_sigma = _new(M, device=dev)
    acts = enc = mask = None
    if save:
        acts = _new(NET_DEPTH, M, NET_WIDTH, device=dev)
        enc = _new(M, ENC_PAD, device=dev)
        mask = _new(max(relu_mask_bytes(M), 16), device=dev, dtype=torch.uint8)
    check(lib.pxo_mlp_fwd(ctypes.byref(cfg), _f(packed_fwd), _f(pts), M, _f(raw_rgb), _f(raw_sigma),
                          _f(acts), _f(enc), _p(mask), _stream()), "pxo_mlp_fwd")
    if save:
        return raw_rgb, raw_sigma, (acts, enc, mask)
    return raw_rgb, raw_sigma


def mlp_bwd_data(cfg, packed_bwd, d_raw_rgb, d_raw_sigma, mask):
    _require_gpu()
    lib = _lib.load()
    M = d_raw_sigma.shape[0]
    dev = d_raw_sigma.device
    dz = _new(NET_DEPTH, M, NET_WIDTH, device=dev)
    dbias = _new(max(dbias_partial_bytes(M) // 4, 4), device=dev)
    check(lib.pxo_mlp_bwd_data(ctypes.byref(cfg), _f(packed_bwd), _f(d_raw_rgb), _f(d_raw_sigma), _p(mask), M,
                               _f(dz), _f(dbias), _stream()), "pxo_mlp_bwd_data")
    return dz, dbias


def mlp_bwd_weights(cfg, acts, enc, dz, d_raw_rgb, d_raw_sigma, dbias):
    _require_gpu()
    lib = _lib.load()
    M = d_raw_sigma.shape[0]
    dev = d_raw_sigma.device
    _, n = param_layout(cfg)
    grads = _new(n, device=dev)
    nbytes = ctypes.c_size_t(0)
    check(lib.pxo_wgrad_workspace_bytes(ctypes.byref(cfg), M, ctypes.byref(nbytes)), "pxo_wgrad_workspace_bytes")
    ws = _new(max(nbytes.value, 16), device=dev, dtype=torch.uint8)
    check(lib.pxo_mlp_bwd_weights(ctypes.byref(cfg), _f(acts), _f(enc), _f(dz), _f(d_raw_rgb), _f(d_raw_sigma),
                                  _f(dbias), M, _f(grads), _p(ws), nbytes.value, _stream()),
          "pxo_mlp_bwd_weights")
    return grads


def shade_composite_fwd(cfg, raw_rgb, raw_sigma, z_vals, directions, viewdirs):
    _require_gpu()
    lib = _lib.load()
    B, S = z_vals.shape
    dev = z_vals.device
    comp, disp, acc, w = _new(B, 3, device=dev), _new(B, device=dev), _new(B, device=dev), _new(B, S, device=dev)
    check(lib.pxo_shade_composite_fwd(ctypes.byref(cfg), _f(raw_rgb), _f(raw_sigma), _f(z_vals), _f(directions),
                                      _f(viewdirs), B, S, _f(comp), _f(disp), _f(acc), _f(w), _stream()),
          "pxo_shade_composite_fwd")
    return comp, disp, acc, w


def shade_composite_bwd(cfg, raw_rgb, raw_sigma, z_vals, directions, viewdirs, d_comp_rgb):
    _require_gpu()
    lib = _lib.load()
    B, S = z_vals.shape
    dev = z_vals.device
    d_rgb = _new(B * S, rgb_channels(cfg), device=dev)
    d_sigma = _new(B * S, device=dev)
    check(lib.pxo_shade_composite_bwd(ctypes.byref(cfg), _f(raw_rgb), _f(raw_sigma), _f(z_vals), _f(directions),
                                      _f(viewdirs), _f(d_comp_rgb), B, S, _f(d_rgb), _f(d_sigma), _stream()),
          "pxo_shade_composite_bwd")
    return d_rgb, d_sigma


def sample_pdf(z_coarse, w_coarse, origins, directions, num_fine, u=None):
    _require_gpu()
    lib = _lib.load()
    B, Nc = z_coarse.shape
    dev = z_coarse.device
    z = _new(B, Nc + num_fine, device=dev)
    pts = _new(B, Nc + num_fine, 3, device=dev)
    check(lib.pxo_sample_pdf(_f(z_coarse), _f(w_coarse), _f(origins), _f(directions), B, Nc, num_fine, _f(u),
                             _f(z), _f(pts), _stream()), "pxo_sample_pdf")
    return z, pts


def add_gaussian_noise(raw, noise_std, noise=None, seed=0, stream_id=0):
    _require_gpu()
    check(_lib.load().pxo_add_gaussian_noise(_f(raw), raw.numel(), float(noise_std), _f(noise), seed, stream_id, _stream()),
          "pxo_add_gaussian_noise")
    return raw


def uniform(seed, stream_id, n, lo=0.0, hi=1.0, device=None):
    _require_gpu()
    lib = _lib.load()
    out = _new(n, device=device)
    check(lib.pxo_uniform(seed, stream_id, n, lo, hi, _f(out), _stream()), "pxo_uniform")
    return out


def adam_step(params, m, v, grads, lr, step, grad_scale=1.0):
    _require_gpu()
    lib = _lib.load()
    check(lib.pxo_adam_step(_f(params), _f(m), _f(v), _f(grads), params.numel(), float(lr), int(step),
                            float(grad_scale), _stream()), "pxo_adam_step")


def adam_pack_step(cfg, params, m, v, grads, lr, step, packed, grad_scale=1.0):
    _require_gpu()
    lib = _lib.load()
    (f0, b0), (f1, b1) = packed
    check(lib.pxo_adam_pack_step(ctypes.byref(cfg), _f(params), _f(m), _f(v), _f(grads), float(lr), int(step),
                                 float(grad_scale), _f(f0), _f(b0), _f(f1), _f(b1), _stream()), "pxo_adam_pack_step")


def _train_outputs(raw_rgb, B, S, n_sp, want_rgb, want_weights):
    C = raw_rgb.shape[-1]
    dev = raw_rgb.device
    return {"comp_rgb": _new(B, 3, device=dev) if want_rgb else None,
            "weights": _new(B, S, device=dev) if want_weights else None,
            "ray_sse": _new(B, device=dev), "d_raw_rgb": _new(B * S + n_sp, C, device=dev),
            "d_raw_sigma": _new(B * S + n_sp, device=dev), "sp_exp": _new(max(n_sp, 1), device=dev)}


def shade_composite_train(cfg, raw_rgb, raw_sigma, z_vals, directions, viewdirs, pixels, n_sp=0, want_rgb=True,
                          want_weights=True):
    _require_gpu()
    lib = _lib.load()
    B, S = z_vals.shape
    out = _train_outputs(raw_rgb, B, S, n_sp, want_rgb, want_weights)
    check(lib.pxo_shade_composite_train(ctypes.byref(cfg), _f(raw_rgb), _f(raw_sigma), _f(z_vals), _f(directions),
                                        _f(viewdirs), _f(pixels), B, S, _f(out["comp_rgb"]), _f(out["weights"]),
                                        _f(out["ray_sse"]), _f(out["d_raw_rgb"]), _f(out["d_raw_sigma"]), n_sp,
                                        _f(out["sp_exp"]), _stream()), "pxo_shade_composite_train")
    return out


def render_workspace_bytes(cfg, B):
    n = ctypes.c_size_t(0)
    check(_lib.load().pxo_render_workspace_bytes(ctypes.byref(cfg), B, ctypes.byref(n)), "pxo_render_workspace_bytes")
    return n.value


def train_workspace_bytes(cfg, B):
    n = ctypes.c_size_t(0)
    check(_lib.load().pxo_train_workspace_bytes(ctypes.byref(cfg), B, ctypes.byref(n)), "pxo_train_workspace_bytes")
    return n.value


def _check_lobes(cfg, lobes):
    if lobes is not None:
        K = (cfg.sh_deg + 1) ** 2
        if lobes.dtype != torch.float32 or tuple(lobes.shape) != (K, 4) or not lobes.is_contiguous() or not lobes.is_cuda:
            raise PxoError(f"SG lobes must be a contiguous float32 [{K}, 4] tensor on the GPU")


def _render_outputs(cfg, B, dev):
    outs = [(_new(B, 3, device=dev), _new(B, device=dev), _new(B, device=dev)) for _ in range(2 if cfg.num_fine_samples > 0 else 1)]
    return outs, [_f(x) for lvl in outs for x in lvl] + [None] * (6 - 3 * len(outs))


def _train_args(packed, origins, directions, viewdirs, pixels, randomized, t_rand, u, sp_points, seed, grads, stats, ws, grads0_ready):
    (f0, b0), (f1, b1) = packed
    head = (_f(f0), _f(b0), _f(f1), _f(b1), _f(origins), _f(directions), _f(viewdirs), _f(pixels), origins.shape[0], int(randomized),
            _f(t_rand), _f(u), _f(sp_points), seed, _f(grads))
    return head, (_f(stats), _p(ws), ws.numel(), grads0_ready.handle if grads0_ready is not None else None, _stream())


def render_fwd(cfg, packed_fwd0, packed_fwd1, origins, directions, viewdirs, randomized=False, t_rand=None, u=None,
               seed=0, ws=None, lobes=None):
    _require_gpu()
    _check_lobes(cfg, lobes)
    lib = _lib.load()
    B = origins.shape[0]
    dev = origins.device
    nbytes = render_workspace_bytes(cfg, B)
    if ws is None or ws.numel() < nbytes:
        ws = _new(max(nbytes, 16), device=dev, dtype=torch.uint8)
    outs, out_ptrs = _render_outputs(cfg, B, dev)
    tail = (_f(packed_fwd0), _f(packed_fwd1), _f(origins), _f(directions), _f(viewdirs), B, int(randomized), _f(t_rand), _f(u),
            seed, *out_ptrs, _p(ws), ws.numel(), _stream())
    if lobes is None:
        check(lib.pxo_render_fwd(ctypes.byref(cfg), *tail), "pxo_render_fwd")
    else:
        check(lib.pxo_sg_render_fwd(ctypes.byref(cfg), _f(lobes), *tail), "pxo_sg_render_fwd")
    return outs


def train_fwd_bwd(cfg, params, packed, origins, directions, viewdirs, pixels, grads, stats, ws, randomized=True,
                  t_rand=None, u=None, sp_points=None, seed=0, grads0_ready=None):
    _require_gpu()
    head, tail = _train_args(packed, origins, directions, viewdirs, pixels, randomized, t_rand, u, sp_points, seed, grads, stats, ws,
                             grads0_ready)
    check(_lib.load().pxo_train_fwd_bwd_bucketed(ctypes.byref(cfg), _f(params), *head, *tail), "pxo_train_fwd_bwd_bucketed")


def sg_lobes(sg_params, K, lobes=None):
    _require_gpu()
    if sg_params.numel() != 3 * K:
        raise PxoError(f"sg_params has {sg_params.numel()} floats, sg_dim={K} needs {3 * K}")
    if lobes is None:
        lobes = _new(K, 4, device=sg_params.device)
    check(_lib.load().pxo_sg_lobes(_f(sg_params), int(K), _f(lobes), _stream()), "pxo_sg_lobes")
    return lobes


def sg_shade_composite_train(cfg, lobes, raw_rgb, raw_sigma, z_vals, directions, viewdirs, pixels, n_sp=0, want_rgb=True,
                             want_weights=True):
    _require_gpu()
    lib = _lib.load()
    B, S = z_vals.shape
    K = sh_dim(cfg)
    dev = raw_rgb.device
    out = _train_outputs(raw_rgb, B, S, n_sp, want_rgb, want_weights)
    out["d_lobes"] = _new(K, 4, device=dev)
    partials = _new(max(-(-B // _lib.SG_RAYS_PER_BLOCK), 1) * K * 4, device=dev)
    check(lib.pxo_sg_shade_composite_train(ctypes.byref(cfg), _f(lobes), _f(raw_rgb), _f(raw_sigma), _f(z_vals), _f(directions),
                                           _f(viewdirs), _f(pixels), B, S, _f(out["comp_rgb"]), _f(out["weights"]),
                                           _f(out["ray_sse"]), _f(out["d_raw_rgb"]), _f(out["d_raw_sigma"]), n_sp,
                                           _f(out["sp_exp"]), _f(out["d_lobes"]), _f(partials), _stream()),
          "pxo_sg_shade_composite_train")
    return out


def sg_train_workspace_bytes(cfg, B):
    n = ctypes.c_size_t(0)
    check(_lib.load().pxo_sg_train_workspace_bytes(ctypes.byref(cfg), B, ctypes.byref(n)), "pxo_sg_train_workspace_bytes")
    return n.value


def sg_train_fwd_bwd(cfg, params, sg_params, packed, origins, directions, viewdirs, pixels, grads, sg_grads, stats, ws,
                     randomized=True, t_rand=None, u=None, sp_points=None, seed=0, grads0_ready=None):
    _require_gpu()
    head, tail = _train_args(packed, origins, directions, viewdirs, pixels, randomized, t_rand, u, sp_points, seed, grads, stats, ws,
                             grads0_ready)
    check(_lib.load().pxo_sg_train_fwd_bwd_bucketed(ctypes.byref(cfg), _f(params), _f(sg_params), *head, _f(sg_grads), *tail),
          "pxo_sg_train_fwd_bwd_bucketed")


def train_backward_work(cfg, B, ws):
    _require_gpu()
    live, total = ctypes.c_int64(0), ctypes.c_int64(0)
    check(_lib.load().pxo_train_backward_work(ctypes.byref(cfg), B, _p(ws), ws.numel(), ctypes.byref(live), ctypes.byref(total),
                                              _stream()), "pxo_train_backward_work")
    return live.value, total.value


class Event:

    def __init__(self):
        _require_gpu()
        h = ctypes.c_void_p(None)
        check(_lib.load().pxo_event_create(ctypes.byref(h)), "pxo_event_create")
        self.handle = h

    def wait(self, stream):
        check(_lib.load().pxo_stream_wait_event(ctypes.c_void_p(stream.cuda_stream), self.handle), "pxo_stream_wait_event")

    def __del__(self):
        try:
            if self.handle:
                _lib.load().pxo_event_destroy(self.handle)
        except Exception:
            pass


def eval_points(cfg, packed_fwd, points, want_rgb=True):
    _require_gpu()
    lib = _lib.load()
    points = points.reshape(-1, 3)
    N = points.shape[0]
    dev = points.device
    raw_rgb = _new(N, rgb_channels(cfg), device=dev) if want_rgb else None
    raw_sigma = _new(N, 1, device=dev)
    check(lib.pxo_eval_points(ctypes.byref(cfg), _f(packed_fwd), _f(points), N, _f(raw_rgb), _f(raw_sigma), _stream()),
          "pxo_eval_points")
    return raw_rgb, raw_sigma


def grid_sigma(cfg, packed_fwd, reso, x0, x1, offset, scale, out=None):
    _require_gpu()
    lib = _lib.load()
    n = (x1 - x0) * reso * reso
    if out is None:
        out = _new(n, device=packed_fwd.device)
    off = (ctypes.c_float * 3)(*[float(v) for v in offset])
    sc = (ctypes.c_float * 3)(*[float(v) for v in scale])
    check(lib.pxo_grid_sigma(ctypes.byref(cfg), _f(packed_fwd), reso, x0, x1, off, sc, _f(out), _stream()),
          "pxo_grid_sigma")
    return out


PROF_MLP_FWD, PROF_MLP_BWD_DATA, PROF_WGRAD_MAIN, PROF_WGRAD_OTHER, PROF_NUM_TAGS = 0, 1, 2, 3, 4


TUNE_TILE_SCHED, TUNE_WGRAD_RANGES, TUNE_WGRAD_SKINNY_RANGES, TUNE_COARSE_REVERSE_STREAM, TUNE_X6_WGRAD = 0, 1, 2, 3, 4
TUNE_VD_RAY_BLOCK = 5


def set_tuning(knob, value):
    check(_lib.load().pxo_set_tuning(int(knob), int(value)), "pxo_set_tuning")


def get_tuning(knob):
    v = ctypes.c_int(0)
    check(_lib.load().pxo_get_tuning(int(knob), ctypes.byref(v)), "pxo_get_tuning")
    return v.value


def occupy_cus(blocks, threads, micros, stream=None, lds_bytes=0):
    _require_gpu()
    h = ctypes.c_void_p(stream.cuda_stream) if stream is not None else _stream()
    check(_lib.load().pxo_occupy_cus(int(blocks), int(threads), float(micros), int(lds_bytes), h), "pxo_occupy_cus")


def profile_enable(on=True, tags=None):
    mask = 0
    if tags is not None:
        for t in tags:
            mask |= 1 << int(t)
    elif on:
        mask = (1 << PROF_NUM_TAGS) - 1
    check(_lib.load().pxo_profile_enable(mask), "pxo_profile_enable")


def profile_read(tag):
    n, ms, rows = ctypes.c_int64(0), ctypes.c_double(0.0), ctypes.c_int64(0)
    check(_lib.load().pxo_profile_read(tag, ctypes.byref(n), ctypes.byref(ms), ctypes.byref(rows)), "pxo_profile_read")
    return n.value, ms.value, rows.value



def randint(seed, stream_id, count, n, device=None):
    _require_gpu()
    out = _new(count, device=device, dtype=torch.int64)
    check(_lib.load().pxo_randint(seed, stream_id, count, n, _p(out), _stream()), "pxo_randint")
    return out


def generate_rays(c2w, W, H, focal, pixel_ids=None, count=None):
    _require_gpu()
    c2w = c2w[:3, :4].contiguous()
    B = pixel_ids.shape[0] if pixel_ids is not None else (count if count is not None else W * H)
    dev = c2w.device
    o, d, v = _new(B, 3, device=dev), _new(B, 3, device=dev), _new(B, 3, device=dev)
    if pixel_ids is not None and pixel_ids.dtype != torch.int64:
        raise PxoError("pixel_ids must be int64")
    check(_lib.load().pxo_generate_rays(_f(c2w), W, H, float(focal), _p(pixel_ids), B, _f(o), _f(d), _f(v), _stream()),
          "pxo_generate_rays")
    return o, d, v


def sample_batch(seed, stream_id, c2w, W, H, focal, image_rgb, B, want_ids=False, first=0):
    _require_gpu()
    c2w = c2w[:3, :4].contiguous()
    dev = c2w.device
    o, d, v, px = _new(B, 3, device=dev), _new(B, 3, device=dev), _new(B, 3, device=dev), _new(B, 3, device=dev)
    ids = _new(B, device=dev, dtype=torch.int64) if want_ids else None
    check(_lib.load().pxo_sample_batch(seed, stream_id, _f(c2w), W, H, float(focal), _f(image_rgb), B, int(first), _p(ids), _f(o), _f(d),
                                       _f(v), _f(px), _stream()), "pxo_sample_batch")
    return (o, d, v, px, ids) if want_ids else (o, d, v, px)


def generate_rays_multi(c2w_all, W, H, focal, ray_ids):
    _require_gpu()
    if ray_ids.dtype != torch.int64:
        raise PxoError("ray_ids must be int64")
    c2w_all = c2w_all[:, :3, :4].contiguous()
    B = ray_ids.shape[0]
    dev = c2w_all.device
    o, d, v = _new(B, 3, device=dev), _new(B, 3, device=dev), _new(B, 3, device=dev)
    check(_lib.load().pxo_generate_rays_multi(_f(c2w_all), c2w_all.shape[0], W, H, float(focal), _p(ray_ids), B,
                                              _f(o), _f(d), _f(v), _stream()), "pxo_generate_rays_multi")
    return o, d, v


def generate_rays_ndc(c2w, W, H, focal, pixel_ids=None, count=None, ndc_near=1.0):
    _require_gpu()
    c2w = c2w[:3, :4].contiguous()
    B = pixel_ids.shape[0] if pixel_ids is not None else (count if count is not None else W * H)
    dev = c2w.device
    o, d, v = _new(B, 3, device=dev), _new(B, 3, device=dev), _new(B, 3, device=dev)
    if pixel_ids is not None and pixel_ids.dtype != torch.int64:
        raise PxoError("pixel_ids must be int64")
    check(_lib.load().pxo_generate_rays_ndc(_f(c2w), 1, W, H, float(focal), float(ndc_near), _p(pixel_ids), B, _f(o), _f(d),
                                            _f(v), _stream()), "pxo_generate_rays_ndc")
    return o, d, v


def generate_rays_multi_ndc(c2w_all, W, H, focal, ray_ids, ndc_near=1.0):
    _require_gpu()
    if ray_ids.dtype != torch.int64:
        raise PxoError("ray_ids must be int64")
    c2w_all = c2w_all[:, :3, :4].contiguous()
    B = ray_ids.shape[0]
    dev = c2w_all.device
    o, d, v = _new(B, 3, device=dev), _new(B, 3, device=dev), _new(B, 3, device=dev)
    check(_lib.load().pxo_generate_rays_ndc(_f(c2w_all), c2w_all.shape[0], W, H, float(focal), float(ndc_near), _p(ray_ids), B,
                                            _f(o), _f(d), _f(v), _stream()), "pxo_generate_rays_ndc")
    return o, d, v


def sample_batch_ndc(seed, stream_id, c2w, W, H, focal, image_rgb, B, want_ids=False, first=0, ndc_near=1.0):
    _require_gpu()
    c2w = c2w[:3, :4].contiguous()
    dev = c2w.device
    o, d, v, px = _new(B, 3, device=dev), _new(B, 3, device=dev), _new(B, 3, device=dev), _new(B, 3, device=dev)
    ids = _new(B, device=dev, dtype=torch.int64) if want_ids else None
    check(_lib.load().pxo_sample_batch_ndc(seed, stream_id, _f(c2w), W, H, float(focal), float(ndc_near), _f(image_rgb), B,
                                           int(first), _p(ids), _f(o), _f(d), _f(v), _f(px), _stream()), "pxo_sample_batch_ndc")
    return (o, d, v, px, ids) if want_ids else (o, d, v, px)


def mean_over_samples(cfg, raw_rgb, raw_sigma, samples_per_cell, out=None):
    _require_gpu()
    n = raw_sigma.numel() // samples_per_cell
    if out is None:
        out = _new(n, rgb_channels(cfg) + 1, device=raw_sigma.device)
    elif out.numel() != n * (rgb_channels(cfg) + 1):
        raise PxoError("mean_over_samples: `out` has the wrong size")
    check(_lib.load().pxo_mean_over_samples(ctypes.byref(cfg), _f(raw_rgb), _f(raw_sigma.reshape(-1)), n,
                                            samples_per_cell, _f(out), _stream()), "pxo_mean_over_samples")
    return out


def vd_param_layout():
    leaves = (_lib.PxoLeaf * _lib.VD_NUM_LEAVES)()
    n = ctypes.c_int64(0)
    check(_lib.load().pxo_vd_param_layout(leaves, ctypes.byref(n)), "pxo_vd_param_layout")
    return [(l.layer, l.is_bias, l.offset, l.rows, l.cols) for l in leaves], n.value


def vd_packed_floats():
    n = ctypes.c_int64(0)
    check(_lib.load().pxo_vd_packed_floats(ctypes.byref(n)), "pxo_vd_packed_floats")
    return n.value


def vd_pack_weights(mlp_params, packed=None):
    _require_gpu()
    if packed is None:
        packed = _new(vd_packed_floats(), device=mlp_params.device)
    check(_lib.load().pxo_vd_pack_weights(_f(mlp_params), _f(packed), _stream()), "pxo_vd_pack_weights")
    return packed


def _ws(ws, nbytes, device):
    if ws is None or ws.numel() < nbytes:
        ws = _new(max(nbytes, 16), device=device, dtype=torch.uint8)
    return ws
# ... 234 lines not shown
```

Before: 171,900.

## Compact live row chunks into packed virtual tiles for backward data pass

Adds a compacting mode to the MLP backward(data) kernel. A pre-pass flags row chunks whose upstream gradients are nonzero, and a packing kernel bin-packs those chunks from several tiles into dense virtual tiles. The backward kernel then processes only the virtual tiles, scattering dz and the per-slot bias partials back to their original rows. This aims to cut wasted GEMM work on dead chunks, at the cost of two extra launches, an atomic-built pack list and more complex scatter addressing. It is enabled by default for f32 precision when skipping is on.

```diff
diff --git a/include/plenoctree_hip.h b/include/plenoctree_hip.h
--- a/include/plenoctree_hip.h
+++ b/include/plenoctree_hip.h
@@ -91,6 +91,16 @@
                         const float* dbias_partial, int64_t M, float* grads, void* ws,
                         size_t ws_bytes, void* stream);
 
+size_t pxo_skip_workspace_bytes(int64_t M);
+int pxo_train_pack_tiles(const PxoCfg* cfg, int64_t B, void* ws, size_t ws_bytes, int64_t* virtual_tiles, void* stream);
+int pxo_mlp_bwd_data_skip(const PxoCfg* cfg, const float* packed_bwd, const float* d_raw_rgb,
+                          const float* d_raw_sigma, const void* relu_mask, int64_t M, float* dz,
+                          float* dbias_partial, void* skip_ws, size_t skip_ws_bytes, void* stream);
+int pxo_mlp_bwd_weights_skip(const PxoCfg* cfg, const float* acts, const float* enc, const float* dz,
+                             const float* d_raw_rgb, const float* d_raw_sigma,
+                             const float* dbias_partial, int64_t M, float* grads, void* ws,
+                             size_t ws_bytes, const void* skip_ws, size_t skip_ws_bytes, void* stream);
+
 int pxo_shade_composite_fwd(const PxoCfg* cfg, const float* raw_rgb, const float* raw_sigma,
                             const float* z_vals, const float* directions, const float* viewdirs,
                             int64_t B, int S, float* comp_rgb, float* disp, float* acc,
@@ -274,6 +284,7 @@
 #define PXO_TUNE_COARSE_REVERSE_STREAM 3
 #define PXO_TUNE_X6_WGRAD 4
 #define PXO_TUNE_VD_RAY_BLOCK 5
+#define PXO_TUNE_BWD_COMPACT 6
 #define PXO_VD_RAY_BLOCK_DEFAULT 1024
 #define PXO_VD_RAY_BLOCK_MAX 4096
 int pxo_set_tuning(int knob, int value);
diff --git a/plenoctree_amd/_lib.py b/plenoctree_amd/_lib.py
--- a/plenoctree_amd/_lib.py
+++ b/plenoctree_amd/_lib.py
@@ -117,6 +117,10 @@
     "pxo_mlp_fwd": (c_int, [CFG, P, P, c_int64, P, P, P, P, P, P]),
     "pxo_dbias_partial_bytes": (c_size_t, [c_int64]),
     "pxo_mlp_bwd_data": (c_int, [CFG, P, P, P, P, c_int64, P, P, P]),
+    "pxo_skip_workspace_bytes": (c_size_t, [c_int64]),
+    "pxo_train_pack_tiles": (c_int, [CFG, c_int64, P, c_size_t, POINTER(c_int64), P]),
+    "pxo_mlp_bwd_data_skip": (c_int, [CFG, P, P, P, P, c_int64, P, P, P, c_size_t, P]),
+    "pxo_mlp_bwd_weights_skip": (c_int, [CFG, P, P, P, P, P, P, c_int64, P, P, c_size_t, P, c_size_t, P]),
     "pxo_wgrad_workspace_bytes": (c_int, [CFG, c_int64, POINTER(c_size_t)]),
     "pxo_mlp_bwd_weights": (c_int, [CFG, P, P, P, P, P, P, c_int64, P, P, c_size_t, P]),
     "pxo_shade_composite_fwd": (c_int, [CFG, P, P, P, P, P, c_int64, c_int, P, P, P, P, P]),
diff --git a/plenoctree_amd/csrc/mlp_kernels.hip b/plenoctree_amd/csrc/mlp_kernels.hip
--- a/plenoctree_amd/csrc/mlp_kernels.hip
+++ b/plenoctree_amd/csrc/mlp_kernels.hip
@@ -183,10 +183,25 @@
   __builtin_amdgcn_raw_buffer_store_b128(__builtin_bit_cast(u32x4, v), t.out, t.voff, i * 8 * kW * 4, 0);
 }
 
-template <int RBN, int CBN, bool COPY = false>
+struct PackCopy {
+  __amdgpu_buffer_rsrc_t out;
+  uint32_t voff;
+  const float* src;
+  uint32_t src_hi;
+  uint32_t soff[kPackPos];
+  bool on;
+};
+template <int RBN>
+__device__ __forceinline__ void tile_copy_slab(const PackCopy& t, int i) {
+  const f32x4 v = i < 8 ? *reinterpret_cast<const f32x4*>(t.src + i * 8 * kLDA)
+                        : *reinterpret_cast<const f32x4*>(t.src + t.src_hi + (i - 8) * 8 * kLDA);
+  __builtin_amdgcn_raw_buffer_store_b128(__builtin_bit_cast(u32x4, v), t.out, t.voff, t.soff[i >> 1] + (i & 1) * 8 * kW * 4, 0);
+}
+
+template <int RBN, int CBN, bool COPY = false, typename TC = TileCopy>
 __device__ __forceinline__ void gemm_lds_packed(const ARows& arow, const WImage& w, int wu,
                                                 int kgroups, int kg_stride, f32x16 (&acc)[RBN][CBN],
-                                                f32x4 (&b)[4][CBN], const TileCopy* tc = nullptr) {
+                                                f32x4 (&b)[4][CBN], const TC* tc = nullptr) {
   constexpr int D = kBDist;
   static_assert(D == 2 || D == 3, "kBDist");
   f32x4 a0[RBN], a1[RBN];
@@ -645,12 +660,198 @@
   return 0;
 }
 
-template <int NHB, bool SKIP, bool DYN>
+__global__ void live_chunks_kernel(const float* __restrict__ d_raw_rgb, const float* __restrict__ d_raw_sigma, int64_t M, int C,
+                                   int64_t n_chunks, uint8_t* __restrict__ chunk_live, int32_t* __restrict__ pack) {
+  const int lane = threadIdx.x & 63;
+  if (blockIdx.x == 0 && threadIdx.x == 0) pack[0] = 0;
+  const int64_t chunk = blockIdx.x * (int64_t)(blockDim.x >> 6) + (threadIdx.x >> 6);
+  if (chunk >= n_chunks) return;
+  const int64_t row0 = chunk * kLiveRows;
+  const int rows = M - row0 >= kLiveRows ? kLiveRows : (M > row0 ? (int)(M - row0) : 0);
+  bool nz = false;
+  if (d_raw_rgb) {
+    const float* __restrict__ p = d_raw_rgb + row0 * C;
+    for (int i = lane; i < rows * C; i += 64) nz |= p[i] != 0.f;
+  }
+  if (lane < rows) nz |= d_raw_sigma[row0 + lane] != 0.f;
+  const bool live = __ballot(nz) != 0ull;
+  if (lane == 0) chunk_live[chunk] = (uint8_t)live;
+}
+constexpr int kPackLanes = 4;
+constexpr int kPackThreads = 64;
+__global__ __launch_bounds__(kPackThreads) void pack_live_kernel(const uint8_t* __restrict__ chunk_live, TileSched ts,
+                                                                 uint8_t* __restrict__ tile_live, int32_t* __restrict__ pack) {
+  __shared__ __attribute__((aligned(4))) uint8_t flags[kPackLanes * kPackWindow * kPackPos];
+  const int t = threadIdx.x;
+  const int64_t n_slots = ts.n_full + ts.n_half, n_win = pack_windows(ts);
+  const int64_t w0 = blockIdx.x * (int64_t)kPackLanes;
+  const int64_t s0 = w0 * kPackWindow, s1 = s0 + kPackLanes * kPackWindow < n_slots ? s0 + kPackLanes * kPackWindow : n_slots;
+  const int64_t c0 = slot_row0(ts, s0) / kLiveRows, c1 = slot_row0(ts, s1) / kLiveRows;
+  const uint32_t* __restrict__ src = reinterpret_cast<const uint32_t*>(chunk_live + c0);
+  for (int i = t; i < (int)(c1 - c0) / 4; i += kPackThreads) reinterpret_cast<uint32_t*>(flags)[i] = src[i];
+  __syncthreads();
+  const int64_t w = w0 + t;
+  if (t >= kPackLanes || w >= n_win) return;
+  const int n = pack_window(flags, ts, w, nullptr, tile_live, c0);
+  if (n == 0) return;
+  const int64_t base = atomicAdd(reinterpret_cast<unsigned int*>(pack), (unsigned int)n);
+  pack_window(flags, ts, w, pack + kPackHead + base * kPackPos, nullptr, c0);
+}
+
+template <int NHB>
+__device__ __forceinline__ void bwd_tile_packed(float* __restrict__ lds, float* __restrict__ dbias_partial,
+                                                const float* __restrict__ pkb, const float* __restrict__ d_raw_rgb,
+                                                const float* __restrict__ d_raw_sigma, const uint32_t* __restrict__ mask,
+                                                int64_t M, int deg, const TileSched& ts, const int32_t* __restrict__ vt,
+                                                float* __restrict__ dz, int* __restrict__ lsrc, int tid, int lane, int wave) {
+  constexpr int NH = 32 * NHB;
+  constexpr int RBN = kRB;
+  constexpr int kRows = 32 * RBN;
+  static_assert(kPackPos == 2 * RBN && kMaskWords == 2 && kCB == 1, "chunk position = (row block, register half)");
+  const int C = rgb_channels(deg);
+  const ARows arow = make_arows(lds, lane);
+  const WImage wimg = make_wimage(pkb, bwd_image_floats(deg), lane);
+  lds_barrier();
+  if (tid < kPackPos) lsrc[tid] = vt[tid];
+  lds_barrier();
+  int slot[kPackPos];
+  uint32_t soff[kPackPos];
+  unsigned used = 0;
+  unsigned ends = 0;
+  unsigned mbytes = 0;
+  const int half_row0 = (int)ts.half_row0, n_full = (int)ts.n_full;
+  const int base_row = __builtin_amdgcn_readfirstlane(lsrc[0]);
+  int end_row = base_row;
+#pragma unroll
+  for (int p = 0; p < kPackPos; ++p) {
+    const int r = __builtin_amdgcn_readfirstlane(lsrc[p]);
+    const bool on = r >= 0, full = r < half_row0;
+    slot[p] = !on ? -1 : full ? r / kTM : n_full + (r - half_row0) / (kTM / 2);
+    const int j = full ? (r % kTM) / kLiveRows : ((r - half_row0) % (kTM / 2)) / kLiveRows;
+    if (on) {
+      used |= 1u << p;
+      mbytes |= (unsigned)((j >> 2) * 4 + 3 - (j & 3)) << (4 * p);
+      end_row = r + kLiveRows;
+    }
+    soff[p] = (uint32_t)(r - base_row) * (kW * 4);
+  }
+#pragma unroll
+  for (int p = 0; p < kPackPos; ++p)
+    if (((used >> p) & 1u) && (p == kPackPos - 1 || slot[p + 1] != slot[p])) ends |= 1u << p;
+  if (end_row > M) end_row = (int)M;
+  const uint32_t span_bytes = (uint32_t)(end_row - base_row) * (kW * 4);
+#pragma unroll
+  for (int p = 0; p < kPackPos; ++p)
+    if (!((used >> p) & 1u)) soff[p] = span_bytes;
+
+  for (int idx = tid; idx < kRows * NH; idx += kMlpThreads) {
+    const int row = idx / NH, col = idx - row * NH;
+    const int s = lsrc[row / kLiveRows];
+    const int64_t grow = (int64_t)s + (row % kLiveRows);
+    float v = 0.f;
+    if (s >= 0 && grow < M) {
+      if (col < C) { if (d_raw_rgb) v = d_raw_rgb[grow * C + col]; }
+      else if (col == C) v = d_raw_sigma[grow];
+    }
+    lds[row * kLDA + col] = v;
+  }
+  lds_barrier();
+  if (tid < kW) {
+    float sum = 0.f;
+#pragma unroll
+    for (int p = 0; p < kPackPos; ++p) {
+      if (!((used >> p) & 1u)) continue;
+      if (tid < NH) {
+#pragma unroll 8
+        for (int row = p * kLiveRows; row < (p + 1) * kLiveRows; ++row) sum += lds[row * kLDA + tid];
+      }
+      if ((ends >> p) & 1u) {
+        dbias_partial[(int64_t)slot[p] * 9 * kW + 8 * kW + tid] = sum;
+        sum = 0.f;
+      }
+    }
+  }
+
+  const uint8_t* __restrict__ mask_bytes = reinterpret_cast<const uint8_t*>(mask);
+  auto load_mask = [&](int l, int t, uint32_t (&mb)[kPackPos]) {
+#pragma unroll
+    for (int p = 0; p < kPackPos; ++p) {
+      mb[p] = 0u;
+      if ((used >> p) & 1u)
+        mb[p] = mask_bytes[((((int64_t)slot[p] * kDepth + l) * kMlpThreads + t) * kMaskWords) * 4 + ((mbytes >> (4 * p)) & 7u)];
+    }
+  };
+  auto join_mask = [&](const uint32_t (&mb)[kPackPos], uint32_t (&mw)[kMaskWords]) {
+#pragma unroll
+    for (int w = 0; w < kMaskWords; ++w)
+      mw[w] = (mb[4 * w] << 24) | (mb[4 * w + 1] << 16) | (mb[4 * w + 2] << 8) | mb[4 * w + 3];
+  };
+
+  f32x16 acc[RBN][kCB];
+  f32x4 bfrag[4][kCB];
+  zero_acc(acc);
+  uint32_t mb[kPackPos];
+  {
+    load_mask(kDepth - 1, tid, mb);
+    const int wp = (wave * kCB) * 64;
+    gemm_prefetch_b<kCB>(wimg, wp, 4 * NHB, 8 * 64, bfrag);
+    gemm_lds_packed<RBN, kCB>(arow, wimg, wp, 4 * NHB, 8 * 64, acc, bfrag);
+  }
+  for (int l = kDepth - 1; l >= 0; --l) {
+    const int wp = (int)(bwd_layer_off(l > 0 ? l : 1, deg) / 4) + (wave * kCB) * 64;
+    if (l > 0) gemm_prefetch_b<kCB>(wimg, wp, 32, 8 * 64, bfrag);
+    uint32_t mw[kMaskWords];
+    join_mask(mb, mw);
+    lds_barrier();
+    int tid_e = tid;
+    asm volatile("" : "+v"(tid_e));
+    const int lane_e = tid_e & 63;
+    {
+      const int col = wave * 32 + (lane_e & 31);
+      float colsum = 0.f;
+#pragma unroll
+      for (int r = 0; r < RBN; ++r)
+#pragma unroll
+        for (int reg = 0; reg < 16; ++reg) {
+          const int row = r * 32 + frag_row(reg, lane_e);
+          const float v = mask_pop(mw[(r * 16 + reg) >> 5], acc[r][0][reg]);
+          lds[row * kLDA + col] = v;
+          colsum += v;
+          if ((reg & 7) == 7 && ((ends >> (2 * r + (reg >> 3))) & 1u)) {
+            const float both = colsum + __shfl_xor(colsum, 32);
+            if (lane_e < 32) dbias_partial[(int64_t)slot[2 * r + (reg >> 3)] * 9 * kW + l * kW + col] = both;
+            colsum = 0.f;
+          }
+        }
+    }
+    const int c4 = lane_e & 7, rsub = lane_e >> 3;
+    PackCopy tc;
+    tc.voff = (uint32_t)(rsub * kW + wave * 32 + c4 * 4) * 4u;
+    tc.src = lds + rsub * kLDA + wave * 32 + c4 * 4;
+    tc.src_hi = 8 * 8 * kLDA;
+    asm volatile("" : "+v"(tc.src_hi));
+#pragma unroll
+    for (int p = 0; p < kPackPos; ++p) tc.soff[p] = soff[p];
+    tc.on = true;
+    tc.out = __builtin_amdgcn_make_buffer_rsrc(dz + ((int64_t)l * M + base_row) * kW, 0, (int)span_bytes, 0x00020000);
+    if (l == 0) {
+#pragma unroll
+      for (int i = 0; i < 4 * RBN; ++i) tile_copy_slab<RBN>(tc, i);
+    }
+    lds_barrier();
+    if (l == 0) break;
+    zero_acc(acc);
+    load_mask(l - 1, tid_e, mb);
+    gemm_lds_packed<RBN, kCB, true, PackCopy>(arow, wimg, wp, 32, 8 * 64, acc, bfrag, &tc);
+  }
+}
+
+template <int NHB, bool SKIP, bool DYN, bool PACK = false>
 __global__ __launch_bounds__(kMlpThreads, kMlpWgPerCu * kMlpWaves / 4) void mlp_bwd_data_kernel(
     const float* __restrict__ pkb, const float* __restrict__ d_raw_rgb,
     const float* __restrict__ d_raw_sigma, const uint32_t* __restrict__ mask, int64_t M, int deg, TileSched ts,
     float* __restrict__ dz, float* __restrict__ dbias_partial, uint8_t* __restrict__ chunk_live,
-    unsigned int* __restrict__ tile_counter) {
+    unsigned int* __restrict__ tile_counter, const int32_t* __restrict__ pack) {
   __shared__ __attribute__((aligned(16))) float lds[kTM * kLDA + kTM / kLiveRows + 4];
   int* __restrict__ nz = reinterpret_cast<int*>(lds + kTM * kLDA);
   const int tid = threadIdx.x, lane = tid & 63;
@@ -669,7 +870,16 @@
       bwd_tile<NHB, kRB / 2, SKIP>(lds, db, tile_live + slot, pkb, d_raw_rgb, d_raw_sigma, mask, M, deg,
                              ts.half_row0 + (slot - ts.n_full) * (kTM / 2), slot, dz, nz, chunk_live, tid, lane, wave);
   };
-  if (!DYN) {
+  if (PACK) {
+    const TileTicket tk{nz + kTM / kLiveRows, tile_counter};
+    const int n_vt = __builtin_amdgcn_readfirstlane(pack[0]);
+    for (int v = blockIdx.x; v < n_vt;) {
+      const int ticket = tk.draw(tid);
+      bwd_tile_packed<NHB>(lds, dbias_partial, pkb, d_raw_rgb, d_raw_sigma, mask, M, deg, ts,
+                           pack + kPackHead + (int64_t)v * kPackPos, dz, nz, tid, lane, wave);
+      v = (int)tk.take(tid, ticket);
+    }
+  } else if (!DYN) {
     for (int64_t slot = blockIdx.x; slot < ts.n_full; slot += gridDim.x) run(slot);
     for (int64_t h = blockIdx.x; h < ts.n_half; h += gridDim.x) run(ts.n_full + h);
   } else {
@@ -690,7 +900,7 @@
 int launch_mlp_bwd_data(const PxoCfg* cfg, const float* packed_bwd, const float* d_raw_rgb,
                         const float* d_raw_sigma, const uint32_t* mask, int64_t M, float* dz,
                         float* dbias_partial, uint8_t* chunk_live, unsigned int* tile_counter, hipStream_t s,
-                        bool bias_from_wgrad) {
+                        bool bias_from_wgrad, bool compact) {
   if (M == 0) return PXO_OK;
   if (cfg->mlp_precision == PXO_MLP_BF16X6)
     return launch_mlp_bwd_data_x6(cfg, packed_bwd, d_raw_rgb, d_raw_sigma, mask, M, dz, dbias_partial, chunk_live, tile_counter, s,
@@ -699,12 +909,25 @@
   KernelTimer timer(PXO_PROF_MLP_BWD_DATA, M, s);
   dim3 grid_dim(mlp_grid(M)), block(kMlpThreads);
   const TileSched ts = tile_sched(M, grid_dim.x);
+  int32_t* const pack = compact ? dbias_pack_list(dbias_partial, M, ts.n_full + ts.n_half) : nullptr;
+  if (compact) {
+    if (!chunk_live || !tile_counter || !pack || M >= ((int64_t)1 << 31)) {
+      set_error("mlp_bwd_data: the compacting mode needs chunk_live, a tile counter, fewer than 2^31 rows and room for the pack list");
+      return PXO_ERR_ARG;
+    }
+    const int64_t n_chunks = num_tiles(M) * (kTM / kLiveRows);
+    hipLaunchKernelGGL(live_chunks_kernel, dim3((unsigned)((n_chunks + 3) / 4)), dim3(256), 0, s, d_raw_rgb, d_raw_sigma, M,
+                       rgb_channels(cfg->sh_deg), n_chunks, chunk_live, pack);
+    hipLaunchKernelGGL(pack_live_kernel, dim3((unsigned)((pack_windows(ts) + kPackLanes - 1) / kPackLanes)), dim3(kPackThreads), 0, s,
+                       chunk_live, ts,
+                       const_cast<uint8_t*>(dbias_tile_live(dbias_partial, M)), pack);
+  }
   head_switch(cfg->sh_deg, [&](auto nhb) {
     constexpr int NHB = decltype(nhb)::value;
-    const auto kernel = chunk_live ? (tile_counter ? mlp_bwd_data_kernel<NHB, true, true> : mlp_bwd_data_kernel<NHB, true, false>)
+    const auto kernel = pack ? mlp_bwd_data_kernel<NHB, true, true, true> : chunk_live ? (tile_counter ? mlp_bwd_data_kernel<NHB, true, true> : mlp_bwd_data_kernel<NHB, true, false>)
                                    : (tile_counter ? mlp_bwd_data_kernel<NHB, false, true> : mlp_bwd_data_kernel<NHB, false, false>);
     hipLaunchKernelGGL(kernel, grid_dim, block, 0, s, packed_bwd, d_raw_rgb, d_raw_sigma, mask, M, cfg->sh_deg, ts, dz,
-                       dbias_partial, chunk_live, tile_counter);
+                       dbias_partial, chunk_live, tile_counter, pack);
   });
   return check_launch("mlp_bwd_data");
 }
diff --git a/plenoctree_amd/csrc/pxo_api.hip b/plenoctree_amd/csrc/pxo_api.hip
--- a/plenoctree_amd/csrc/pxo_api.hip
+++ b/plenoctree_amd/csrc/pxo_api.hip
@@ -47,9 +47,10 @@
 static std::atomic<int> g_tune_x6_wgrad{1};
 static std::atomic<int> g_tune_coarse_stream{0};
 static std::atomic<int> g_tune_vd_ray_block{PXO_VD_RAY_BLOCK_DEFAULT};
+static std::atomic<int> g_tune_bwd_compact{1};
 Tuning tuning_snapshot() {
   return Tuning{g_tune_tile_sched.load(), g_tune_wgrad_ranges.load(), g_tune_wgrad_skinny_ranges.load(),
-                g_tune_coarse_stream.load(), g_tune_x6_wgrad.load(), g_tune_vd_ray_block.load()};
+                g_tune_coarse_stream.load(), g_tune_x6_wgrad.load(), g_tune_vd_ray_block.load(), g_tune_bwd_compact.load()};
 }
 
 struct SideStream { hipStream_t stream = nullptr; hipEvent_t fork = nullptr, join = nullptr; };
@@ -400,7 +401,8 @@
     d_sigma = k->d_sigma_live;
   }
   uint8_t* const live = plan.skip ? p.live : nullptr;
-  PXO_TRY(launch_mlp_bwd_data(cfg, packed_bwd, d_rgb, d_sigma, p.mask, M, p.dz, p.dbias, live, tile_counter, s, plan.bias_from_wgrad));
+  PXO_TRY(launch_mlp_bwd_data(cfg, packed_bwd, d_rgb, d_sigma, p.mask, M, p.dz, p.dbias, live, tile_counter, s, plan.bias_from_wgrad,
+                              plan.compact));
   if (join && !join->join()) {
     set_error("%s: join of the side stream failed", who);
     return PXO_ERR_HIP;
@@ -453,6 +455,10 @@
                   PXO_VD_RAY_BLOCK_MAX, value);
       g_tune_vd_ray_block = value;
       return PXO_OK;
+    case PXO_TUNE_BWD_COMPACT:
+      PXO_REQUIRE(value == 0 || value == 1, "pxo_set_tuning: compacting backward(data) must be 0 (tile / half-tile skipping) or 1, got %d", value);
+      g_tune_bwd_compact = value;
+      return PXO_OK;
     default:
       set_error("pxo_set_tuning: unknown knob %d", knob);
       return PXO_ERR_ARG;
@@ -467,6 +473,7 @@
     case PXO_TUNE_COARSE_REVERSE_STREAM: *value = g_tune_coarse_stream; return PXO_OK;
     case PXO_TUNE_X6_WGRAD: *value = g_tune_x6_wgrad; return PXO_OK;
     case PXO_TUNE_VD_RAY_BLOCK: *value = g_tune_vd_ray_block; return PXO_OK;
+    case PXO_TUNE_BWD_COMPACT: *value = g_tune_bwd_compact; return PXO_OK;
     default: set_error("pxo_get_tuning: unknown knob %d", knob); return PXO_ERR_ARG;
   }
 }
@@ -536,6 +543,53 @@
               "pxo_mlp_bwd_data: bad arguments");
   return launch_mlp_bwd_data(cfg, packed_bwd, d_raw_rgb, d_raw_sigma, (const uint32_t*)relu_mask, M, dz,
                              dbias_partial, nullptr, nullptr, (hipStream_t)stream, false);
+}
+
+struct SkipWs { uint8_t* live; unsigned int* counter; size_t total; };
+static SkipWs carve_skip(void* ws, int64_t M) {
+  Carver c(ws);
+  SkipWs k;
+  k.live = c.take<uint8_t>(live_flags(M));
+  k.counter = c.take<unsigned int>(4);
+  k.total = (c.off + 255) & ~(size_t)255;
+  return k;
+}
+size_t pxo_skip_workspace_bytes(int64_t M) { return carve_skip(nullptr, M > 0 ? M : 1).total; }
+
+int pxo_mlp_bwd_data_skip(const PxoCfg* cfg, const float* packed_bwd, const float* d_raw_rgb, const float* d_raw_sigma,
+                          const void* relu_mask, int64_t M, float* dz, float* dbias_partial, void* skip_ws, size_t skip_ws_bytes,
+                          void* stream) {
+  PXO_TRY(validate_cfg(cfg));
+  if (M == 0) return PXO_OK;
+  PXO_REQUIRE(M >= 0 && packed_bwd && d_raw_rgb && d_raw_sigma && relu_mask && dz && dbias_partial && skip_ws,
+              "pxo_mlp_bwd_data_skip: bad arguments");
+  PXO_TRY(require_train_precision(cfg, "pxo_mlp_bwd_data_skip"));
+  PxoCfg c = *cfg;
+  c.skip_zero_rows = 1;
+  const StepPlan plan = plan_step(c, M, 0, num_cus(), tuning_snapshot());
+  PXO_REQUIRE(plan.skip, "pxo_mlp_bwd_data_skip: %lld rows do not fit the live-chunk lists of the weight gradients", (long long)M);
+  const SkipWs k = carve_skip(skip_ws, M);
+  if (skip_ws_bytes < k.total) { set_error("pxo_mlp_bwd_data_skip: workspace %zu < %zu", skip_ws_bytes, k.total); return PXO_ERR_WORKSPACE; }
+  hipStream_t s = (hipStream_t)stream;
+  if (hipMemsetAsync(k.counter, 0, sizeof(unsigned int), s) != hipSuccess) { set_error("hipMemsetAsync failed"); return PXO_ERR_HIP; }
+  return launch_mlp_bwd_data(cfg, packed_bwd, d_raw_rgb, d_raw_sigma, (const uint32_t*)relu_mask, M, dz, dbias_partial, k.live,
+                             k.counter, s, plan.bias_from_wgrad, plan.compact);
+}
+
+int pxo_mlp_bwd_weights_skip(const PxoCfg* cfg, const float* acts, const float* enc, const float* dz, const float* d_raw_rgb,
+                             const float* d_raw_sigma, const float* dbias_partial, int64_t M, float* grads, void* ws,
+                             size_t ws_bytes, const void* skip_ws, size_t skip_ws_bytes, void* stream) {
+  PXO_TRY(validate_cfg(cfg));
+  PXO_REQUIRE(M >= 0 && acts && enc && dz && d_raw_rgb && d_raw_sigma && dbias_partial && grads && ws && skip_ws,
+              "pxo_mlp_bwd_weights_skip: bad arguments");
+  PxoCfg c = *cfg;
+  c.skip_zero_rows = 1;
+  const StepPlan plan = plan_step(c, M, 0, num_cus(), tuning_snapshot());
+  PXO_REQUIRE(plan.skip, "pxo_mlp_bwd_weights_skip: %lld rows do not fit the live-chunk lists of the weight gradients", (long long)M);
+  const SkipWs k = carve_skip(const_cast<void*>(skip_ws), M > 0 ? M : 1);
+  if (skip_ws_bytes < k.total) { set_error("pxo_mlp_bwd_weights_skip: workspace %zu < %zu", skip_ws_bytes, k.total); return PXO_ERR_WORKSPACE; }
+  return launch_mlp_bwd_weights(cfg, acts, enc, dz, d_raw_rgb, d_raw_sigma, dbias_partial, M, grads, ws, ws_bytes, k.live,
+                                (hipStream_t)stream, plan.split_c, plan.x6_main, plan.bias_from_wgrad);
 }
 
 int pxo_wgrad_workspace_bytes(const PxoCfg* cfg, int64_t M, size_t* bytes) {
@@ -801,7 +855,7 @@
   unsigned int* const cnt_bwd_f = (plan.dyn || cfg->skip_zero_rows) ? counters + 3 : nullptr;
   Draws dr;
   PXO_TRY(prepare_draws(cfg, t, B, randomized, t_rand, u, sp_points, seed, s, dr, params, 2 * n_mlp, sumsq_partial, step_words,
-                        kStepWords, cx ? kStepRecordCulled : kStepRecord | (plan.skip ? 1u : 0u)));
+                        kStepWords, cx ? kStepRecordCulled : kStepRecord | (plan.skip ? 1u : 0u) | (plan.compact ? 2u : 0u)));
   if (sg) PXO_TRY(launch_sg_lobes(sg_params, sgK, g.lobes, s));
   int64_t M_c = 0, M_f = 0;
   PXO_TRY(level_forward(cfg, t, 0, packed_fwd0, origins, directions, viewdirs, B, dr, pixels, nullptr, nullptr, nullptr, s,
@@ -938,7 +992,7 @@
               "live rows only (the chunk totals of the dense row count do not describe it; see its live_rows)");
     return PXO_ERR_ARG;
   }
-  if ((record & ~1u) != kStepRecord) { set_error("pxo_train_backward_work: no pxo_train_fwd_bwd call has used this workspace"); return PXO_ERR_ARG; }
+  if ((record & ~3u) != kStepRecord) { set_error("pxo_train_backward_work: no pxo_train_fwd_bwd call has used this workspace"); return PXO_ERR_ARG; }
   if (!(record & 1u)) {
     *live_chunks = nc + nf;
     return PXO_OK;
@@ -953,6 +1007,32 @@
     return PXO_ERR_HIP;
   }
   *live_chunks = (int64_t)host;
+  return PXO_OK;
+}
+
+int pxo_train_pack_tiles(const PxoCfg* cfg, int64_t B, void* ws, size_t ws_bytes, int64_t* virtual_tiles, void* stream) {
+  PXO_TRY(validate_cfg(cfg));
+  PXO_REQUIRE(B >= 1 && ws && virtual_tiles, "pxo_train_pack_tiles: bad arguments");
+  Layout L;
+  PXO_TRY(lay_out(cfg, B, ws, ws_bytes, true, false, false, "pxo_train_pack_tiles", L));
+  const TrainWs& t = L.t;
+  hipStream_t s = (hipStream_t)stream;
+  unsigned int record = 0;
+  int32_t n[2] = {0, 0};
+  bool ok = hipMemcpyAsync(&record, t.scalars + kStepWordsAt, sizeof(record), hipMemcpyDeviceToHost, s) == hipSuccess &&
+            hipStreamSynchronize(s) == hipSuccess;
+  if (ok && (record & ~3u) == kStepRecord && (record & 2u)) {
+    const int32_t* pack_c = dbias_pack_list(t.c.dbias, t.c.M, mlp_bwd_partials(t.c.M));
+    const int32_t* pack_f = cfg->num_fine_samples > 0 ? dbias_pack_list(t.f.dbias, t.f.M, mlp_bwd_partials(t.f.M)) : nullptr;
+    ok = pack_c && hipMemcpyAsync(&n[0], pack_c, sizeof(int32_t), hipMemcpyDeviceToHost, s) == hipSuccess &&
+         (!pack_f || hipMemcpyAsync(&n[1], pack_f, sizeof(int32_t), hipMemcpyDeviceToHost, s) == hipSuccess) &&
+         hipStreamSynchronize(s) == hipSuccess;
+  } else if (ok) {
+    set_error("pxo_train_pack_tiles: the last step on this workspace did not run the compacting backward(data)");
+    return PXO_ERR_ARG;
+  }
+  if (!ok) { set_error("pxo_train_pack_tiles: copy back failed"); return PXO_ERR_HIP; }
+  *virtual_tiles = (int64_t)n[0] + n[1];
   return PXO_OK;
 }
 
diff --git a/plenoctree_amd/csrc/pxo_common.h b/plenoctree_amd/csrc/pxo_common.h
--- a/plenoctree_amd/csrc/pxo_common.h
+++ b/plenoctree_amd/csrc/pxo_common.h
@@ -114,6 +114,64 @@
   return reinterpret_cast<const uint8_t*>(dbias_partial + mask_slots(M) * 9 * kW);
 }
 
+constexpr int kPackPos = kTM / kLiveRows;
+constexpr int kPackWindow = 64;
+constexpr int kPackOpen = 16;
+constexpr int kPackHead = 4;
+constexpr int32_t kPackEmpty = -1;
+__host__ __device__ inline int64_t slot_row0(const TileSched& ts, int64_t slot) {
+  return slot < ts.n_full ? slot * kTM : ts.half_row0 + (slot - ts.n_full) * (kTM / 2);
+}
+__host__ __device__ inline int slot_chunks(const TileSched& ts, int64_t slot) {
+  return slot < ts.n_full ? kPackPos : kPackPos / 2;
+}
+__host__ __device__ inline int64_t pack_windows(const TileSched& ts) {
+  return (ts.n_full + ts.n_half + kPackWindow - 1) / kPackWindow;
+}
+__host__ __device__ inline int64_t pack_words(int64_t n_slots) { return kPackHead + n_slots * kPackPos; }
+__host__ __device__ inline int32_t* dbias_pack_list(float* dbias_partial, int64_t M, int64_t n_slots) {
+  const int64_t spare = (mask_slots(M) - n_slots) * 9 * kW;
+  return pack_words(n_slots) <= spare ? reinterpret_cast<int32_t*>(dbias_partial + n_slots * 9 * kW) : nullptr;
+}
+__host__ __device__ inline bool pack_list_fits(int64_t M) {
+  const int64_t worst_slots = num_tiles(M) + kMaxMlpGrid / 4 + 2;
+  return M < ((int64_t)1 << 31) && pack_words(worst_slots) <= (kMaxMlpGrid / 2 - kMaxMlpGrid / 4 - 2) * (int64_t)(9 * kW);
+}
+__host__ __device__ inline int pack_window(const uint8_t* chunk_live, const TileSched& ts, int64_t w, int32_t* tiles,
+                                           uint8_t* tile_live, int64_t chunk0 = 0) {
+  const int64_t n_slots = ts.n_full + ts.n_half;
+  const int64_t s0 = w * kPackWindow, s1 = s0 + kPackWindow < n_slots ? s0 + kPackWindow : n_slots;
+  int n_tiles = 0;
+  uint64_t fills = 0;
+  for (int64_t s = s0; s < s1; ++s) {
+    const int64_t row0 = slot_row0(ts, s);
+    const uint8_t* cl = chunk_live + (row0 / kLiveRows - chunk0);
+    const int nch = slot_chunks(ts, s);
+    int n = 0;
+    for (int j = 0; j < nch; ++j) n += cl[j] != 0;
+    if (tile_live) tile_live[s] = (uint8_t)(n != 0);
+    if (n == 0) continue;
+    int t = n_tiles > kPackOpen ? n_tiles - kPackOpen : 0;
+    for (; t < n_tiles; ++t)
+      if ((int)((fills >> (4 * (t % kPackOpen))) & 15u) + n <= kPackPos) break;
+    if (t == n_tiles) {
+      if (tiles)
+        for (int p = 0; p < kPackPos; ++p) tiles[(int64_t)t * kPackPos + p] = kPackEmpty;
+      fills &= ~((uint64_t)15u << (4 * (t % kPackOpen)));
+      ++n_tiles;
+    }
+    const int sh = 4 * (t % kPackOpen);
+    int fill = (int)((fills >> sh) & 15u);
+    for (int j = 0; j < nch; ++j)
+      if (cl[j] != 0) {
+        if (tiles) tiles[(int64_t)t * kPackPos + fill] = (int32_t)(row0 + j * kLiveRows);
+        ++fill;
+      }
+    fills = (fills & ~((uint64_t)15u << sh)) | ((uint64_t)fill << sh);
+  }
+  return n_tiles;
+}
+
 void set_error(const char* fmt, ...);
 int check_launch(const char* what);
 
@@ -147,7 +205,7 @@
 int launch_mlp_bwd_data(const PxoCfg* cfg, const float* packed_bwd, const float* d_raw_rgb,
                         const float* d_raw_sigma, const uint32_t* mask, int64_t M, float* dz,
                         float* dbias_partial, uint8_t* chunk_live, unsigned int* tile_counter, hipStream_t s,
-                        bool bias_from_wgrad);
+                        bool bias_from_wgrad, bool compact = false);
 
 struct Tuning {
   int tile_sched;
@@ -156,6 +214,7 @@
   int coarse_stream;
   int x6_wgrad;
   int vd_ray_block;
+  int bwd_compact;
 };
 Tuning tuning_snapshot();
 
@@ -192,6 +251,7 @@
   bool x6_main;
   bool bias_from_wgrad;
   bool fork;
+  bool compact;
 };
 inline StepPlan plan_step(const PxoCfg& cfg, int64_t M_c, int64_t M_f, int ncu, const Tuning& tu) {
   StepPlan p;
@@ -203,6 +263,7 @@
   p.x6_main = cfg.mlp_precision == PXO_MLP_BF16X6 && tu.x6_wgrad != 0;
   p.bias_from_wgrad = p.x6_main;
   p.fork = M_f > 0 && tu.coarse_stream != 0;
+  p.compact = p.skip && cfg.mlp_precision == PXO_MLP_F32 && tu.bwd_compact != 0 && pack_list_fits(M_c) && pack_list_fits(M_f);
   return p;
 }
 
diff --git a/plenoctree_amd/ops.py b/plenoctree_amd/ops.py
--- a/plenoctree_amd/ops.py
+++ b/plenoctree_amd/ops.py
@@ -146,6 +146,38 @@
     return grads
 
 
+def mlp_bwd_data_skip(cfg, packed_bwd, d_raw_rgb, d_raw_sigma, mask, poison=False):
+    _require_gpu()
+    lib = _lib.load()
+    M = d_raw_sigma.shape[0]
+    dev = d_raw_sigma.device
+    dz = _new(NET_DEPTH, M, NET_WIDTH, device=dev)
+    dbias = _new(max(dbias_partial_bytes(M) // 4, 4), device=dev)
+    nbytes = lib.pxo_skip_workspace_bytes(M)
+    skip_ws = _new(nbytes, device=dev, dtype=torch.uint8)
+    if poison:
+        dz.view(torch.uint8).fill_(0xFF); dbias.view(torch.uint8).fill_(0xFF); skip_ws.fill_(0xFF)
+    check(lib.pxo_mlp_bwd_data_skip(ctypes.byref(cfg), _f(packed_bwd), _f(d_raw_rgb), _f(d_raw_sigma), _p(mask), M,
+                                    _f(dz), _f(dbias), _p(skip_ws), nbytes, _stream()), "pxo_mlp_bwd_data_skip")
+    return dz, dbias, skip_ws
+
+
+def mlp_bwd_weights_skip(cfg, acts, enc, dz, d_raw_rgb, d_raw_sigma, dbias, skip_ws):
+    _require_gpu()
+    lib = _lib.load()
+    M = d_raw_sigma.shape[0]
+    dev = d_raw_sigma.device
+    _, n = param_layout(cfg)
+    grads = _new(n, device=dev)
+    nbytes = ctypes.c_size_t(0)
+    check(lib.pxo_wgrad_workspace_bytes(ctypes.byref(cfg), M, ctypes.byref(nbytes)), "pxo_wgrad_workspace_bytes")
+    ws = _new(max(nbytes.value, 16), device=dev, dtype=torch.uint8)
+    check(lib.pxo_mlp_bwd_weights_skip(ctypes.byref(cfg), _f(acts), _f(enc), _f(dz), _f(d_raw_rgb), _f(d_raw_sigma),
+                                       _f(dbias), M, _f(grads), _p(ws), nbytes.value, _p(skip_ws), skip_ws.numel(), _stream()),
+          "pxo_mlp_bwd_weights_skip")
+    return grads
+
+
 def shade_composite_fwd(cfg, raw_rgb, raw_sigma, z_vals, directions, viewdirs):
     _require_gpu()
     lib = _lib.load()
@@ -393,8 +425,16 @@
 PROF_MLP_FWD, PROF_MLP_BWD_DATA, PROF_WGRAD_MAIN, PROF_WGRAD_OTHER, PROF_NUM_TAGS = 0, 1, 2, 3, 4
 
 
+def train_pack_tiles(cfg, B, ws):
+    n = ctypes.c_int64(0)
+    check(_lib.load().pxo_train_pack_tiles(ctypes.byref(cfg), B, _p(ws), ws.numel(), ctypes.byref(n), _stream()),
+          "pxo_train_pack_tiles")
+    return n.value
+
+
 TUNE_TILE_SCHED, TUNE_WGRAD_RANGES, TUNE_WGRAD_SKINNY_RANGES, TUNE_COARSE_REVERSE_STREAM, TUNE_X6_WGRAD = 0, 1, 2, 3, 4
 TUNE_VD_RAY_BLOCK = 5
+TUNE_BWD_COMPACT = 6
 
 
 def set_tuning(knob, value):
```

After: 171,600. No clear change (-0.2%).
